# r4dl/LAENeRF

Measured on AMD Instinct MI355X. Metric: Mrays/s, lego 800x800 train-step (4096 rays/step), higher is better.
Workload: dtype f16 (table, MLP) / f32 (march, composite)

## Files before the change

### include/laenerf.h

```cpp
#ifndef LAENERF_H
#define LAENERF_H

#include <stdint.h>

#ifdef __cplusplus
extern "C" {
#endif

#if defined(__GNUC__) || defined(__clang__)
#define LAE_API __attribute__((visibility("default")))
#else
#define LAE_API
#endif

#define LAE_OK 0
#define LAE_EINVAL (-1)
#define LAE_ELAUNCH (-2)
#define LAE_ENULL (-3)

#define LAE_F32 0
#define LAE_F16 1

#define LAE_GRID_HASH 0
#define LAE_GRID_TILED 1
#define LAE_INTERP_LINEAR 0
#define LAE_INTERP_SMOOTHSTEP 1

#define LAE_ACT_RELU 0
#define LAE_ACT_EXPONENTIAL 1
#define LAE_ACT_SINE 2
#define LAE_ACT_SIGMOID 3
#define LAE_ACT_SQUAREPLUS 4
#define LAE_ACT_SOFTPLUS 5
#define LAE_ACT_NONE 6

#define LAE_ABI_TAG "abi10"
LAE_API const char* lae_version(void);
LAE_API const char* lae_last_error(void);


LAE_API int lae_near_far_from_aabb(const float* rays_o, const float* rays_d, const float* aabb,
                           uint32_t N, float min_near, float* nears, float* fars, void* stream);

LAE_API int lae_get_rays(const float* poses, uint32_t B, float fx, float fy, float cx, float cy, uint32_t H, uint32_t W,
                 const int64_t* inds, uint64_t inds_batch_stride, uint32_t N, int perturb, float off_x, float off_y,
                 float* rays_o, float* rays_d, const float* aabb, float min_near, float* nears, float* fars, void* stream);

#define LAE_IMG_U8 0
#define LAE_IMG_F16 1
#define LAE_IMG_F32 2
#define LAE_BATCH_IMAGE 0
#define LAE_BATCH_ALL 1
#define LAE_BG_WHITE 0
#define LAE_BG_RANDOM 1
LAE_API int lae_sample_train_batch(const void* images, int dtype, uint32_t n_img, uint32_t H, uint32_t W, uint32_t C,
                           const float* poses, float fx, float fy, float cx, float cy, uint32_t N,
                           const float* aabb, float min_near, uint64_t seed, int64_t* step_counter, int mode, int bg_mode,
                           int srgb_to_linear, float* rays_o, float* rays_d, float* nears, float* fars, float* gt,
                           float* bg_out, int64_t* inds, void* stream);

LAE_API int lae_sample_train_batch_weighted(const void* images, int dtype, uint32_t n_img, uint32_t H, uint32_t W, uint32_t C,
                                    const float* poses, float fx, float fy, float cx, float cy, uint32_t N,
                                    const float* aabb, float min_near, uint64_t seed, int64_t* step_counter, int bg_mode,
                                    int srgb_to_linear, const float* error_map, int32_t* cells_out, float* rays_o, float* rays_d,
                                    float* nears, float* fars, float* gt, float* bg_out, int64_t* inds, void* stream);

LAE_API int lae_error_map_update(float* error_map, uint32_t n_img, uint32_t H, uint32_t W, const int64_t* inds, const int32_t* cells,
                                 const float* pred, const float* gt, uint32_t N, void* stream);

LAE_API int lae_sph_from_ray(const float* rays_o, const float* rays_d, float radius, uint32_t N,
                     float* coords, void* stream);

LAE_API int lae_morton3D(const int32_t* coords, uint32_t N, int32_t* indices, void* stream);

LAE_API int lae_morton3D_invert(const int32_t* indices, uint32_t N, int32_t* coords, void* stream);

LAE_API int lae_packbits(const float* grid, uint32_t N, float density_thresh, uint8_t* bitfield,
                 void* stream);

LAE_API uint64_t lae_march_rays_train_scratch_bytes(uint32_t N);
LAE_API int lae_march_rays_train(const float* rays_o, const float* rays_d, const uint8_t* grid,
                         float bound, float dt_gamma, uint32_t max_steps,
                         uint32_t N, uint32_t C, uint32_t H, uint32_t M,
                         const float* nears, const float* fars,
                         float* xyzs, float* dirs, float* deltas,
                         int32_t* rays, int32_t* counter, const float* noises,
                         void* scratch, uint32_t* rows_end_out, void* stream);

LAE_API int lae_march_rays_train_limit(const float* rays_o, const float* rays_d, const uint8_t* grid,
                               float bound, float dt_gamma, uint32_t max_steps,
                               uint32_t N, uint32_t C, uint32_t H, uint32_t M_cap, const uint32_t* m_limit,
                               const float* nears, const float* fars,
                               float* xyzs, float* dirs, float* deltas,
                               int32_t* rays, int32_t* counter, const float* noises,
                               void* scratch, uint32_t* rows_end_out, void* stream);

LAE_API int lae_composite_rays_train_forward(const float* sigmas, const float* rgbs, const float* deltas,
                                     const int32_t* rays, uint32_t M, uint32_t N, float T_thresh,
                                     float* weights_sum, float* depth, float* image, void* stream);

LAE_API int lae_composite_rays_train_backward(const float* grad_weights_sum, const float* grad_image,
                                      const float* sigmas, const float* rgbs, const float* deltas,
                                      const int32_t* rays, const float* weights_sum,
                                      const float* image, uint32_t M, uint32_t N, float T_thresh,
                                      float* grad_sigmas, float* grad_rgbs, void* stream);

LAE_API int lae_composite_rays_train_forward_blend(const float* sigmas, const float* rgbs, const float* deltas, const int32_t* rays,
                                           uint32_t M, uint32_t N, float T_thresh, const float* nears, const float* fars,
                                           const float* bg_rays, float bg_r, float bg_g, float bg_b, float* weights_sum,
                                           float* depth, float* image, float* depth_out, float* image_out, void* stream);
LAE_API int lae_composite_rays_train_step(const float* sigmas, const float* rgbs, const float* deltas, const int32_t* rays, uint32_t M,
                                  uint32_t N, float T_thresh, const float* nears, const float* fars, const float* bg_rays, float bg_r,
                                  float bg_g, float bg_b, const uint32_t* rows_end, const float* target, const float* scale,
                                  float* weights_sum, float* depth, float* image, float* depth_out, float* image_out,
                                  float* grad_image, float* grad_sigmas, float* grad_rgbs, float* loss_out, float* partials,
                                  int defer_loss, void* stream);
LAE_API int lae_loss_finish(const float* partials, uint32_t n_part, uint32_t n_elem, const float* scale, float* loss_out, void* stream);

LAE_API int lae_composite_rays_train_backward_blend(const float* grad_weights_sum, const float* grad_image, const float* sigmas,
                                            const float* rgbs, const float* deltas, const int32_t* rays,
                                            const float* weights_sum, const float* image, uint32_t M, uint32_t N,
                                            float T_thresh, const float* bg_rays, float bg_r, float bg_g, float bg_b,
                                            const uint32_t* rows_end, float* grad_sigmas, float* grad_rgbs, void* stream);
LAE_API int lae_composite_rays_train_backward_blend_ex(const float* grad_weights_sum, const float* grad_image, const float* sigmas,
                                               const float* rgbs, const float* deltas, const int32_t* rays,
                                               const float* weights_sum, const float* image, uint32_t M, uint32_t N,
                                               float T_thresh, const float* bg_rays, float bg_r, float bg_g, float bg_b,
                                               const uint32_t* rows_end, const float* grad_scale, float* grad_sigmas,
                                               float* grad_rgbs, void* stream);

LAE_API int lae_march_rays(uint32_t n_alive, uint32_t n_step, const int32_t* rays_alive,
                   const float* rays_t, const float* rays_o, const float* rays_d,
                   float bound, float dt_gamma, uint32_t max_steps, uint32_t C, uint32_t H,
                   const uint8_t* grid, const float* nears, const float* fars,
                   float* xyzs, float* dirs, float* deltas, const float* noises, void* stream);

LAE_API int lae_march_rays_distill(uint32_t n_alive, uint32_t n_step, const int32_t* rays_alive,
                           const float* rays_t, const float* rays_o, const float* rays_d,
                           float bound, float dt_gamma, uint32_t max_steps, uint32_t C, uint32_t H,
                           const uint8_t* grid, const uint8_t* edit_grid,
                           const float* nears, const float* fars,
                           float* xyzs, float* dirs, float* deltas, uint8_t* edit_occ,
                           const float* noises, void* stream);

LAE_API int lae_composite_rays(uint32_t n_alive, uint32_t n_step, float T_thresh,
                       int32_t* rays_alive, float* rays_t,
                       const float* sigmas, const float* rgbs, const float* deltas,
                       float* weights_sum, float* depth, float* image, void* stream);

LAE_API int lae_composite_rays_distill(uint32_t n_alive, uint32_t n_step, float T_thresh,
                               int32_t* rays_alive, float* rays_t,
                               const float* sigmas, const float* rgbs, const float* deltas,
                               float* weights_sum, float* weights_edit_sum,
                               float* depth, float* depth_edit,
                               const uint8_t* edit_occ, float* image, void* stream);

LAE_API uint64_t lae_render_frame_workspace_bytes(uint32_t N, uint32_t L, uint64_t row_budget);
LAE_API int lae_render_frame_set_overlap(int on);
LAE_API int lae_render_frame_mode(void);
LAE_API int lae_render_frame_last_status(void);
LAE_API int lae_render_frame_probe_us(float* us, uint32_t n);
LAE_API int lae_render_frame(const float* rays_o, const float* rays_d, uint32_t N, const float* aabb, float min_near,
                     const uint8_t* grid, const uint8_t* edit_grid, float bound, float dt_gamma, uint32_t max_steps,
                     uint32_t C, uint32_t H, const void* table_f16, const int32_t* offsets, const int32_t* offsets_host,
                     uint32_t L, float S,
                     uint32_t base_resolution, uint32_t gridtype, int align_corners, uint32_t interp,
                     const void* sigma_weights, const void* color_weights, float density_scale, float T_thresh,
                     uint32_t max_n_step, uint64_t row_budget, const float* noises, const float* bg_rays, float bg_r, float bg_g,
                     float bg_b, int blend_bg, int scale_depth, float* weights_sum, float* depth, float* image,
                     float* weights_edit, float* depth_edit, void* workspace, uint64_t workspace_bytes, uint32_t* stats_out,
                     void* stream);

LAE_API uint64_t lae_compact_scratch_bytes(uint32_t n_alive);
LAE_API int lae_compact_rays_alive(const int32_t* rays_alive, uint32_t n_alive, int32_t* out_alive,
                           int32_t* n_out_dev, void* scratch, void* stream);


LAE_API int lae_grid_encode_forward(const float* inputs, const void* embeddings, const int32_t* offsets,
                            void* outputs, uint32_t B, uint32_t D, uint32_t C, uint32_t L,
                            float S, uint32_t H, void* dy_dx, uint32_t gridtype,
                            int align_corners, uint32_t interp, int dtype, void* stream);

LAE_API int lae_grid_encode_backward(const void* grad, const float* inputs, const void* embeddings,
                             const int32_t* offsets, void* grad_embeddings, uint32_t B,
                             uint32_t D, uint32_t C, uint32_t L, float S, uint32_t H,
                             const void* dy_dx, void* grad_inputs, uint32_t gridtype,
                             int align_corners, uint32_t interp, int dtype, void* stream);

LAE_API int lae_grid_encode_forward_ex(const float* inputs, const void* embeddings, const int32_t* offsets, void* outputs,
                               uint32_t B, uint32_t D, uint32_t C, uint32_t L, float S, uint32_t H, void* dy_dx,
                               uint32_t gridtype, int align_corners, uint32_t interp, int dtype, int blc, float in_shift,
                               float in_scale, const int32_t* offsets_host, void* stream);
LAE_API int lae_grid_encode_backward_ex(const void* grad, const float* inputs, const void* embeddings, const int32_t* offsets,
                                void* grad_embeddings, uint32_t B, uint32_t D, uint32_t C, uint32_t L, float S,
                                uint32_t H, const void* dy_dx, void* grad_inputs, uint32_t gridtype,
                                int align_corners, uint32_t interp, int dtype, int blc, float in_shift, float in_scale,
                                const int32_t* offsets_host, int32_t* nonfinite_flag, uint32_t* touched_lines, void* stream);

LAE_API uint64_t lae_grid_backward_plan_bytes(uint32_t B, uint32_t L);
LAE_API uint64_t lae_grid_touched_lines_words(uint64_t n_entries);
LAE_API int lae_grid_encode_backward_plan(const float* inputs, const int32_t* offsets, uint32_t B, uint32_t D, uint32_t C, uint32_t L,
                                  float S, uint32_t H, uint32_t gridtype, int align_corners, uint32_t interp, int dtype,
                                  float in_shift, float in_scale, const int32_t* offsets_host, void* plan,
                                  uint32_t* touched_lines, void* stream);
LAE_API int lae_grid_encode_backward_planned(const void* grad, const float* inputs, const int32_t* offsets, void* grad_embeddings,
                                     uint32_t B, uint32_t D, uint32_t C, uint32_t L, float S, uint32_t H, uint32_t gridtype,
                                     int align_corners, uint32_t interp, int dtype, float in_shift, float in_scale,
                                     const int32_t* offsets_host, const void* plan, int32_t* nonfinite_flag, void* stream);

LAE_API uint64_t lae_grid_backward_workspace_bytes(uint32_t B, uint32_t L, int dtype);

LAE_API int lae_grid_forward_schedule(const int32_t* offsets_host, uint32_t L, float S, uint32_t H, uint32_t n_chunks,
                              uint32_t* nseg_out, uint32_t* segs_out);

LAE_API int lae_grid_set_forward_mode(int mode);

LAE_API int lae_grid_set_backward_mode(int mode);

LAE_API int lae_grad_total_variation(const void* inputs, const void* embeddings, void* grad,
                             const int32_t* offsets, float weight, uint32_t B, uint32_t D,
                             uint32_t C, uint32_t L, float S, uint32_t H, uint32_t gridtype,
                             int align_corners, int dtype, void* stream);


LAE_API int lae_sh_encode_forward(const float* inputs, float* outputs, uint32_t B, uint32_t D,
                          uint32_t C, float* dy_dx, void* stream);

LAE_API int lae_sh_encode_backward(const float* grad, const float* inputs, uint32_t B, uint32_t D,
                           uint32_t C, const float* dy_dx, float* grad_inputs, void* stream);


LAE_API int lae_ffmlp_forward(const void* inputs, const void* weights, uint32_t B, uint32_t input_dim,
                      uint32_t output_dim, uint32_t hidden_dim, uint32_t num_layers,
                      uint32_t activation, uint32_t output_activation, void* forward_buffer,
                      void* outputs, void* stream);

LAE_API int lae_ffmlp_inference(const void* inputs, const void* weights, uint32_t B, uint32_t input_dim,
                        uint32_t output_dim, uint32_t hidden_dim, uint32_t num_layers,
                        uint32_t activation, uint32_t output_activation, void* inference_buffer,
                        void* outputs, void* stream);

LAE_API int lae_ffmlp_backward(const void* grad, const void* inputs, const void* weights,
                       const void* forward_buffer, uint32_t B, uint32_t input_dim,
                       uint32_t output_dim, uint32_t hidden_dim, uint32_t num_layers,
                       uint32_t activation, uint32_t output_activation, int calc_grad_inputs,
                       void* backward_buffer, void* grad_inputs, void* grad_weights,
                       void* stream);
LAE_API int lae_ffmlp_backward_ex(const void* grad, const void* inputs, const void* weights,
                          const void* forward_buffer, uint32_t B, uint32_t input_dim,
                          uint32_t output_dim, uint32_t hidden_dim, uint32_t num_layers,
                          uint32_t activation, uint32_t output_activation, int calc_grad_inputs,
                          void* backward_buffer, void* grad_inputs, void* grad_weights,
                          int accumulate, int32_t* nonfinite_flag, void* stream);

LAE_API int lae_nerf_head_forward(const void* enc, const float* dirs, const void* sigma_weights, const void* color_weights,
                          uint32_t M, float density_scale, void* h_out, float* sigmas, float* rgbs, int enc_level_major,
                          void* stream);

LAE_API int lae_nerf_density_forward(const void* enc, const void* sigma_weights, uint32_t M, float density_scale, void* h_out,
                             float* sigmas, int enc_level_major, void* stream);

LAE_API int lae_nerf_head_backward(const float* grad_sigmas, const float* grad_rgbs, const void* enc, const float* dirs, const void* h,
                           const float* rgbs, const void* sigma_weights, const void* color_weights, uint32_t M,
                           float density_scale, void* grad_h, void* grad_enc, void* grad_sigma_weights,
                           void* grad_color_weights, int accumulate_weight_grads, int enc_level_major,
                           int32_t* nonfinite_flag, const float* loss_partials, uint32_t loss_n_part, uint32_t loss_n_elem,
                           const float* loss_scale, float* loss_out, void* stream);

LAE_API int lae_freq_encode_forward(const float* inputs, uint32_t B, uint32_t D, uint32_t deg, uint32_t C, float* outputs,
                            void* stream);
LAE_API int lae_freq_encode_backward(const float* grad, const float* outputs, uint32_t B, uint32_t D, uint32_t deg, uint32_t C,
                             float* grad_inputs, void* stream);

LAE_API int lae_palette_forward(const void* w_logits, const void* o_raw, const float* palette, uint32_t P, uint32_t active_mask,
                        uint32_t M, void* pred, float* w_hat, void* o_hat, void* stream);
LAE_API uint64_t lae_palette_backward_scratch_bytes(uint32_t M);
LAE_API int lae_palette_backward(const void* w_logits, const void* o_raw, const float* palette, uint32_t P, uint32_t active_mask,
                         uint32_t M, const void* g_pred, const float* g_w, const void* g_o, void* g_w_logits, void* g_o_raw,
                         float* g_palette, void* scratch, void* stream);

#define LAE_RECOLOR_PREVIEW 0
#define LAE_RECOLOR_WEIGHTS 1
#define LAE_RECOLOR_OFFSETS 2
#define LAE_RECOLOR_EVAL 3
#define LAE_RECOLOR_NO_OFFSETS 1
#define LAE_RECOLOR_TANH 2
LAE_API uint64_t lae_recolor_compact_scratch_bytes(uint32_t N);
LAE_API int lae_recolor_compact(const float* depth, const float* weights_sum, const float* rays_o, const float* rays_d, uint32_t N,
                                int32_t* indices, int32_t* slot_map, float* x_term, float* dirs, float* alpha, int32_t* count,
                                void* scratch, void* stream);
LAE_API int lae_recolor_compose(const int32_t* slot_map, uint32_t N, const void* w_logits, uint32_t w_stride, const void* o_raw,
                                uint32_t o_stride, uint32_t P, uint32_t active_mask, const float* palette, const float* p_weights,
                                const float* p_bias, const float* alpha, const float* base, const float* bg, int mode, uint32_t k,
                                int flags, float* out, uint8_t* out_u8, void* stream);

#define LAE_STYLE_WITH_REG 1
#define LAE_STYLE_ACCUMULATE_PALETTE 2
LAE_API uint64_t lae_style_loss_scratch_bytes(uint32_t M);
LAE_API int lae_style_loss_forward(const void* pred, const float* target, const float* w_hat, const void* o_hat, uint32_t M,
                           uint32_t n_active, float w_uniform, float w_non_uniform, float c_offset, const float* scale, float* fin,
                           void* scratch, const float* reg_palette, uint32_t reg_P, float w_valid, float w_distinct, void* stream);
LAE_API int lae_style_loss_backward(const void* w_logits, const void* o_raw, const float* palette, uint32_t P, uint32_t active_mask,
                            uint32_t M, const float* target, const float* fin, const float* upstream, float w_uniform,
                            float w_non_uniform, float c_offset, void* g_w_logits, void* g_o_raw, float* g_palette, void* scratch,
                            int flags, float w_valid, float w_distinct, void* stream);

LAE_API int lae_style_loss_forward_dev(const void* pred, const float* target, const float* w_hat, const void* o_hat, uint32_t cap,
                               const uint32_t* m_dev, uint32_t n_active, float w_uniform, float w_non_uniform, float c_offset,
                               const float* scale, float* fin, void* scratch, const float* reg_palette, uint32_t reg_P, float w_valid,
                               float w_distinct, void* stream);
LAE_API int lae_style_loss_backward_dev(const void* w_logits, const void* o_raw, const float* palette, uint32_t P, uint32_t active_mask,
                                uint32_t cap, const uint32_t* m_dev, const float* target, const float* fin, const float* upstream,
                                float w_uniform, float w_non_uniform, float c_offset, void* g_w_logits, void* g_o_raw, float* g_palette,
                                void* scratch, int flags, float w_valid, float w_distinct, void* stream);

LAE_API int lae_sample_edit_view(const float* x_term, const float* dirs, const float* targets, const int64_t* offsets, const int32_t* counts,
                         const float* depth_factor, uint32_t V, const int32_t* schedule, uint32_t n_sched, uint32_t cap, uint64_t seed,
                         int64_t* step_counter, float* x, float* d, float* target, uint32_t* m_dev, void* stream);

LAE_API int lae_style_assemble_forward(const void* feats_lm, const float* dirs, uint32_t M, uint32_t Mp, uint32_t degree, void* feat,
                               void* off_in, uint32_t off_cols, void* stream);
LAE_API int lae_style_assemble_backward(const void* g_feat, const void* g_off, uint32_t M, uint32_t off_cols, void* grad_lm, void* stream);

LAE_API int lae_grow_region(uint8_t* grid, const float* density_grid, uint32_t C, uint32_t H, float density_thresh,
                    uint32_t* queue, uint32_t capacity, uint32_t* state, uint32_t grow_iterations, uint32_t max_batch,
                    void* stream);

LAE_API int lae_min_dist_to_points(const float* pts, uint32_t n, const float* set, uint32_t m, float max_dist, float* out,
                           float* out_max, void* scratch, void* stream);

LAE_API int lae_density_grid_positions(const int32_t* coords, uint32_t n, uint32_t H, float bound_c, const float* noise,
                               float* xyzs, int32_t* indices, void* stream);
LAE_API uint64_t lae_density_grid_partial_scratch_bytes(uint32_t cells, uint32_t n);
LAE_API int lae_density_grid_partial_positions(const float* grid_c, uint32_t cells, const int32_t* coords_rand, const float* u, const float* rnd,
                                       uint32_t n, uint32_t H, float bound_c, const float* noise, float* xyzs, int32_t* indices,
                                       void* scratch, void* stream);
LAE_API int lae_density_grid_update(const float* sigmas, const int32_t* indices, uint32_t n, float density_scale, float decay,
                            uint32_t cells, float* grid, uint32_t* tmp, void* stream);
LAE_API int lae_mark_untrained_grid(const float* poses, uint32_t B, float fx, float fy, float cx, float cy, uint32_t C, uint32_t H,
                            float bound, float min_near, int filter_close_point, float* grid, void* stream);

LAE_API int lae_adam_check(const void* grad, int grad_is_half, uint64_t n, void* state, void* stream);
LAE_API int lae_adam_begin(void* state, float beta1, float beta2, int growth_interval, float growth_factor, float backoff_factor,
                   int use_scaler, void* stream);
LAE_API int lae_adam_apply(float* param, float* exp_avg, float* exp_avg_sq, void* grad, int grad_is_half, void* shadow_half, uint64_t n,
                   const void* state, const float* lr, float beta1, float beta2, float eps, float weight_decay, void* stream);

LAE_API int lae_mse_loss_forward(const float* pred, const float* target, uint32_t n, const float* scale, float* loss_out, float* grad,
                         void* stream);

LAE_API int lae_adam_check_multi(uint32_t n_tensors, const void* const* grads, const int* grad_is_half, const uint64_t* sizes, void* state,
                         void* stream);
LAE_API int lae_adam_apply_multi(uint32_t n_tensors, float* const* params, float* const* exp_avgs, float* const* exp_avg_sqs, void* const* grads,
                         const int* grad_is_half, void* const* shadows_half, const uint64_t* sizes, const float* const* lrs, const void* const* touched_lines,
                         const void* state, float beta1, float beta2, float eps, float weight_decay, void* stream);

LAE_API int lae_ema_update_multi(uint32_t n_tensors, float* const* shadows, const float* const* params, const uint64_t* sizes,
                         float one_minus_decay, void* stream);

LAE_API int lae_ffmlp_set_mode(int mode);

LAE_API int lae_allocate_splitk(uint64_t size);
LAE_API int lae_free_splitk(void);

LAE_API int lae_free_workspaces(void);
LAE_API uint64_t lae_workspace_bytes(int retired);

#ifdef __cplusplus
}
#endif
#endif
```

### laenerf_amd/_lib.py

```python
import ctypes
import os

import torch

_HERE = os.path.dirname(os.path.abspath(__file__))
SO_PATH = os.environ.get("LAE_HIP_LIB") or os.path.join(_HERE, "lib", "liblaenerf_hip.so")

u32, u64, f32, i32, vp = ctypes.c_uint32, ctypes.c_uint64, ctypes.c_float, ctypes.c_int, ctypes.c_void_p

SIGNATURES = {
    "lae_near_far_from_aabb": [vp, vp, vp, u32, f32, vp, vp, vp],
    "lae_sph_from_ray": [vp, vp, f32, u32, vp, vp],
    "lae_get_rays": [vp, u32, f32, f32, f32, f32, u32, u32, vp, u64, u32, i32, f32, f32, vp, vp, vp, f32, vp, vp, vp],
    "lae_morton3D": [vp, u32, vp, vp],
    "lae_morton3D_invert": [vp, u32, vp, vp],
    "lae_packbits": [vp, u32, f32, vp, vp],
    "lae_march_rays_train_scratch_bytes": [u32],
    "lae_march_rays_train": [vp, vp, vp, f32, f32, u32, u32, u32, u32, u32, vp, vp, vp, vp, vp, vp, vp, vp, vp, vp, vp],
    "lae_march_rays_train_limit": [vp, vp, vp, f32, f32, u32, u32, u32, u32, u32, vp, vp, vp, vp, vp, vp, vp, vp, vp, vp, vp, vp],
    "lae_sample_train_batch": [vp, i32, u32, u32, u32, u32, vp, f32, f32, f32, f32, u32, vp, f32, u64, vp, i32, i32, i32, vp, vp, vp, vp, vp,
                               vp, vp, vp],
    "lae_sample_train_batch_weighted": [vp, i32, u32, u32, u32, u32, vp, f32, f32, f32, f32, u32, vp, f32, u64, vp, i32, i32, vp, vp,
                                        vp, vp, vp, vp, vp, vp, vp, vp],
    "lae_error_map_update": [vp, u32, u32, u32, vp, vp, vp, vp, u32, vp],
    "lae_composite_rays_train_forward": [vp, vp, vp, vp, u32, u32, f32, vp, vp, vp, vp],
    "lae_composite_rays_train_backward": [vp, vp, vp, vp, vp, vp, vp, vp, u32, u32, f32, vp, vp, vp],
    "lae_composite_rays_train_forward_blend": [vp, vp, vp, vp, u32, u32, f32, vp, vp, vp, f32, f32, f32, vp, vp, vp, vp, vp, vp],
    "lae_composite_rays_train_step": [vp, vp, vp, vp, u32, u32, f32, vp, vp, vp, f32, f32, f32, vp, vp, vp, vp, vp, vp, vp, vp, vp, vp, vp, vp, vp, i32, vp],
    "lae_loss_finish": [vp, u32, u32, vp, vp, vp],
    "lae_composite_rays_train_backward_blend": [vp, vp, vp, vp, vp, vp, vp, vp, u32, u32, f32, vp, f32, f32, f32, vp, vp, vp, vp],
    "lae_composite_rays_train_backward_blend_ex": [vp, vp, vp, vp, vp, vp, vp, vp, u32, u32, f32, vp, f32, f32, f32, vp, vp, vp, vp, vp],
    "lae_march_rays": [u32, u32, vp, vp, vp, vp, f32, f32, u32, u32, u32, vp, vp, vp, vp, vp, vp, vp, vp],
    "lae_march_rays_distill": [u32, u32, vp, vp, vp, vp, f32, f32, u32, u32, u32, vp, vp, vp, vp, vp, vp, vp, vp, vp, vp],
    "lae_composite_rays": [u32, u32, f32, vp, vp, vp, vp, vp, vp, vp, vp, vp],
    "lae_composite_rays_distill": [u32, u32, f32, vp, vp, vp, vp, vp, vp, vp, vp, vp, vp, vp, vp],
    "lae_render_frame_workspace_bytes": [u32, u32, u64],
    "lae_render_frame_set_overlap": [i32],
    "lae_render_frame_mode": [],
    "lae_render_frame_last_status": [],
    "lae_render_frame_probe_us": [vp, u32],
    "lae_render_frame": [vp, vp, u32, vp, f32, vp, vp, f32, f32, u32, u32, u32, vp, vp, vp, u32, f32, u32, u32, i32, u32, vp, vp, f32, f32,
                         u32, u64, vp, vp, f32, f32, f32, i32, i32, vp, vp, vp, vp, vp, vp, u64, vp, vp],
    "lae_compact_scratch_bytes": [u32],
    "lae_compact_rays_alive": [vp, u32, vp, vp, vp, vp],
    "lae_grid_encode_forward": [vp, vp, vp, vp, u32, u32, u32, u32, f32, u32, vp, u32, i32, u32, i32, vp],
    "lae_grid_encode_backward": [vp, vp, vp, vp, vp, u32, u32, u32, u32, f32, u32, vp, vp, u32, i32, u32, i32, vp],
    "lae_grid_encode_forward_ex": [vp, vp, vp, vp, u32, u32, u32, u32, f32, u32, vp, u32, i32, u32, i32, i32, f32, f32, vp, vp],
    "lae_grid_encode_backward_ex": [vp, vp, vp, vp, vp, u32, u32, u32, u32, f32, u32, vp, vp, u32, i32, u32, i32, i32, f32, f32, vp, vp, vp, vp],
    "lae_grid_backward_workspace_bytes": [u32, u32, i32],
    "lae_grid_backward_plan_bytes": [u32, u32],
    "lae_grid_touched_lines_words": [u64],
    "lae_grid_encode_backward_plan": [vp, vp, u32, u32, u32, u32, f32, u32, u32, i32, u32, i32, f32, f32, vp, vp, vp, vp],
    "lae_grid_encode_backward_planned": [vp, vp, vp, vp, u32, u32, u32, u32, f32, u32, u32, i32, u32, i32, f32, f32, vp, vp, vp, vp],
    "lae_grid_set_backward_mode": [i32],
    "lae_grid_set_forward_mode": [i32],
    "lae_grid_forward_schedule": [vp, u32, f32, u32, u32, vp, vp],
    "lae_grad_total_variation": [vp, vp, vp, vp, f32, u32, u32, u32, u32, f32, u32, u32, i32, i32, vp],
    "lae_sh_encode_forward": [vp, vp, u32, u32, u32, vp, vp],
    "lae_sh_encode_backward": [vp, vp, u32, u32, u32, vp, vp, vp],
    "lae_freq_encode_forward": [vp, u32, u32, u32, u32, vp, vp],
    "lae_freq_encode_backward": [vp, vp, u32, u32, u32, u32, vp, vp],
    "lae_ffmlp_forward": [vp, vp, u32, u32, u32, u32, u32, u32, u32, vp, vp, vp],
    "lae_ffmlp_inference": [vp, vp, u32, u32, u32, u32, u32, u32, u32, vp, vp, vp],
    "lae_ffmlp_backward": [vp, vp, vp, vp, u32, u32, u32, u32, u32, u32, u32, i32, vp, vp, vp, vp],
    "lae_ffmlp_backward_ex": [vp, vp, vp, vp, u32, u32, u32, u32, u32, u32, u32, i32, vp, vp, vp, i32, vp, vp],
    "lae_nerf_head_forward": [vp, vp, vp, vp, u32, f32, vp, vp, vp, i32, vp],
    "lae_nerf_density_forward": [vp, vp, u32, f32, vp, vp, i32, vp],
    "lae_density_grid_positions": [vp, u32, u32, f32, vp, vp, vp, vp],
    "lae_density_grid_partial_scratch_bytes": [u32, u32],
    "lae_density_grid_partial_positions": [vp, u32, vp, vp, vp, u32, u32, f32, vp, vp, vp, vp, vp],
    "lae_density_grid_update": [vp, vp, u32, f32, f32, u32, vp, vp, vp],
    "lae_mark_untrained_grid": [vp, u32, f32, f32, f32, f32, u32, u32, f32, f32, i32, vp, vp],
    "lae_nerf_head_backward": [vp, vp, vp, vp, vp, vp, vp, vp, u32, f32, vp, vp, vp, vp, i32, i32, vp, vp, u32, u32, vp, vp, vp],
    "lae_palette_forward": [vp, vp, vp, u32, u32, u32, vp, vp, vp, vp],
    "lae_palette_backward_scratch_bytes": [u32],
    "lae_palette_backward": [vp, vp, vp, u32, u32, u32, vp, vp, vp, vp, vp, vp, vp, vp],
    "lae_recolor_compact_scratch_bytes": [u32],
    "lae_recolor_compact": [vp, vp, vp, vp, u32, vp, vp, vp, vp, vp, vp, vp, vp],
    "lae_recolor_compose": [vp, u32, vp, u32, vp, u32, u32, u32, vp, vp, vp, vp, vp, vp, i32, u32, i32, vp, vp, vp],
    "lae_style_loss_scratch_bytes": [u32],
    "lae_style_loss_forward": [vp, vp, vp, vp, u32, u32, f32, f32, f32, vp, vp, vp, vp, u32, f32, f32, vp],
    "lae_style_loss_backward": [vp, vp, vp, u32, u32, u32, vp, vp, vp, f32, f32, f32, vp, vp, vp, vp, i32, f32, f32, vp],
    "lae_style_loss_forward_dev": [vp, vp, vp, vp, u32, vp, u32, f32, f32, f32, vp, vp, vp, vp, u32, f32, f32, vp],
    "lae_style_loss_backward_dev": [vp, vp, vp, u32, u32, u32, vp, vp, vp, vp, f32, f32, f32, vp, vp, vp, vp, i32, f32, f32, vp],
    "lae_sample_edit_view": [vp, vp, vp, vp, vp, vp, u32, vp, u32, u32, u64, vp, vp, vp, vp, vp, vp],
    "lae_grow_region": [vp, vp, u32, u32, f32, vp, u32, vp, u32, u32, vp],
    "lae_style_assemble_forward": [vp, vp, u32, u32, u32, vp, vp, u32, vp],
    "lae_style_assemble_backward": [vp, vp, u32, u32, vp, vp],
    "lae_min_dist_to_points": [vp, u32, vp, u32, f32, vp, vp, vp, vp],
    "lae_mse_loss_forward": [vp, vp, u32, vp, vp, vp, vp],
    "lae_adam_check": [vp, i32, u64, vp, vp],
    "lae_adam_check_multi": [u32, vp, vp, vp, vp, vp],
    "lae_adam_apply_multi": [u32, vp, vp, vp, vp, vp, vp, vp, vp, vp, vp, f32, f32, f32, f32, vp],
    "lae_adam_begin": [vp, f32, f32, i32, f32, f32, i32, vp],
    "lae_ema_update_multi": [u32, vp, vp, vp, f32, vp],
    "lae_adam_apply": [vp, vp, vp, vp, i32, vp, u64, vp, vp, f32, f32, f32, f32, vp],
    "lae_ffmlp_set_mode": [i32],
    "lae_allocate_splitk": [u64],
    "lae_free_splitk": [],
    "lae_free_workspaces": [],
    "lae_workspace_bytes": [i32],
    "lae_version": [],
    "lae_last_error": [],
}
_RESTYPES = {
    "lae_march_rays_train_scratch_bytes": u64,
    "lae_compact_scratch_bytes": u64,
    "lae_density_grid_partial_scratch_bytes": u64,
    "lae_palette_backward_scratch_bytes": u64,
    "lae_style_loss_scratch_bytes": u64,
    "lae_recolor_compact_scratch_bytes": u64,
    "lae_render_frame_workspace_bytes": u64,
    "lae_workspace_bytes": u64,
    "lae_grid_backward_workspace_bytes": u64,
    "lae_grid_backward_plan_bytes": u64,
    "lae_grid_touched_lines_words": u64,
    "lae_version": ctypes.c_char_p,
    "lae_last_error": ctypes.c_char_p,
}

_lib = None
ABI_TAG = b"abi10"


def _abi_of(path):
    lib = ctypes.CDLL(path)
    fn = lib.lae_version
    fn.argtypes, fn.restype = [], ctypes.c_char_p
    return lib, fn().split()[-1]


def load():
    global _lib
    if _lib is not None:
        return _lib
    if not os.path.exists(SO_PATH):
        raise RuntimeError(
            f"laenerf_amd: HIP library not built ({SO_PATH}); run `python -m laenerf_amd.build` "
            "(there is no CPU fallback)")
    if not os.environ.get("LAE_HIP_LIB"):
        from . import build as _build
        if _build.default_is_packed(SO_PATH):
            _build.build(force=True)
            if _build.default_is_packed(SO_PATH):
                raise RuntimeError(f"laenerf_amd: {SO_PATH} was built with packed-fp32 instructions and could not be rebuilt without them")
    lib, tag = _abi_of(SO_PATH)
    if tag != ABI_TAG:
        if os.environ.get("LAE_HIP_LIB"):
            raise RuntimeError(f"laenerf_amd: {SO_PATH} is ABI {tag.decode()}, this package binds {ABI_TAG.decode()}")
        import fcntl
        import shutil
        from . import build as _build
        with open(SO_PATH + ".lock", "w") as lock:
            fcntl.flock(lock, fcntl.LOCK_EX)
            try:
                probe = SO_PATH + f".{os.getpid()}.probe"
                shutil.copyfile(SO_PATH, probe)
                try:
                    still_stale = _abi_of(probe)[1] != ABI_TAG
                finally:
                    os.remove(probe)
                if still_stale:
                    _build.build(force=True)
            finally:
                fcntl.flock(lock, fcntl.LOCK_UN)
        fresh = SO_PATH + f".{os.getpid()}.reload"
        shutil.copyfile(SO_PATH, fresh)
        try:
            lib, tag = _abi_of(fresh)
        finally:
            os.remove(fresh)
        if tag != ABI_TAG:
            raise RuntimeError(f"laenerf_amd: rebuilt library is ABI {tag.decode()}, this package binds {ABI_TAG.decode()}")
    for name, argtypes in SIGNATURES.items():
        fn = getattr(lib, name)
        fn.argtypes = argtypes
        fn.restype = _RESTYPES.get(name, ctypes.c_int)
    _lib = lib
    return lib


def check(rc, what):
    if rc != 0:
        msg = load().lae_last_error().decode() if rc == -2 else {-1: "invalid argument / unsupported configuration",
                                                                 -3: "null pointer"}.get(rc, "error")
        raise RuntimeError(f"laenerf_amd.{what} failed (code {rc}): {msg}")


def ptr(t):
    return None if t is None else t.data_ptr()


def stream():
    return torch.cuda.current_stream().cuda_stream


def need_cuda(*tensors):
    cur = None
    for t in tensors:
        if t is None:
            continue
        if not t.is_cuda:
            raise RuntimeError("laenerf_amd: tensor must be on the GPU (HIP backend, no CPU fallback)")
        if cur is None:
            cur = torch.cuda.current_device()
# ... 10 lines not shown
```

### laenerf_amd/backend.py

```python
import sys
import types

import numpy as np
import torch

from . import _lib
from ._lib import check, need_contig, need_cuda, ptr, stream

_F16 = torch.float16


def _dtype_code(t):
    if t.dtype == torch.float32:
        return 0
    if t.dtype == torch.float16:
        return 1
    raise RuntimeError(f"laenerf_amd: unsupported dtype {t.dtype} (float32 / float16 only)")


def _host_i32(a, n):
    if a is None:
        return None
    if not (isinstance(a, np.ndarray) and a.dtype == np.int32 and a.flags.c_contiguous and a.size == n):
        raise RuntimeError("laenerf_amd: offsets_host must be a contiguous int32 numpy array with L + 1 entries")
# ... 291 lines not shown
        check(lib.lae_render_frame(ptr(rays_o), ptr(rays_d), N, ptr(aabb), float(min_near), ptr(grid), ptr(edit_grid), float(bound),
                                   float(dt_gamma), max_steps, C, H, ptr(table_f16), ptr(offsets), _host_i32(offsets_host, L + 1), L, float(S),
                                   base_resolution,
                                   gridtype, int(bool(align_corners)), interp, ptr(sigma_weights), ptr(color_weights),
                                   float(density_scale), float(T_thresh), max_n_step, int(row_budget), ptr(noises), ptr(bg_rays), float(bg_rgb[0]),
                                   float(bg_rgb[1]), float(bg_rgb[2]), int(bool(blend_bg)), int(bool(scale_depth)), ptr(weights_sum),
                                   ptr(depth), ptr(image), ptr(weights_edit), ptr(depth_edit), ptr(ws), ws.numel(),
                                   ctypes.cast(stats, ctypes.c_void_p) if want_stats else None, stream()), "render_frame")
        if want_stats:
            if lib.lae_render_frame_last_status() == 1:
                raise RuntimeError("laenerf_amd.render_frame: a cross-stream wait timed out behind the call; the frame's outputs are NaN")
            return {"iterations": stats[0], "rows": stats[1], "iterations_launched": stats[2]}
        return None

    @staticmethod
    def render_frame_set_overlap(on):
        check(_lib.load().lae_render_frame_set_overlap(int(bool(on))), "render_frame_set_overlap")

    @staticmethod
    def render_frame_probe():
        import ctypes
        us = (ctypes.c_float * 5)(*([-1.0] * 5))
        used = int(_lib.load().lae_render_frame_probe_us(ctypes.cast(us, ctypes.c_void_p), 5))
        return {"in_use": used, "handshake_us": [round(float(v), 1) for v in us]}

    @staticmethod
    def render_frame_mode():
        return int(_lib.load().lae_render_frame_mode())

    @staticmethod
    def render_frame_last_status():
        return int(_lib.load().lae_render_frame_last_status())

    @staticmethod
    def render_frame_check():
        torch.cuda.current_stream().synchronize()
        if _lib.load().lae_render_frame_last_status() == 1:
            raise RuntimeError("laenerf_amd.render_frame: a cross-stream wait of the most recent frame timed out after the call returned; "
                               "its outputs are NaN -- render the frame again (the library runs in line from now on)")

    @staticmethod
    def compact_rays_alive(rays_alive, n_alive, out_alive, n_out_dev):
        need_cuda(rays_alive, out_alive, n_out_dev)
        lib = _lib.load()
        ws = _workspace(rays_alive.device, lib.lae_compact_scratch_bytes(n_alive))
        check(lib.lae_compact_rays_alive(ptr(rays_alive), n_alive, ptr(out_alive), ptr(n_out_dev), ptr(ws), stream()),
              "compact_rays_alive")


class _GridEncoder:
    @staticmethod
    def grid_encode_forward(inputs, embeddings, offsets, outputs, B, D, C, L, S, H, dy_dx, gridtype, align_corners,
                            interp, blc=False, in_map=(0.0, 1.0), offsets_host=None):
        need_cuda(inputs, embeddings, offsets, outputs, dy_dx); need_contig(inputs, embeddings, offsets, outputs, dy_dx)
        if inputs.dtype != torch.float32 or offsets.dtype != torch.int32:
            raise RuntimeError("grid_encode_forward: inputs must be float32, offsets int32")
        if outputs.dtype != embeddings.dtype or (dy_dx is not None and dy_dx.dtype != embeddings.dtype):
            raise RuntimeError("grid_encode_forward: outputs/dy_dx must have the embeddings dtype")
        lib = _lib.load()
        args = (ptr(inputs), ptr(embeddings), ptr(offsets), ptr(outputs), B, D, C, L, float(S), H, ptr(dy_dx), gridtype,
                int(bool(align_corners)), interp, _dtype_code(embeddings))
        if blc or tuple(in_map) != (0.0, 1.0) or offsets_host is not None:
            check(lib.lae_grid_encode_forward_ex(*args, int(bool(blc)), float(in_map[0]), float(in_map[1]), _host_i32(offsets_host, L + 1),
                                                 stream()), "grid_encode_forward")
        else:
            check(lib.lae_grid_encode_forward(*args, stream()), "grid_encode_forward")

    @staticmethod
    def grid_backward_plan(inputs, offsets, B, D, C, L, S, H, gridtype, align_corners, interp, half, in_map=(0.0, 1.0),
                           offsets_host=None, touched_lines=None):
        need_cuda(inputs, offsets); need_contig(inputs, offsets)
        lib = _lib.load()
        plan = torch.empty(int(lib.lae_grid_backward_plan_bytes(B, L)), dtype=torch.uint8, device=inputs.device)
        check(lib.lae_grid_encode_backward_plan(ptr(inputs), ptr(offsets), B, D, C, L, float(S), H, gridtype, int(bool(align_corners)),
                                                interp, 1 if half else 0, float(in_map[0]), float(in_map[1]),
                                                _host_i32(offsets_host, L + 1), ptr(plan), touched_lines, stream()),
              "grid_backward_plan")
        plan.marks_touched = touched_lines is not None
        return plan

    @staticmethod
    def grid_encode_backward(grad, inputs, embeddings, offsets, grad_embeddings, B, D, C, L, S, H, dy_dx, grad_inputs,
                             gridtype, align_corners, interp, blc=False, in_map=(0.0, 1.0), offsets_host=None, plan=None,
                             nonfinite_flag=None, touched_lines=None):
        ts = (grad, inputs, embeddings, offsets, grad_embeddings, dy_dx, grad_inputs, plan)
        need_cuda(*ts); need_contig(*ts)
        if grad.dtype != grad_embeddings.dtype:
            raise RuntimeError("grid_encode_backward: grad and grad_embeddings dtypes differ")
        lib = _lib.load()
        if plan is not None:
            if blc or dy_dx is not None:
                raise RuntimeError("grid_encode_backward: a plan needs level-major gradients and no input gradient")
            if touched_lines is not None and not getattr(plan, "marks_touched", False):
                raise RuntimeError("grid_encode_backward: the plan was made without the touched-lines bitmap (pass it to grid_backward_plan)")
            check(lib.lae_grid_encode_backward_planned(ptr(grad), ptr(inputs), ptr(offsets), ptr(grad_embeddings), B, D, C, L, float(S), H,
                                                       gridtype, int(bool(align_corners)), interp, _dtype_code(grad), float(in_map[0]),
                                                       float(in_map[1]), _host_i32(offsets_host, L + 1), ptr(plan), nonfinite_flag, stream()),
                  "grid_encode_backward")
            return
        args = (ptr(grad), ptr(inputs), ptr(embeddings), ptr(offsets), ptr(grad_embeddings), B, D, C, L, float(S), H,
                ptr(dy_dx), ptr(grad_inputs), gridtype, int(bool(align_corners)), interp, _dtype_code(grad))
        if blc or tuple(in_map) != (0.0, 1.0) or offsets_host is not None or nonfinite_flag is not None or touched_lines is not None:
            check(lib.lae_grid_encode_backward_ex(*args, int(bool(blc)), float(in_map[0]), float(in_map[1]), _host_i32(offsets_host, L + 1),
                                                  nonfinite_flag, touched_lines, stream()), "grid_encode_backward")
        else:
            check(lib.lae_grid_encode_backward(*args, stream()), "grid_encode_backward")

    @staticmethod
    def grid_backward_workspace_bytes(B, L, half=True):
        return int(_lib.load().lae_grid_backward_workspace_bytes(B, L, 1 if half else 0))

    @staticmethod
    def set_backward_mode(mode):
        check(_lib.load().lae_grid_set_backward_mode(int(mode)), "grid_set_backward_mode")

    @staticmethod
    def grad_total_variation(inputs, embeddings, grad, offsets, weight, B, D, C, L, S, H, gridtype, align_corners):
        need_cuda(inputs, embeddings, grad, offsets); need_contig(inputs, embeddings, grad, offsets)
        check(_lib.load().lae_grad_total_variation(ptr(inputs), ptr(embeddings), ptr(grad), ptr(offsets), float(weight), B, D,
                                                   C, L, float(S), H, gridtype, int(bool(align_corners)),
                                                   _dtype_code(embeddings), stream()), "grad_total_variation")


class _SHEncoder:
    @staticmethod
    def sh_encode_forward(inputs, outputs, B, D, C, dy_dx):
        need_cuda(inputs, outputs, dy_dx); need_contig(inputs, outputs, dy_dx)
        if inputs.dtype != torch.float32 or outputs.dtype != torch.float32:
            raise RuntimeError("sh_encode_forward: float32 required (sphere_harmonics.py:16 casts to fp32)")
        check(_lib.load().lae_sh_encode_forward(ptr(inputs), ptr(outputs), B, D, C, ptr(dy_dx), stream()), "sh_encode_forward")

    @staticmethod
    def sh_encode_backward(grad, inputs, B, D, C, dy_dx, grad_inputs):
        need_cuda(grad, inputs, dy_dx, grad_inputs); need_contig(grad, inputs, dy_dx, grad_inputs)
        if grad.dtype != torch.float32:
            raise RuntimeError("sh_encode_backward: float32 required")
        check(_lib.load().lae_sh_encode_backward(ptr(grad), ptr(inputs), B, D, C, ptr(dy_dx), ptr(grad_inputs), stream()),
              "sh_encode_backward")


class _FreqEncoder:

    @staticmethod
    def freq_encode_forward(inputs, B, D, deg, C, outputs):
        need_cuda(inputs, outputs); need_contig(inputs, outputs); _need_f32(inputs, outputs)
        check(_lib.load().lae_freq_encode_forward(ptr(inputs), B, D, deg, C, ptr(outputs), stream()), "freq_encode_forward")

    @staticmethod
    def freq_encode_backward(grad, outputs, B, D, deg, C, grad_inputs):
        need_cuda(grad, outputs, grad_inputs); need_contig(grad, outputs, grad_inputs); _need_f32(grad, outputs, grad_inputs)
        check(_lib.load().lae_freq_encode_backward(ptr(grad), ptr(outputs), B, D, deg, C, ptr(grad_inputs), stream()),
              "freq_encode_backward")


class _FFMLP:
    @staticmethod
    def _half(*ts):
        for t in ts:
            if t is not None and t.dtype != _F16:
                raise RuntimeError("ffmlp: float16 tensors required (CHECK_IS_HALF, ffmlp.cu:638-642)")

    @staticmethod
    def ffmlp_forward(inputs, weights, B, input_dim, output_dim, hidden_dim, num_layers, activation, output_activation,
                      forward_buffer, outputs):
        need_cuda(inputs, weights, forward_buffer, outputs); need_contig(inputs, weights, forward_buffer, outputs)
        _FFMLP._half(inputs, weights, forward_buffer, outputs)
        check(_lib.load().lae_ffmlp_forward(ptr(inputs), ptr(weights), B, input_dim, output_dim, hidden_dim, num_layers,
                                            activation, output_activation, ptr(forward_buffer), ptr(outputs), stream()),
              "ffmlp_forward")

    @staticmethod
    def ffmlp_inference(inputs, weights, B, input_dim, output_dim, hidden_dim, num_layers, activation, output_activation,
                        inference_buffer, outputs):
        need_cuda(inputs, weights, outputs); need_contig(inputs, weights, outputs)
        _FFMLP._half(inputs, weights, outputs)
        check(_lib.load().lae_ffmlp_inference(ptr(inputs), ptr(weights), B, input_dim, output_dim, hidden_dim, num_layers,
                                              activation, output_activation, ptr(inference_buffer), ptr(outputs), stream()),
              "ffmlp_inference")

    @staticmethod
    def ffmlp_backward(grad, inputs, weights, forward_buffer, B, input_dim, output_dim, hidden_dim, num_layers, activation,
                       output_activation, calc_grad_inputs, backward_buffer, grad_inputs, grad_weights, accumulate=False,
                       nonfinite_flag=None):
        ts = (grad, inputs, weights, forward_buffer, backward_buffer, grad_inputs, grad_weights)
        need_cuda(*ts); need_contig(*ts); _FFMLP._half(*ts)
        if accumulate or nonfinite_flag is not None:
            check(_lib.load().lae_ffmlp_backward_ex(ptr(grad), ptr(inputs), ptr(weights), ptr(forward_buffer), B, input_dim,
# ... 283 lines not shown
```

### laenerf_amd/csrc/gridencoder.hip

```cpp
#include <math.h>
#include <stdio.h>
#include <stdlib.h>
#include <algorithm>
#include <type_traits>
#include "lae_common.h"
#include <vector>
#include <mutex>
#include <utility>

namespace {

constexpr int MAX_LEVELS = 32;
struct LevelScales { float scale[MAX_LEVELS]; float in_shift, in_scale; };

typedef _Float16 half_t;
typedef _Float16 half2_t __attribute__((ext_vector_type(2)));

__constant__ uint32_t k_primes[7] = {1u, 2654435761u, 805459861u, 3674653429u, 2097192037u, 1434869437u, 2165219737u};

#ifdef LAE_GRID_STAMPS
__device__ unsigned long long g_grid_stamps[32768 * 32];
#define GRID_STAMP(slot, i) do { if (threadIdx.x == 0 && (uint32_t)(i) < 32u) g_grid_stamps[(size_t)(slot) * 32 + (i)] = wall_clock64(); } while (0)
#define GRID_NOTE(slot, i, v) do { if (threadIdx.x == 0 && (uint32_t)(i) < 32u) g_grid_stamps[(size_t)(slot) * 32 + (i)] = (v); } while (0)
#else
// ... 292 lines not shown
struct LevelBins { uint32_t P, SUB; };
__host__ __device__ __forceinline__ LevelBins level_bins_of(uint32_t hashmap_size, uint32_t bk_target = BK_TARGET) {
    LevelBins lb;
    lb.P = (hashmap_size + PART - 1) >> PART_SHIFT;
    lb.SUB = lb.P >= bk_target ? 1u : (bk_target + lb.P - 1) / lb.P;
    return lb;
}
__host__ __device__ __forceinline__ bool level_is_binned(uint32_t hashmap_size) { return level_bins_of(hashmap_size).P <= BK_MAX; }


template <typename T, int D, int C>
__global__ __launch_bounds__(GRID_BLOCK) void k_grid_bwd(
    const T* __restrict__ grad, const float* __restrict__ inputs, const int32_t* __restrict__ offsets,
    T* __restrict__ grad_grid, uint32_t B, uint32_t L, LevelScales sc, uint32_t gridtype, bool align_corners,
    uint32_t interp, uint32_t nb, bool xcd_mode, uint64_t gs_b, uint64_t gs_l, bool only_unbinned) {
    uint32_t level, chunk;
    block_to_level_chunk(nb, xcd_mode, level, chunk);
    if (level >= L) return;
    const uint32_t b = chunk * GRID_BLOCK + threadIdx.x;
    if (b >= B) return;
    const LevelInfo<D> li = level_info<D>(sc, offsets, level, gridtype, align_corners);
    if (only_unbinned) {
        if constexpr (D == 3) { if (level_is_binned(li.hashmap_size)) return; }
    }
    T* __restrict__ tab = grad_grid + (size_t)li.table_off * C;

    float frac[D];
    uint32_t pg[D];
#pragma unroll
    for (int d = 0; d < D; d++) {
        const float xv = (inputs[(size_t)b * D + d] + sc.in_shift) * sc.in_scale;
        if (xv < 0.0f || xv > 1.0f) return;
        float p = fmaf(xv, li.scale, align_corners ? 0.0f : 0.5f);
        const float fl = floorf(p);
        pg[d] = (uint32_t)fl;
        p -= (float)pg[d];
        if (interp == 1) p = p * p * (3.0f - 2.0f * p);
        frac[d] = p;
    }
    const T* g = grad + (size_t)b * gs_b + (size_t)level * gs_l;
    float gc[C];
#pragma unroll
    for (int ch = 0; ch < C; ch++) gc[ch] = (float)g[ch];

#pragma unroll
    for (int idx = 0; idx < (1 << D); idx++) {
        float w = 1.0f;
        uint32_t pgl[D];
#pragma unroll
        for (int d = 0; d < D; d++) {
            if ((idx & (1 << d)) == 0) { w *= 1 - frac[d]; pgl[d] = pg[d]; }
            else { w *= frac[d]; pgl[d] = pg[d] + 1; }
        }
        const uint32_t gi = cell_index<D>(li, pgl) * C;
        if constexpr (sizeof(T) == 2) {
            static_assert(C % 2 == 0 || sizeof(T) == 4, "fp16 grads need an even channel count");
#pragma unroll
            for (int ch = 0; ch < C; ch += 2) {
                half2_t v = {(half_t)(w * gc[ch]), (half_t)(w * gc[ch + 1])};
                __builtin_amdgcn_global_atomic_fadd_v2f16(
                    (__attribute__((address_space(1))) half2_t*)(tab + gi + ch), v);
            }
        } else {
#pragma unroll
            for (int ch = 0; ch < C; ch++) atomicAdd(tab + gi + ch, w * gc[ch]);
        }
    }
}

template <typename T> struct BVal;
template <> struct BVal<half_t> { using type = uint2; };
template <> struct BVal<float> { using type = float4; };
constexpr int FILL_THREADS = 256;
constexpr int SPT = 4;
constexpr int SEGS = 1;
constexpr uint32_t UNIT_SAMPLES = FILL_THREADS * SPT;
constexpr uint32_t STAGE_CAP = 4096 + 256;
constexpr uint32_t KEY_SINGLE = 15u;
constexpr int ACC_THREADS = 1024;
constexpr uint32_t BWD_MAX_SAMPLES = 1u << 24;
constexpr uint32_t COARSE_RES = 64;
constexpr bool WIDE_COARSE_UNITS = false;
constexpr uint32_t SUB_RECS = 64;
constexpr uint32_t TICKET_ARRIVALS = 2;
constexpr uint32_t TICKET_WORDS = TICKET_ARRIVALS + MAX_LEVELS * SUB_RECS;
template <typename T> constexpr uint32_t sub_rec_words() { return (sizeof(T) == 2 ? 2 * PART : PART) + PART / 64; }

struct BwdPlan {
    uint16_t* cnt;
    uint32_t* part_cnt;
    uint32_t* totals;
    uint32_t* offs;
    uint32_t* tickets;
};

__device__ __forceinline__ uint32_t pack_half2(float a, float b) {
    const half2_t h = {(half_t)a, (half_t)b};
    return __builtin_bit_cast(uint32_t, h);
}

template <typename T, bool FILL, bool PLAIN>
__global__ __launch_bounds__(FILL_THREADS) void k_bwd_walk(
    const T* __restrict__ gradT, const float* __restrict__ inputs, const int32_t* __restrict__ offsets, uint32_t B,
    uint32_t L, LevelScales sc, uint32_t gridtype_, bool align_corners_, uint32_t interp_, uint32_t U, BwdPlan plan,
    typename BVal<T>::type* __restrict__ qvals, uint16_t* __restrict__ qkeys, uint32_t* __restrict__ touched_,
    uint32_t* __restrict__ level_full) {
    const uint32_t gridtype = PLAIN ? 0u : gridtype_, interp = PLAIN ? 0u : interp_;
    const bool align_corners = PLAIN ? false : align_corners_;
    using V = typename BVal<T>::type;
    if constexpr (FILL) GRID_STAMP(blockIdx.x, 0);
    const uint32_t NBLK = U / SEGS;
    const uint32_t level = blockIdx.x / NBLK, chunk = blockIdx.x % NBLK;
    if (FILL && blockIdx.x == 0) for (uint32_t k = threadIdx.x; k < TICKET_WORDS; k += FILL_THREADS) plan.tickets[k] = 0;
    const LevelInfo<3> li = level_info<3>(sc, offsets, level, gridtype, align_corners);
    const uint32_t P = (li.hashmap_size + PART - 1) >> PART_SHIFT;
    if (P > BK_MAX) return;
    __shared__ uint32_t hist[BK_MAX], start[BK_MAX + 1], gbase[FILL ? BK_MAX : 1];
    __shared__ __attribute__((aligned(16))) V s_vals[FILL ? STAGE_CAP : 1];
    __shared__ __attribute__((aligned(16))) uint16_t s_keys[FILL ? STAGE_CAP : 8];
    extern __shared__ uint32_t s_lines[];
    const uint32_t tid = threadIdx.x, lane = tid & 63u;
    const uint32_t line_shift = (li.table_off >> 3) & 31u;
    const uint32_t line_words = (line_shift + ((li.hashmap_size + 7u) >> 3) + 31u) >> 5;
    __shared__ uint32_t s_mark;
    if (!FILL) {
        if (tid == 0) s_mark = (touched_ && !level_full[level]) ? 1u : 0u;
        __syncthreads();
    }
    uint32_t* __restrict__ touched = (!FILL && s_mark) ? touched_ : nullptr;
    if (!FILL && touched) { for (uint32_t k = tid; k < line_words; k += FILL_THREADS) s_lines[k] = 0u; }
    const bool wide = li.resolution < COARSE_RES && WIDE_COARSE_UNITS;
    const uint32_t NSUB = wide ? 4u : 1u;
    if (wide && (chunk & 3u)) {
        if constexpr (!FILL) {
            const uint32_t u_e = chunk * SEGS, unit_e = level * U + u_e;
            for (uint32_t k = tid; k < BK_MAX / 2; k += FILL_THREADS) reinterpret_cast<uint32_t*>(plan.cnt + (size_t)unit_e * BK_MAX)[k] = 0u;
            for (uint32_t k = tid; k < P; k += FILL_THREADS) plan.part_cnt[((size_t)level * BK_MAX + k) * U + u_e] = 0u;
        }
        return;
    }
    const uint32_t b0 = wide ? ((chunk >> 2) * (UNIT_SAMPLES * 4u) + tid * (SPT * 4u)) : (chunk * FILL_THREADS + tid) * (SPT * SEGS);
    const uint32_t NC = (P <= BK_MAX / 8 && li.resolution >= COARSE_RES) ? 8u : 1u;
    const T* __restrict__ g_lvl = gradT + (size_t)level * B * 2;

    uint32_t cpg[3] = {0, 0, 0};
    bool have = false;
    float a0[8], a1[8];
#pragma unroll
    for (int c = 0; c < 8; c++) { a0[c] = 0.f; a1[c] = 0.f; }

    struct Rows { uint32_t c0[4], k0[4], c1[4], k1[4], i0[4], i1[4]; bool pair[4]; };
    auto cell_rows = [&](const uint32_t (&cp)[3], Rows& r) {
        const uint32_t lane_copy = lane & (NC - 1);
        if (li.use_hash && li.pow2) {
            const uint32_t m = li.hashmap_size - 1u;
            const uint32_t dx = (cp[0] ^ (cp[0] + 1u)) & m;
            const bool pr = dx != 0u && dx < PART;
            const uint32_t code = (pr ? (uint32_t)(__builtin_popcount(dx) - 1) : KEY_SINGLE) << 12;
            const uint32_t hy0 = cp[1] * 2654435761u, hy1 = hy0 + 2654435761u, hz0 = cp[2] * 805459861u, hz1 = hz0 + 805459861u;
#pragma unroll
            for (int yz = 0; yz < 4; yz++) {
                const uint32_t i0 = (cp[0] ^ ((yz & 1) ? hy1 : hy0) ^ ((yz & 2) ? hz1 : hz0)) & m, i1 = i0 ^ dx;
                r.c0[yz] = (i0 >> PART_SHIFT) * NC + lane_copy; r.c1[yz] = (i1 >> PART_SHIFT) * NC + lane_copy;
                r.i0[yz] = i0; r.i1[yz] = i1;
                r.pair[yz] = pr;
                r.k0[yz] = (i0 & (PART - 1)) | code;
// ... 246 lines not shown
                    const uint32_t np = min(64u, kend - kb);
#pragma unroll 4
                    for (uint32_t q = 0; q < np; q += 2) {
                        const int src = (int)(q + (lane >> 5));
                        const uint32_t s0 = __shfl(s0v, src, 64), s1 = __shfl(s1v, src, 64), gb = __shfl(gbv, src, 64);
                        for (uint32_t i = s0 + (lane & 31u); i < s1; i += 32) { qvals[gb + (i - s0)] = s_vals[i]; qkeys[gb + (i - s0)] = s_keys[i]; }
                    }
                }
            }
            GRID_STAMP(blockIdx.x, 6);
            GRID_NOTE(blockIdx.x, 7, total);
            __syncthreads();
        }
    }
}

__global__ __launch_bounds__(256) void k_bwd_scan_units(const int32_t* __restrict__ offsets, uint32_t L, uint32_t U, BwdPlan plan) {
    const uint32_t t = blockIdx.x * 4 + (threadIdx.x >> 6);
    if (t >= L * BK_MAX) return;
    const uint32_t level = t / BK_MAX, k = t % BK_MAX;
    const uint32_t size = (uint32_t)(offsets[level + 1] - offsets[level]);
    const uint32_t P = (size + PART - 1) >> PART_SHIFT;
    const int lane = threadIdx.x & 63;
    if (P > BK_MAX || k >= P) { if (lane == 0) plan.totals[t] = 0; return; }
    uint32_t* p = plan.part_cnt + (size_t)t * U;
    uint32_t carry = 0;
    for (uint32_t c0 = 0; c0 < U; c0 += 64) {
        const uint32_t c = c0 + lane;
        const uint32_t v = c < U ? p[c] : 0u;
        const uint32_t inc = lae::wave_incl_scan(v);
        if (c < U) p[c] = carry + inc - v;
        carry += __shfl(inc, 63, 64);
    }
    if (lane == 0) plan.totals[t] = carry;
}

__global__ __launch_bounds__(1024) void k_bwd_scan_parts(uint32_t n, BwdPlan plan) {
    __shared__ uint32_t lds[17];
    uint32_t carry = 0;
    for (uint32_t base = 0; base < n; base += 1024) {
        const uint32_t i = base + threadIdx.x;
        const uint32_t v = i < n ? plan.totals[i] : 0;
        uint32_t total;
        const uint32_t ex = lae::block_excl_scan<16>(v, &total, lds);
        if (i < n) plan.offs[i] = carry + ex;
        carry += total;
    }
}

__device__ __forceinline__ long long half_to_fix24(uint32_t u) {
    const uint32_t e = (u >> 10) & 31u;
    const int32_t smask = (int32_t)(u << 16) >> 31;
    const uint32_t mant = (u & 1023u) | (min(e, 1u) << 10);
    const int32_t sm = (int32_t)(mant ^ (uint32_t)smask) - smask;
    return (long long)sm << (max(e, 1u) - 1u);
}
__device__ __forceinline__ void half2_to_fix24_small(uint32_t w, long long& lo, long long& hi) {
    const half2_t h = __builtin_bit_cast(half2_t, w);
    lo = (long long)(int32_t)((float)h[0] * 16777216.0f);
    hi = (long long)(int32_t)((float)h[1] * 16777216.0f);
}
__device__ __forceinline__ uint32_t fix24_to_half(long long t) {
    const uint32_t sign = t < 0 ? 0x8000u : 0u;
    const unsigned long long mag = t < 0 ? (unsigned long long)(-t) : (unsigned long long)t;
    if (mag < 1024ull) return sign | (uint32_t)mag;
    const int msb = 63 - __builtin_clzll(mag);
    const int shift = msb - 10;
    unsigned long long q = mag >> shift;
    if (shift > 0) {
        const unsigned long long rem = mag & ((1ull << shift) - 1ull), halfway = 1ull << (shift - 1);
        if (rem > halfway || (rem == halfway && (q & 1ull))) q++;
    }
    int e = msb - 9;
    if (q == 2048ull) { q = 1024ull; e++; }
    if (e >= 31) return sign | 0x7c00u;
    return sign | ((uint32_t)e << 10) | ((uint32_t)q & 1023u);
}
__device__ __forceinline__ bool half_nonfinite(uint32_t u) { return (u & 0x7c00u) == 0x7c00u; }

template <typename T>
__global__ __launch_bounds__(ACC_THREADS, 8) void k_bwd_acc(
    const int32_t* __restrict__ offsets, T* __restrict__ grad_grid, uint32_t L, LevelScales sc, uint32_t gridtype,
    bool align_corners, BwdPlan plan, const typename BVal<T>::type* __restrict__ qvals, const uint16_t* __restrict__ qkeys,
    unsigned long long* __restrict__ partials, int32_t* __restrict__ nf_flag, uint32_t bk_target) {
    using V = typename BVal<T>::type;
    constexpr bool HALF = sizeof(T) == 2;
    constexpr uint32_t ACCW = HALF ? 2 * PART : PART;
    __shared__ unsigned long long acc64[ACCW];
    __shared__ uint32_t poison[PART / 32];
    __shared__ uint32_t s_cnt[MAX_LEVELS], s_sub[MAX_LEVELS], s_first[MAX_LEVELS];
    __shared__ uint32_t s_ticket, s_arr;
    const uint32_t tid = threadIdx.x;
    if (tid < L) {
        const LevelBins lb = level_bins_of((uint32_t)(offsets[tid + 1] - offsets[tid]), bk_target);
        s_cnt[tid] = lb.P <= BK_MAX ? lb.P * lb.SUB : 0u;
        s_sub[tid] = lb.SUB;
    }
    __syncthreads();
    if (tid == 0) { uint32_t run = 0; for (uint32_t l = 0; l < L; l++) { s_first[l] = run; run += s_cnt[l]; } s_arr = run; }
    __syncthreads();
    const uint32_t total_buckets = s_arr;
    __syncthreads();

    auto apply = [&](uint32_t key, const V& v) {
        const uint32_t e0 = key & (PART - 1), code = key >> 12;
        const uint32_t e1 = e0 ^ ((2u << code) - 1u);
        if constexpr (HALF) {
            const uint32_t w0 = v.x, w1 = v.y;
            const uint32_t carry = (((w0 & 0x7c007c00u) + 0x28002800u) | ((w1 & 0x7c007c00u) + 0x28002800u)) & 0x80008000u;
            if (carry == 0) {
                long long a, b;
                half2_to_fix24_small(w0, a, b);
                atomicAdd(&acc64[e0], (unsigned long long)a);
                atomicAdd(&acc64[PART + e0], (unsigned long long)b);
                const uint32_t e1s = code != KEY_SINGLE ? e1 : e0;
                half2_to_fix24_small(w1, a, b);
                atomicAdd(&acc64[e1s], (unsigned long long)a);
                atomicAdd(&acc64[PART + e1s], (unsigned long long)b);
            } else {
                if (half_nonfinite(w0) || half_nonfinite(w0 >> 16)) atomicOr(&poison[e0 >> 5], 1u << (e0 & 31));
                else {
                    atomicAdd(&acc64[e0], (unsigned long long)half_to_fix24(w0 & 0xffffu));
                    atomicAdd(&acc64[PART + e0], (unsigned long long)half_to_fix24(w0 >> 16));
                }
                if (code != KEY_SINGLE) {
                    if (half_nonfinite(w1) || half_nonfinite(w1 >> 16)) atomicOr(&poison[e1 >> 5], 1u << (e1 & 31));
                    else {
                        atomicAdd(&acc64[e1], (unsigned long long)half_to_fix24(w1 & 0xffffu));
                        atomicAdd(&acc64[PART + e1], (unsigned long long)half_to_fix24(w1 >> 16));
                    }
                }
            }
        } else {
            float* af = reinterpret_cast<float*>(acc64);
            atomicAdd(af + e0, v.x); atomicAdd(af + PART + e0, v.y);
            if (code != KEY_SINGLE) { atomicAdd(af + e1, v.z); atomicAdd(af + PART + e1, v.w); }
        }
    };

    bool first_task = true;
    [[maybe_unused]] uint32_t stamp_task = 0;
    GRID_STAMP(4096 + blockIdx.x, 0);
    for (;;) {
        if (tid == 0) s_ticket = first_task ? blockIdx.x : atomicAdd(&plan.tickets[0], 1u) + gridDim.x;
        first_task = false;
        __syncthreads();
        const uint32_t t = __builtin_amdgcn_readfirstlane(s_ticket);
        GRID_STAMP(4096 + blockIdx.x, 1 + stamp_task * 6);
        if (t >= total_buckets) break;
        GRID_NOTE(4096 + blockIdx.x, 2 + stamp_task * 6, t);
        const uint32_t item = t;
        uint32_t level = 0;
        while (level + 1 < L && item >= s_first[level + 1]) level++;
        level = __builtin_amdgcn_readfirstlane(level);
        const uint32_t bk = item - __builtin_amdgcn_readfirstlane(s_first[level]);
        const uint32_t SUB = __builtin_amdgcn_readfirstlane(s_sub[level]), p = bk / SUB, sub = bk % SUB;
        const uint32_t table_off = (uint32_t)offsets[level], hashmap_size = (uint32_t)offsets[level + 1] - table_off;
        const uint32_t n = __builtin_amdgcn_readfirstlane(plan.totals[level * BK_MAX + p]), q0 = __builtin_amdgcn_readfirstlane(plan.offs[level * BK_MAX + p]);
        const uint32_t lo = (uint32_t)(((uint64_t)n * sub) / SUB), hi = (uint32_t)(((uint64_t)n * (sub + 1)) / SUB);
        if (n == 0) { __syncthreads(); continue; }
        const uint32_t part_lo = p << PART_SHIFT;
        const uint32_t n_ent = min(PART, hashmap_size - part_lo);
        T* __restrict__ dst = grad_grid + ((size_t)table_off + part_lo) * 2;
        uint32_t oldv[HALF ? PART / ACC_THREADS : 1];
        if constexpr (HALF) {
#pragma unroll
            for (int it = 0; it < (int)(PART / ACC_THREADS); it++) { const uint32_t e = tid + it * ACC_THREADS; oldv[it] = e < n_ent ? reinterpret_cast<const uint32_t*>(dst)[e] : 0u; }
        }
        for (uint32_t i = tid; i < ACCW; i += ACC_THREADS) acc64[i] = 0ull;
        if (tid < PART / 32) poison[tid] = 0u;
        __syncthreads();
        GRID_STAMP(4096 + blockIdx.x, 3 + stamp_task * 6);
        const uint32_t scale_res = (uint32_t)ceilf(sc.scale[level]) + 1;
        const V* __restrict__ pv = qvals + q0;
        const uint16_t* __restrict__ pk = qkeys + q0;
        if (!HALF && scale_res >= COARSE_RES) {
            uint32_t i = lo + tid;
            for (; i + 3 * ACC_THREADS < hi; i += 4 * ACC_THREADS) {
                V v[4]; uint32_t k[4];
#pragma unroll
                for (int j = 0; j < 4; j++) { v[j] = pv[i + j * ACC_THREADS]; k[j] = pk[i + j * ACC_THREADS]; }
#pragma unroll
                for (int j = 0; j < 4; j++) apply(k[j], v[j]);
            }
            for (; i < hi; i += ACC_THREADS) { const V v = pv[i]; const uint32_t k = pk[i]; apply(k, v); }
        } else {
            if constexpr (HALF) {
                using u4 = __attribute__((__vector_size__(16))) uint32_t;
                const uint32_t abs_lo = q0 + lo, abs_hi = q0 + hi, A0 = abs_lo & ~7u;
                const uint32_t n_groups = (abs_hi - A0 + 7u) >> 3;
                const __amdgpu_buffer_rsrc_t rs_v = __builtin_amdgcn_make_buffer_rsrc(const_cast<V*>(qvals + A0), 0, (int)(n_groups * 64u), 0x00020000);
                const __amdgpu_buffer_rsrc_t rs_k = __builtin_amdgcn_make_buffer_rsrc(const_cast<uint16_t*>(qkeys + A0), 0, (int)(n_groups * 16u), 0x00020000);
                const bool coarse = scale_res < COARSE_RES;
                for (uint32_t gq = coarse ? (tid & 63u) * (ACC_THREADS / 64) + (tid >> 6) : tid; gq < n_groups; gq += ACC_THREADS) {
                    const u4 va = __builtin_amdgcn_raw_buffer_load_b128(rs_v, (int)(gq * 64u), 0, 0);
                    const u4 vb = __builtin_amdgcn_raw_buffer_load_b128(rs_v, (int)(gq * 64u + 16u), 0, 0);
                    const u4 vc = __builtin_amdgcn_raw_buffer_load_b128(rs_v, (int)(gq * 64u + 32u), 0, 0);
                    const u4 vd = __builtin_amdgcn_raw_buffer_load_b128(rs_v, (int)(gq * 64u + 48u), 0, 0);
                    const u4 kk = __builtin_amdgcn_raw_buffer_load_b128(rs_k, (int)(gq * 16u), 0, 0);
                    const uint32_t w[16] = {va[0], va[1], va[2], va[3], vb[0], vb[1], vb[2], vb[3], vc[0], vc[1], vc[2], vc[3], vd[0], vd[1], vd[2], vd[3]};
                    const uint32_t a0 = A0 + gq * 8u;
                    const uint32_t first = a0 < abs_lo ? abs_lo - a0 : 0u, last = min(8u, abs_hi - a0);
                    if (!coarse) {
#pragma unroll
                        for (int j = 0; j < 8; j++)
                            if ((uint32_t)j >= first && (uint32_t)j < last) { V v; v.x = w[2 * j]; v.y = w[2 * j + 1]; apply((kk[j >> 1] >> (16 * (j & 1))) & 0xffffu, v); }
                        continue;
                    }
                    uint32_t ckey = 0;
                    long long s00 = 0, s01 = 0, s10 = 0, s11 = 0;
                    bool bad0 = false, bad1 = false, started = false;
                    auto flush = [&]() {
                        const uint32_t e0 = ckey & (PART - 1), code = ckey >> 12;
                        const uint32_t e1 = e0 ^ ((2u << code) - 1u);
                        if (bad0) atomicOr(&poison[e0 >> 5], 1u << (e0 & 31));
                        else { atomicAdd(&acc64[e0], (unsigned long long)s00); atomicAdd(&acc64[PART + e0], (unsigned long long)s01); }
                        if (code != KEY_SINGLE) {
                            if (bad1) atomicOr(&poison[e1 >> 5], 1u << (e1 & 31));
                            else { atomicAdd(&acc64[e1], (unsigned long long)s10); atomicAdd(&acc64[PART + e1], (unsigned long long)s11); }
                        }
                    };
#pragma unroll
                    for (int j = 0; j < 8; j++) {
                        if ((uint32_t)j >= first && (uint32_t)j < last) {
                            const uint32_t kj = (kk[j >> 1] >> (16 * (j & 1))) & 0xffffu;
                            if (!started || kj != ckey) {
                                if (started) flush();
                                ckey = kj; s00 = s01 = s10 = s11 = 0; bad0 = bad1 = false; started = true;
                            }
                            const uint32_t w0 = w[2 * j], w1 = w[2 * j + 1];
                            const uint32_t carry = (((w0 & 0x7c007c00u) + 0x28002800u) | ((w1 & 0x7c007c00u) + 0x28002800u)) & 0x80008000u;
                            if (carry == 0) {
                                long long a, b;
                                half2_to_fix24_small(w0, a, b); s00 += a; s01 += b;
                                half2_to_fix24_small(w1, a, b); s10 += a; s11 += b;
                            } else {
                                if (half_nonfinite(w0) || half_nonfinite(w0 >> 16)) bad0 = true;
                                else { s00 += half_to_fix24(w0 & 0xffffu); s01 += half_to_fix24(w0 >> 16); }
                                if (half_nonfinite(w1) || half_nonfinite(w1 >> 16)) bad1 = true;
                                else { s10 += half_to_fix24(w1 & 0xffffu); s11 += half_to_fix24(w1 >> 16); }
                            }
                        }
                    }
                    if (started) flush();
                }
            } else {
                for (uint32_t c = lo + tid * 8u; c < hi; c += ACC_THREADS * 8u) {
                    V v[8]; uint32_t k[8];
#pragma unroll
                    for (int j = 0; j < 8; j++) { const uint32_t ii = min(c + (uint32_t)j, hi - 1u); v[j] = pv[ii]; k[j] = pk[ii]; }
                    const uint32_t cnt = min(8u, hi - c);
#pragma unroll
                    for (int j = 0; j < 8; j++) if ((uint32_t)j < cnt) apply(k[j], v[j]);
                }
            }
        }
        GRID_STAMP(4096 + blockIdx.x, 4 + stamp_task * 6);
        __syncthreads();
        GRID_STAMP(4096 + blockIdx.x, 5 + stamp_task * 6);
        if (SUB > 1) {
            unsigned long long* __restrict__ rec = partials + (size_t)(level * SUB_RECS + p) * sub_rec_words<T>();
            uint32_t* __restrict__ rec_poison = reinterpret_cast<uint32_t*>(rec + ACCW);
            if constexpr (HALF) {
                for (uint32_t i = tid; i < ACCW; i += ACC_THREADS) { const unsigned long long v = acc64[i]; if (v) atomicAdd(rec + i, v); }
            } else {
                const float* af = reinterpret_cast<const float*>(acc64);
                float* rf = reinterpret_cast<float*>(rec);
                for (uint32_t i = tid; i < 2 * PART; i += ACC_THREADS) { const float v = af[i]; if (v != 0.0f) atomicAdd(rf + i, v); }
            }
            if (tid < PART / 32 && poison[tid]) atomicOr(rec_poison + tid, poison[tid]);
            asm volatile("s_waitcnt vmcnt(0)" ::: "memory");
            __syncthreads();
            if (tid == 0) s_arr = atomicAdd(&plan.tickets[TICKET_ARRIVALS + level * SUB_RECS + p], 1u);
            __syncthreads();
            if (s_arr != SUB - 1) { GRID_STAMP(4096 + blockIdx.x, 6 + stamp_task * 6); stamp_task++; __syncthreads(); continue; }
            for (uint32_t i = tid; i < ACCW; i += ACC_THREADS) acc64[i] = atomicExch(rec + i, 0ull);
            if (tid < PART / 32) poison[tid] = atomicExch(rec_poison + tid, 0u);
            __syncthreads();
        }
        if constexpr (HALF) {
            uint32_t* d2 = reinterpret_cast<uint32_t*>(dst);
            bool wrote_nonfinite = false;
#pragma unroll
            for (int it = 0; it < (int)(PART / ACC_THREADS); it++) {
                const uint32_t e = tid + it * ACC_THREADS;
                if (e >= n_ent) break;
                const long long i0 = (long long)acc64[e], i1 = (long long)acc64[PART + e];
                const bool bad = (poison[e >> 5] >> (e & 31)) & 1u;
                if (i0 == 0 && i1 == 0 && !bad) continue;
                const uint32_t o = oldv[it];
                uint32_t r0, r1;
                if (bad) { r0 = 0x7e00u; r1 = 0x7e00u; }
                else {
                    r0 = half_nonfinite(o) ? (o & 0xffffu) : fix24_to_half(i0 + half_to_fix24(o & 0xffffu));
                    r1 = half_nonfinite(o >> 16) ? (o >> 16) : fix24_to_half(i1 + half_to_fix24(o >> 16));
                }
                d2[e] = r0 | (r1 << 16);
                wrote_nonfinite |= half_nonfinite(r0) || half_nonfinite(r1);
            }
            if (nf_flag && wrote_nonfinite) atomicOr(nf_flag, 1);
        } else {
            const float* af = reinterpret_cast<const float*>(acc64);
            float2* d2 = reinterpret_cast<float2*>(dst);
            for (uint32_t e = tid; e < n_ent; e += ACC_THREADS) {
                const float v0 = af[e], v1 = af[PART + e];
                if (v0 == 0.0f && v1 == 0.0f) continue;
                float2 o = d2[e]; o.x += v0; o.y += v1; d2[e] = o;
                if (nf_flag && !(isfinite(o.x) && isfinite(o.y))) atomicOr(nf_flag, 1);
            }
        }
        GRID_STAMP(4096 + blockIdx.x, 6 + stamp_task * 6);
        stamp_task++;
        __syncthreads();
    }
}

template <typename T>
__global__ __launch_bounds__(256) void k_out_transpose(const T* __restrict__ in, T* __restrict__ out, uint32_t B, uint32_t L) {
    using V = typename std::conditional<sizeof(T) == 2, uint32_t, uint2>::type;
    __shared__ V tile[256 * 33];
    const uint32_t b0 = blockIdx.x * 256;
    const uint32_t nb = min(256u, B - b0);
    const V* src = reinterpret_cast<const V*>(in);
    for (uint32_t e = threadIdx.x; e < nb * L; e += 256) {
        const uint32_t l = e / nb, b = e % nb;
        tile[b * (L + 1) + l] = src[(size_t)l * B + b0 + b];
    }
    __syncthreads();
    V* dstv = reinterpret_cast<V*>(out) + (size_t)b0 * L;
    for (uint32_t e = threadIdx.x; e < nb * L; e += 256) dstv[e] = tile[(e / L) * (L + 1) + (e % L)];
}

template <typename T>
__global__ __launch_bounds__(256) void k_grad_transpose(const T* __restrict__ in, T* __restrict__ out, uint32_t B, uint32_t L) {
    using V = typename std::conditional<sizeof(T) == 2, uint32_t, uint2>::type;
    __shared__ V tile[256 * 33];
    const uint32_t b0 = blockIdx.x * 256;
    const uint32_t nb = min(256u, B - b0);
    const V* src = reinterpret_cast<const V*>(in) + (size_t)b0 * L;
    for (uint32_t e = threadIdx.x; e < nb * L; e += 256) tile[(e / L) * (L + 1) + (e % L)] = src[e];
    __syncthreads();
    V* dstv = reinterpret_cast<V*>(out);
    for (uint32_t e = threadIdx.x; e < nb * L; e += 256) {
        const uint32_t l = e / nb, b = e % nb;
        dstv[(size_t)l * B + b0 + b] = tile[b * (L + 1) + l];
    }
}

template <typename T>
__global__ void k_grid_input_bwd(const T* __restrict__ grad, const T* __restrict__ dy_dx, T* __restrict__ grad_inputs,
                                 uint32_t B, uint32_t D, uint32_t C, uint32_t L, uint64_t gs_b, uint64_t gs_l) {
    const uint32_t t = blockIdx.x * blockDim.x + threadIdx.x;
    if (t >= B * D) return;
    const uint32_t b = t / D, d = t - b * D;
    const T* dd = dy_dx + (size_t)b * L * D * C;
    T r = (T)0.0f;
    for (uint32_t l = 0; l < L; l++)
        for (uint32_t ch = 0; ch < C; ch++) {
            const T gv = grad[(size_t)b * gs_b + (size_t)l * gs_l + ch];
            const T dv = dd[(size_t)l * D * C + d * C + ch];
            if constexpr (sizeof(T) == 2) r = (half_t)((float)r + (float)(half_t)((float)gv * (float)dv));
            else r = fmaf(gv, dv, r);
        }
    grad_inputs[t] = r;
}

template <int D, int C>
__global__ __launch_bounds__(GRID_BLOCK) void k_grad_tv(const float* __restrict__ inputs, const float* __restrict__ grid,
                                                         float* __restrict__ grad, const int32_t* __restrict__ offsets,
                                                         float weight, uint32_t B, uint32_t L, LevelScales sc,
                                                         uint32_t gridtype, bool align_corners, uint32_t nb) {
    uint32_t level, chunk;
    block_to_level_chunk(nb, false, level, chunk);
    if (level >= L) return;
    const uint32_t b = chunk * GRID_BLOCK + threadIdx.x;
// ... 128 lines not shown
                    c0 += pieces[x][l];
                }
                if (c0 != std::min(8u, lae::cdiv(nb, piece))) ok = false;
                continue;
            }
            for (int x = 0; x < 8; x++) {
                if (!pieces[x][l]) continue;
                const uint32_t n = std::min(pieces[x][l] * piece, nb - c0);
                if (fs.nseg[x] < FWD_MAX_SEG) fs.seg[x][fs.nseg[x]++] = FwdSeg{l, c0, n, 0u}; else ok = false;
                c0 += n;
            }
            if (c0 != nb) ok = false;
        }
    }
    if (!ok) fwd_sched_default(fs, L, nb);
    uint32_t mx = 0;
    for (int x = 0; x < 8; x++) {
        uint32_t t = 0;
        for (uint32_t q = 0; q < fs.nseg[x]; q++) t += fs.seg[x][q].n;
        mx = std::max(mx, t);
    }
    return mx;
}
static int g_fwd_mode = 0;

template <typename T, int D, int C>
static void launch_fwd(const FwdArgs& a) {
    const uint32_t nb_safe = lae::cdiv(a.B_dev ? a.B_launch : a.B, GRID_BLOCK);
    static const uint32_t tail_min_chunks = [] { const char* e = getenv("LAE_GRID_FWD_TAIL_MIN"); return e ? (uint32_t)atoi(e) : 2048u; }();
    uint32_t nb = a.B_dev && a.B_likely ? std::min((lae::cdiv(a.B_likely, GRID_BLOCK) + 7u) / 8u * 8u, nb_safe) : nb_safe;
    if (nb_safe - nb < tail_min_chunks) nb = nb_safe;
    if constexpr (std::is_same<T, half_t>::value && D == 3 && C == 2) {
        if (g_fwd_mode != 2 && !a.dy_dx && a.interp == 0 && !a.align && a.gridtype == 0 && a.L <= 8 * FWD_MAX_SEG && a.L <= MAX_LEVELS) {
            FwdSched fs;
            static const std::vector<float> env_cost = [] {
                std::vector<float> v; const char* e = getenv("LAE_GRID_FWD_COSTS");
                while (e && *e) { char* end; v.push_back(strtof(e, &end)); if (end == e) break; e = *end ? end + 1 : end; }
                return v; }();
            const float* co = a.level_cost ? a.level_cost : (env_cost.size() >= a.L ? env_cost.data() : nullptr);
            const uint32_t per_xcd = fwd_sched_build(fs, a.L, nb, a.sc, g_fwd_mode == 0 ? a.offsets_host : nullptr, a.B_dev != nullptr, co);
            k_grid_fwd_lean<<<per_xcd * 8, GRID_BLOCK, 0, a.stream>>>(a.inputs, (const half_t*)a.emb, a.offsets, (half_t*)a.out, std::min(a.B, nb * (uint32_t)GRID_BLOCK), a.sc,
                                                                      fs, a.os_b, a.os_l, a.B_dev
#ifdef LAE_GRID_FWD_LOOP_PROBE
                                                                      , 0u
#endif
                                                                      );
            if (nb < nb_safe)
                k_grid_fwd_lean_tail<<<nb_safe - nb, GRID_BLOCK, 0, a.stream>>>(a.inputs, (const half_t*)a.emb, a.offsets, (half_t*)a.out, a.B, a.sc, a.L,
                                                                                 a.os_b, a.os_l, a.B_dev, nb * (uint32_t)GRID_BLOCK);
            return;
        }
    }
    const bool xcd = (a.L % 8) == 0;
    k_grid_fwd<T, D, C><<<nb_safe * a.L, GRID_BLOCK, 0, a.stream>>>(a.inputs, (const T*)a.emb, a.offsets, (T*)a.out, a.B, a.L,
                                                                a.sc, (T*)a.dy_dx, a.gridtype, a.align, a.interp, nb_safe,
                                                                xcd, a.os_b, a.os_l, a.B_dev);
}
template <typename T, int D>
static int dispatch_fwd_c(const FwdArgs& a, uint32_t C) {
    switch (C) {
        case 1: launch_fwd<T, D, 1>(a); return LAE_OK;
        case 2: launch_fwd<T, D, 2>(a); return LAE_OK;
        case 4: launch_fwd<T, D, 4>(a); return LAE_OK;
        case 8: launch_fwd<T, D, 8>(a); return LAE_OK;
        default: return LAE_EINVAL;
    }
}
template <typename T>
static int dispatch_fwd_d(const FwdArgs& a, uint32_t D, uint32_t C) {
    switch (D) {
        case 2: return dispatch_fwd_c<T, 2>(a, C);
        case 3: return dispatch_fwd_c<T, 3>(a, C);
        case 4: return dispatch_fwd_c<T, 4>(a, C);
        case 5: return dispatch_fwd_c<T, 5>(a, C);
        default: return LAE_EINVAL;
    }
}

struct BwdArgs {
    const void* grad; const float* inputs; const int32_t* offsets; void* gemb; uint32_t B, L; LevelScales sc;
    uint32_t gridtype; bool align; uint32_t interp; uint64_t gs_b, gs_l; hipStream_t stream;
    const int32_t* offsets_host = nullptr;
    int32_t* nf_flag = nullptr;
    uint32_t* touched = nullptr;
    uint32_t* touched_full = nullptr;
};
template <typename T, int D, int C>
static void launch_bwd(const BwdArgs& a) {
    const uint32_t nb = lae::cdiv(a.B, GRID_BLOCK);
    const bool xcd = (a.L % 8) == 0;
    k_grid_bwd<T, D, C><<<nb * a.L, GRID_BLOCK, 0, a.stream>>>(a.grad ? (const T*)a.grad : nullptr, a.inputs, a.offsets,
                                                                (T*)a.gemb, a.B, a.L, a.sc, a.gridtype, a.align,
                                                                a.interp, nb, xcd, a.gs_b, a.gs_l, false);
}
template <typename T, int D>
static int dispatch_bwd_c(const BwdArgs& a, uint32_t C) {
    if constexpr (sizeof(T) == 2) {
        switch (C) {
            case 2: launch_bwd<T, D, 2>(a); return LAE_OK;
            case 4: launch_bwd<T, D, 4>(a); return LAE_OK;
            case 8: launch_bwd<T, D, 8>(a); return LAE_OK;
            default: return LAE_EINVAL;
        }
    } else {
        switch (C) {
            case 1: launch_bwd<T, D, 1>(a); return LAE_OK;
            case 2: launch_bwd<T, D, 2>(a); return LAE_OK;
            case 4: launch_bwd<T, D, 4>(a); return LAE_OK;
            case 8: launch_bwd<T, D, 8>(a); return LAE_OK;
            default: return LAE_EINVAL;
        }
    }
}
template <typename T>
static int dispatch_bwd_d(const BwdArgs& a, uint32_t D, uint32_t C) {
    switch (D) {
        case 2: return dispatch_bwd_c<T, 2>(a, C);
        case 3: return dispatch_bwd_c<T, 3>(a, C);
        case 4: return dispatch_bwd_c<T, 4>(a, C);
        case 5: return dispatch_bwd_c<T, 5>(a, C);
        default: return LAE_EINVAL;
    }
}

static int grid_forward(const float* inputs, const void* embeddings, const int32_t* offsets, void* outputs, uint32_t B,
                        uint32_t D, uint32_t C, uint32_t L, float S, uint32_t H, void* dy_dx, uint32_t gridtype,
                        int align_corners, uint32_t interp, int dtype, bool blc, void* stream, float in_shift = 0.0f,
                        float in_scale = 1.0f, const int32_t* offsets_host = nullptr) {
    if (B == 0) return LAE_OK;
    if (!inputs || !embeddings || !offsets || !outputs) return LAE_ENULL;
    if (gridtype > 1 || interp > 1) return LAE_EINVAL;
    FwdArgs a;
    a.offsets_host = offsets_host;
    a.inputs = inputs; a.emb = embeddings; a.offsets = offsets; a.out = outputs; a.B = B; a.L = L;
    int rc = fill_scales(a.sc, L, S, H);
    if (rc) return rc;
    a.sc.in_shift = in_shift; a.sc.in_scale = in_scale;
    a.dy_dx = dy_dx; a.gridtype = gridtype; a.align = align_corners != 0; a.interp = interp;
    a.stream = reinterpret_cast<hipStream_t>(stream);
    if (dtype != LAE_F32 && dtype != LAE_F16) return LAE_EINVAL;
    const bool staged = blc && C == 2 && L <= 32;
    void* lbc = nullptr;
    if (staged) {
        lbc = lae::workspace(lae::WS_GRID_OUT_T, (size_t)B * L * C * (dtype == LAE_F16 ? 2 : 4), a.stream);
        if (!lbc) return LAE_ELAUNCH;
        a.out = lbc;
    }
    const bool level_major = !blc || staged;
    a.os_b = level_major ? C : (uint64_t)L * C;
    a.os_l = level_major ? (uint64_t)B * C : C;
    if (dtype == LAE_F32) rc = dispatch_fwd_d<float>(a, D, C);
    else rc = dispatch_fwd_d<half_t>(a, D, C);
    if (rc) return rc;
    if (staged) {
        if (dtype == LAE_F16) k_out_transpose<half_t><<<lae::cdiv(B, 256), 256, 0, a.stream>>>((const half_t*)lbc, (half_t*)outputs, B, L);
        else k_out_transpose<float><<<lae::cdiv(B, 256), 256, 0, a.stream>>>((const float*)lbc, (float*)outputs, B, L);
    }
    return lae::check_launch("grid_encode_forward");
}

struct PlanLayout { size_t totals_off, offs_off, cnt_off, part_off, bytes; };
static inline uint32_t bwd_units(uint32_t B) { return lae::cdiv(B, UNIT_SAMPLES * SEGS) * SEGS; }
static inline PlanLayout plan_layout(uint32_t B, uint32_t L) {
    const size_t U = bwd_units(B);
    auto up = [](size_t v) { return (v + 255) / 256 * 256; };
    PlanLayout w;
// ... 15 lines not shown
    plan.part_cnt = reinterpret_cast<uint32_t*>(p + lay.part_off);
    return plan;
}
static inline size_t merge_bytes() { return ((size_t)MAX_LEVELS * SUB_RECS * sub_rec_words<half_t>() * 8 + 255) / 256 * 256; }
template <typename T>
static inline size_t bwd_exec_ws_bytes(uint32_t B, uint32_t L) {
    auto up = [](size_t v) { return (v + 255) / 256 * 256; };
    const size_t cap = (size_t)L * bwd_units(B) * UNIT_SAMPLES * 8;
    return merge_bytes() + up(cap * sizeof(typename BVal<T>::type)) + up(cap * 2);
}

template <typename T>
static void bwd_plan(const float* inputs, const int32_t* offsets, uint32_t B, uint32_t L, const BwdArgs& a, const BwdPlan& plan) {
    const uint32_t U = bwd_units(B);
    size_t line_lds = 0;
    if (a.touched) {
        uint32_t words = ((1u << 21) >> 3 >> 5) + 2;
        if (a.offsets_host) {
            words = 1;
            for (uint32_t l = 0; l < L; l++) {
                const uint32_t off = (uint32_t)a.offsets_host[l], size = (uint32_t)(a.offsets_host[l + 1] - a.offsets_host[l]);
                words = std::max(words, ((((off >> 3) & 31u) + ((size + 7u) >> 3) + 31u) >> 5));
            }
        }
        line_lds = (size_t)words * 4;
    }
    if (a.gridtype == 0 && !a.align && a.interp == 0)
        k_bwd_walk<T, false, true><<<U / SEGS * L, FILL_THREADS, line_lds, a.stream>>>(nullptr, inputs, offsets, B, L, a.sc, a.gridtype, a.align, a.interp, U, plan, nullptr, nullptr, a.touched, a.touched_full);
    else
        k_bwd_walk<T, false, false><<<U / SEGS * L, FILL_THREADS, line_lds, a.stream>>>(nullptr, inputs, offsets, B, L, a.sc, a.gridtype, a.align, a.interp, U, plan, nullptr, nullptr, a.touched, a.touched_full);
    k_bwd_scan_units<<<lae::cdiv((size_t)L * BK_MAX, 4), 256, 0, a.stream>>>(offsets, L, U, plan);
    k_bwd_scan_parts<<<1, 1024, 0, a.stream>>>(L * BK_MAX, plan);
}

template <typename T>
static int launch_bwd_fast(const void* gT, const float* inputs, const int32_t* offsets, void* gemb, uint32_t B, uint32_t L,
                           const BwdArgs& a, const void* caller_plan = nullptr) {
    using V = typename BVal<T>::type;
    auto up = [](size_t v) { return (v + 255) / 256 * 256; };
    const uint32_t U = bwd_units(B);
    const size_t plan_bytes = caller_plan ? 0 : plan_layout(B, L).bytes;
    uint8_t* ws = reinterpret_cast<uint8_t*>(lae::workspace(lae::WS_GRID_BINS, plan_bytes + bwd_exec_ws_bytes<T>(B, L), a.stream));
    if (!ws) return LAE_ELAUNCH;
    unsigned long long* partials = reinterpret_cast<unsigned long long*>(ws);
    {
        static std::mutex mtx;
        static std::vector<void*> zeroed;
        static uint64_t epoch = 0;
        std::lock_guard<std::mutex> lk(mtx);
        if (epoch != lae::workspace_epoch()) { zeroed.clear(); epoch = lae::workspace_epoch(); }
        if (std::find(zeroed.begin(), zeroed.end(), (void*)ws) == zeroed.end()) {
            if (hipMemsetAsync(ws, 0, merge_bytes(), a.stream) != hipSuccess) {
                (void)hipGetLastError();
                lae::set_last_error_str("grid backward: could not zero the merge records (first call inside a capture? warm up eagerly)");
                return LAE_ELAUNCH;
            }
            if (zeroed.size() > 64) zeroed.clear();
            zeroed.push_back((void*)ws);
        }
    }
    const BwdPlan plan = plan_at(caller_plan ? const_cast<void*>(caller_plan) : ws + merge_bytes(), B, L);
    uint8_t* ex = ws + merge_bytes() + plan_bytes;
    const size_t cap = (size_t)L * U * UNIT_SAMPLES * 8;
    V* qvals = reinterpret_cast<V*>(ex);
    uint16_t* qkeys = reinterpret_cast<uint16_t*>(ex + up(cap * sizeof(V)));
    const T* g = (const T*)gT;
    T* ge = (T*)gemb;
    if (!caller_plan) bwd_plan<T>(inputs, offsets, B, L, a, plan);
#ifdef LAE_GRID_BWD_PHASE_PROBE
    const char* phase_env = getenv("LAE_GRID_BWD_PHASE");
    const int phase_probe = phase_env ? atoi(phase_env) : 0;
    if (phase_probe != 2)
#endif
    if (a.gridtype == 0 && !a.align && a.interp == 0)
        k_bwd_walk<T, true, true><<<U / SEGS * L, FILL_THREADS, 0, a.stream>>>(g, inputs, offsets, B, L, a.sc, a.gridtype, a.align, a.interp, U, plan, qvals, qkeys, nullptr, nullptr);
    else
        k_bwd_walk<T, true, false><<<U / SEGS * L, FILL_THREADS, 0, a.stream>>>(g, inputs, offsets, B, L, a.sc, a.gridtype, a.align, a.interp, U, plan, qvals, qkeys, nullptr, nullptr);
#ifdef LAE_GRID_BWD_PHASE_PROBE
    if (phase_probe == 1) return lae::check_launch("grid backward (fill-only probe)");
#endif
    static const uint32_t bk_env = [] { const char* e = getenv("LAE_GRID_BWD_BK_TARGET"); return e ? (uint32_t)std::min(std::max(atoi(e), 1), (int)SUB_RECS) : 0u; }();
    static_assert(BK_TARGET <= SUB_RECS && 64u <= SUB_RECS, "bk_target choices must fit the merge records");
    const uint32_t bk_target = std::min(bk_env ? bk_env : (B >= 400000u ? 64u : BK_TARGET), SUB_RECS);
    k_bwd_acc<T><<<(uint32_t)lae::num_cus() * 2, ACC_THREADS, 0, a.stream>>>(offsets, ge, L, a.sc, a.gridtype, a.align, plan, qvals, qkeys, partials, a.nf_flag, bk_target);
    bool need_generic = true;
    if (a.offsets_host) {
        need_generic = false;
        for (uint32_t l = 0; l < L; l++)
            if (!level_is_binned((uint32_t)(a.offsets_host[l + 1] - a.offsets_host[l]))) need_generic = true;
    }
    if (need_generic) {
        const uint32_t nbg = lae::cdiv(B, GRID_BLOCK);
        k_grid_bwd<T, 3, 2><<<nbg * L, GRID_BLOCK, 0, a.stream>>>(g, inputs, offsets, ge, B, L, a.sc, a.gridtype, a.align, a.interp, nbg,
                                                                  (L % 8) == 0, 2, (uint64_t)B * 2, true);
    }
    return LAE_OK;
}

static inline size_t touched_words(const int32_t* offsets_host, uint32_t L) { return ((size_t)offsets_host[L] >> 3 >> 5) + 2; }

static int g_force_atomic_bwd = 0;

static int grid_backward(const void* grad, const float* inputs, const void* embeddings, const int32_t* offsets,
                         void* grad_embeddings, uint32_t B, uint32_t D, uint32_t C, uint32_t L, float S, uint32_t H,
                         const void* dy_dx, void* grad_inputs, uint32_t gridtype, int align_corners, uint32_t interp,
                         int dtype, bool blc, void* stream, float in_shift = 0.0f, float in_scale = 1.0f,
                         const int32_t* offsets_host = nullptr, const void* plan = nullptr, int32_t* nf_flag = nullptr,
                         uint32_t* touched = nullptr) {
    (void)embeddings;
    if (B == 0) return LAE_OK;
    if (!grad || !inputs || !offsets || !grad_embeddings) return LAE_ENULL;
    if (plan && !(D == 3 && C == 2 && L <= 32 && B <= BWD_MAX_SAMPLES && !blc && !g_force_atomic_bwd)) return LAE_EINVAL;
    if (gridtype > 1 || interp > 1) return LAE_EINVAL;
    if (touched && dtype != LAE_F16) return LAE_EINVAL;
    if (nf_flag || touched) {
        if (!(D == 3 && C == 2 && L <= 32 && B <= BWD_MAX_SAMPLES && !g_force_atomic_bwd) || !offsets_host) return LAE_EINVAL;
        for (uint32_t l = 0; l < L; l++)
            if (!level_is_binned((uint32_t)(offsets_host[l + 1] - offsets_host[l]))) return LAE_EINVAL;
    }
    BwdArgs a;
    a.offsets_host = offsets_host;
    a.nf_flag = nf_flag;
    a.touched = touched;
    if (touched) a.touched_full = touched + touched_words(offsets_host, L);
    a.grad = grad; a.inputs = inputs; a.offsets = offsets; a.gemb = grad_embeddings; a.B = B; a.L = L;
    int rc = fill_scales(a.sc, L, S, H);
    if (rc) return rc;
    a.sc.in_shift = in_shift; a.sc.in_scale = in_scale;
    a.gridtype = gridtype; a.align = align_corners != 0; a.interp = interp;
    a.gs_b = blc ? (uint64_t)L * C : C;
    a.gs_l = blc ? C : (uint64_t)B * C;
    a.stream = reinterpret_cast<hipStream_t>(stream);
    if (dtype != LAE_F32 && dtype != LAE_F16) return LAE_EINVAL;
    if (D == 3 && C == 2 && L <= 32 && B <= BWD_MAX_SAMPLES && !g_force_atomic_bwd) {
        const size_t esz = dtype == LAE_F16 ? 2 : 4;
        const void* gT = grad;
        if (blc) {
            void* ws = lae::workspace(lae::WS_GRID_GRAD_T, (size_t)B * L * 2 * esz, a.stream);
            if (!ws) return LAE_ELAUNCH;
            if (dtype == LAE_F16) k_grad_transpose<half_t><<<lae::cdiv(B, 256), 256, 0, a.stream>>>((const half_t*)grad, (half_t*)ws, B, L);
            else k_grad_transpose<float><<<lae::cdiv(B, 256), 256, 0, a.stream>>>((const float*)grad, (float*)ws, B, L);
            gT = ws;
        }
        rc = (dtype == LAE_F16) ? launch_bwd_fast<half_t>(gT, inputs, offsets, grad_embeddings, B, L, a, plan)
                                : launch_bwd_fast<float>(gT, inputs, offsets, grad_embeddings, B, L, a, plan);
        if (rc) return rc;
        rc = LAE_OK;
    } else if (dtype == LAE_F32) rc = dispatch_bwd_d<float>(a, D, C);
    else rc = dispatch_bwd_d<half_t>(a, D, C);
    if (rc) return rc;
    if (dy_dx && grad_inputs) {
        const uint32_t n = B * D;
        if (dtype == LAE_F32)
            k_grid_input_bwd<float><<<lae::cdiv(n, 256), 256, 0, a.stream>>>((const float*)grad, (const float*)dy_dx,
                                                                            (float*)grad_inputs, B, D, C, L, a.gs_b, a.gs_l);
        else
            k_grid_input_bwd<half_t><<<lae::cdiv(n, 256), 256, 0, a.stream>>>((const half_t*)grad, (const half_t*)dy_dx,
                                                                             (half_t*)grad_inputs, B, D, C, L, a.gs_b, a.gs_l);
    }
    return lae::check_launch("grid_encode_backward");
}

template <int D>
static int tv_c(const float* inputs, const float* emb, float* grad, const int32_t* offsets, float weight, uint32_t B,
                uint32_t C, uint32_t L, const LevelScales& sc, uint32_t gridtype, bool align, hipStream_t s) {
    const uint32_t nb = lae::cdiv(B, GRID_BLOCK);
    switch (C) {
        case 1: k_grad_tv<D, 1><<<nb * L, GRID_BLOCK, 0, s>>>(inputs, emb, grad, offsets, weight, B, L, sc, gridtype, align, nb); break;
        case 2: k_grad_tv<D, 2><<<nb * L, GRID_BLOCK, 0, s>>>(inputs, emb, grad, offsets, weight, B, L, sc, gridtype, align, nb); break;
        case 4: k_grad_tv<D, 4><<<nb * L, GRID_BLOCK, 0, s>>>(inputs, emb, grad, offsets, weight, B, L, sc, gridtype, align, nb); break;
        case 8: k_grad_tv<D, 8><<<nb * L, GRID_BLOCK, 0, s>>>(inputs, emb, grad, offsets, weight, B, L, sc, gridtype, align, nb); break;
        default: return LAE_EINVAL;
    }
    return LAE_OK;
}

}

int lae::grid_forward_frame(const float* inputs, const void* embeddings, const int32_t* offsets, void* outputs, uint32_t B_cap,
                            uint32_t B_launch, const uint32_t* B_dev, uint32_t L, float S, uint32_t H, uint32_t gridtype,
                            int align_corners, uint32_t interp, float in_shift, float in_scale, hipStream_t stream,
                            const int32_t* offsets_host, uint32_t B_likely) {
    if (B_launch == 0) return LAE_OK;
    FwdArgs a;
    a.offsets_host = offsets_host;
    a.inputs = inputs; a.emb = embeddings; a.offsets = offsets; a.out = outputs; a.B = B_cap; a.L = L;
    int rc = fill_scales(a.sc, L, S, H);
    if (rc) return rc;
    a.sc.in_shift = in_shift; a.sc.in_scale = in_scale;
    a.dy_dx = nullptr; a.gridtype = gridtype; a.align = align_corners != 0; a.interp = interp;
    a.stream = stream; a.os_b = 2; a.os_l = (uint64_t)B_cap * 2;
    a.B_dev = B_dev; a.B_launch = std::min(B_launch, B_cap); a.B_likely = std::min(B_likely, a.B_launch);
    launch_fwd<half_t, 3, 2>(a);
    return LAE_OK;
}

extern "C" {

int lae_grid_encode_forward(const float* inputs, const void* embeddings, const int32_t* offsets, void* outputs,
                            uint32_t B, uint32_t D, uint32_t C, uint32_t L, float S, uint32_t H, void* dy_dx,
                            uint32_t gridtype, int align_corners, uint32_t interp, int dtype, void* stream) {
    return grid_forward(inputs, embeddings, offsets, outputs, B, D, C, L, S, H, dy_dx, gridtype, align_corners, interp,
                        dtype, false, stream);
}
int lae_grid_encode_backward(const void* grad, const float* inputs, const void* embeddings, const int32_t* offsets,
                             void* grad_embeddings, uint32_t B, uint32_t D, uint32_t C, uint32_t L, float S, uint32_t H,
                             const void* dy_dx, void* grad_inputs, uint32_t gridtype, int align_corners,
                             uint32_t interp, int dtype, void* stream) {
    return grid_backward(grad, inputs, embeddings, offsets, grad_embeddings, B, D, C, L, S, H, dy_dx, grad_inputs,
                         gridtype, align_corners, interp, dtype, false, stream);
}

int lae_grid_encode_forward_ex(const float* inputs, const void* embeddings, const int32_t* offsets, void* outputs,
                               uint32_t B, uint32_t D, uint32_t C, uint32_t L, float S, uint32_t H, void* dy_dx,
                               uint32_t gridtype, int align_corners, uint32_t interp, int dtype, int blc, float in_shift,
                               float in_scale, const int32_t* offsets_host, void* stream) {
    return grid_forward(inputs, embeddings, offsets, outputs, B, D, C, L, S, H, dy_dx, gridtype, align_corners, interp,
                        dtype, blc != 0, stream, in_shift, in_scale, offsets_host);
}
int lae_grid_encode_backward_ex(const void* grad, const float* inputs, const void* embeddings, const int32_t* offsets,
                                void* grad_embeddings, uint32_t B, uint32_t D, uint32_t C, uint32_t L, float S,
                                uint32_t H, const void* dy_dx, void* grad_inputs, uint32_t gridtype,
                                int align_corners, uint32_t interp, int dtype, int blc, float in_shift, float in_scale,
                                const int32_t* offsets_host, int32_t* nonfinite_flag, uint32_t* touched_lines, void* stream) {
    return grid_backward(grad, inputs, embeddings, offsets, grad_embeddings, B, D, C, L, S, H, dy_dx, grad_inputs,
                         gridtype, align_corners, interp, dtype, blc != 0, stream, in_shift, in_scale, offsets_host, nullptr,
                         nonfinite_flag, touched_lines);
}

uint64_t lae_grid_backward_workspace_bytes(uint32_t B, uint32_t L, int dtype) {
    return plan_layout(B, L).bytes + (dtype == LAE_F16 ? bwd_exec_ws_bytes<half_t>(B, L) : bwd_exec_ws_bytes<float>(B, L));
}

uint64_t lae_grid_backward_plan_bytes(uint32_t B, uint32_t L) { return plan_layout(B, L).bytes; }

uint64_t lae_grid_touched_lines_words(uint64_t n_entries) { return (n_entries >> 3 >> 5) + 2 + MAX_LEVELS; }

int lae_grid_encode_backward_plan(const float* inputs, const int32_t* offsets, uint32_t B, uint32_t D, uint32_t C, uint32_t L, float S,
                                  uint32_t H, uint32_t gridtype, int align_corners, uint32_t interp, int dtype, float in_shift,
                                  float in_scale, const int32_t* offsets_host, void* plan, uint32_t* touched_lines, void* stream) {
    if (B == 0) return LAE_OK;
    if (!inputs || !offsets || !plan) return LAE_ENULL;
    if (D != 3 || C != 2 || L > 32 || B > BWD_MAX_SAMPLES || gridtype > 1 || interp > 1 || (dtype != LAE_F32 && dtype != LAE_F16)) return LAE_EINVAL;
    if (touched_lines) {
        if (!offsets_host || dtype != LAE_F16 || g_force_atomic_bwd) return LAE_EINVAL;
        for (uint32_t l = 0; l < L; l++)
            if (!level_is_binned((uint32_t)(offsets_host[l + 1] - offsets_host[l]))) return LAE_EINVAL;
    }
    BwdArgs a;
    a.offsets_host = offsets_host;
    a.touched = touched_lines;
    if (touched_lines) a.touched_full = touched_lines + touched_words(offsets_host, L);
    a.grad = nullptr; a.inputs = inputs; a.offsets = offsets; a.gemb = nullptr; a.B = B; a.L = L;
    int rc = fill_scales(a.sc, L, S, H);
    if (rc) return rc;
    a.sc.in_shift = in_shift; a.sc.in_scale = in_scale;
    a.gridtype = gridtype; a.align = align_corners != 0; a.interp = interp;
    a.gs_b = C; a.gs_l = (uint64_t)B * C;
    a.stream = reinterpret_cast<hipStream_t>(stream);
    if (dtype == LAE_F16) bwd_plan<half_t>(inputs, offsets, B, L, a, plan_at(plan, B, L));
    else bwd_plan<float>(inputs, offsets, B, L, a, plan_at(plan, B, L));
    return lae::check_launch("grid_encode_backward_plan");
}

int lae_grid_encode_backward_planned(const void* grad, const float* inputs, const int32_t* offsets, void* grad_embeddings, uint32_t B,
                                     uint32_t D, uint32_t C, uint32_t L, float S, uint32_t H, uint32_t gridtype, int align_corners,
                                     uint32_t interp, int dtype, float in_shift, float in_scale, const int32_t* offsets_host,
                                     const void* plan, int32_t* nonfinite_flag, void* stream) {
    if (!plan) return LAE_ENULL;
    return grid_backward(grad, inputs, nullptr, offsets, grad_embeddings, B, D, C, L, S, H, nullptr, nullptr, gridtype, align_corners,
                         interp, dtype, false, stream, in_shift, in_scale, offsets_host, plan, nonfinite_flag, nullptr);
}

int lae_grid_forward_schedule(const int32_t* offsets_host, uint32_t L, float S, uint32_t H, uint32_t n_chunks, uint32_t* nseg_out,
                              uint32_t* segs_out) {
    if (!offsets_host || !nseg_out || !segs_out) return LAE_ENULL;
    LevelScales sc;
    if (fill_scales(sc, L, S, H) != LAE_OK || L > 8 * FWD_MAX_SEG) return LAE_EINVAL;
    FwdSched fs;
    const uint32_t per_xcd = fwd_sched_build(fs, L, n_chunks, sc, offsets_host);
    for (int x = 0; x < 8; x++) {
        nseg_out[x] = fs.nseg[x];
        for (uint32_t q = 0; q < fs.nseg[x]; q++) {
            uint32_t* o = segs_out + ((size_t)x * FWD_MAX_SEG + q) * 3;
            o[0] = fs.seg[x][q].level; o[1] = fs.seg[x][q].c0; o[2] = fs.seg[x][q].n;
        }
    }
    return (int)per_xcd;
}

int lae_grid_set_forward_mode(int mode) {
    if (mode < 0 || mode > 2) return LAE_EINVAL;
    g_fwd_mode = mode;
    return LAE_OK;
}

int lae_grid_set_backward_mode(int mode) {
    if (mode != 0 && mode != 1) return LAE_EINVAL;
    g_force_atomic_bwd = mode;
    return LAE_OK;
}

int lae_grad_total_variation(const void* inputs, const void* embeddings, void* grad, const int32_t* offsets,
                             float weight, uint32_t B, uint32_t D, uint32_t C, uint32_t L, float S, uint32_t H,
                             uint32_t gridtype, int align_corners, int dtype, void* stream) {
    if (B == 0) return LAE_OK;
    if (!inputs || !embeddings || !grad || !offsets) return LAE_ENULL;
    if (dtype != LAE_F32 || gridtype > 1) return LAE_EINVAL;
    LevelScales sc;
    int rc = fill_scales(sc, L, S, H);
    if (rc) return rc;
    hipStream_t s = reinterpret_cast<hipStream_t>(stream);
    const bool al = align_corners != 0;
    const float* in = (const float*)inputs; const float* e = (const float*)embeddings; float* g = (float*)grad;
    switch (D) {
        case 2: rc = tv_c<2>(in, e, g, offsets, weight, B, C, L, sc, gridtype, al, s); break;
        case 3: rc = tv_c<3>(in, e, g, offsets, weight, B, C, L, sc, gridtype, al, s); break;
        case 4: rc = tv_c<4>(in, e, g, offsets, weight, B, C, L, sc, gridtype, al, s); break;
        case 5: rc = tv_c<5>(in, e, g, offsets, weight, B, C, L, sc, gridtype, al, s); break;
        default: rc = LAE_EINVAL;
    }
    if (rc) return rc;
    return lae::check_launch("grad_total_variation");
}

}

#ifdef LAE_GRID_STAMPS
extern "C" __attribute__((visibility("default"))) int lae_debug_grid_stamps(void* out, size_t bytes) {
    if (hipDeviceSynchronize() != hipSuccess) return 1;
    return hipMemcpyFromSymbol(out, HIP_SYMBOL(g_grid_stamps), bytes) == hipSuccess ? 0 : 1;
}
#endif
```

### laenerf_amd/csrc/optimizer.hip

```cpp
#include "lae_common.h"
#include <hip/hip_fp16.h>

#define STREAM(s) reinterpret_cast<hipStream_t>(s)

namespace {

typedef _Float16 half_t;

struct OptState {
    float scale;
    int32_t growth_tracker;
    int32_t found_inf;
    int32_t skip;
    int32_t step;
    float inv_bc1;
    float bc2_sqrt;
    float inv_scale;
    int32_t skipped_total;
    float next_inv_bc1;
    float next_bc2_sqrt;
    int32_t next_for;
    float next_beta1;
    float next_beta2;
    int32_t pad[2];
};

__device__ __forceinline__ void bias_corrections(float beta1, float beta2, int step, float& inv_bc1, float& bc2_sqrt) {
    inv_bc1 = (float)(1.0 / (1.0 - pow((double)beta1, (double)step)));
    bc2_sqrt = (float)sqrt(1.0 - pow((double)beta2, (double)step));
}
__device__ __forceinline__ void prepare_next_step(OptState* st, float beta1, float beta2) {
    const int nxt = st->step + 1;
    float a, b;
    bias_corrections(beta1, beta2, nxt, a, b);
    st->next_inv_bc1 = a; st->next_bc2_sqrt = b; st->next_beta1 = beta1; st->next_beta2 = beta2;
    st->next_for = nxt;
}

template <typename G> __device__ __forceinline__ float ldg(const G* g, size_t i) { return (float)g[i]; }

template <typename G>
__global__ __launch_bounds__(256) void k_check(const G* __restrict__ grad, size_t n, OptState* __restrict__ st) {
    bool bad = false;
    const size_t stride = (size_t)gridDim.x * blockDim.x * 8;
    for (size_t i = ((size_t)blockIdx.x * blockDim.x + threadIdx.x) * 8; i < n; i += stride) {
        if (i + 8 <= n) {
            if constexpr (sizeof(G) == 2) {
                const uint4 v = *reinterpret_cast<const uint4*>(grad + i);
                const uint32_t w[4] = {v.x, v.y, v.z, v.w};
#pragma unroll
                for (int k = 0; k < 4; k++) bad |= ((w[k] & 0x7c00u) == 0x7c00u) || ((w[k] & 0x7c000000u) == 0x7c000000u);
            } else {
                const float4 a = *reinterpret_cast<const float4*>(grad + i), b = *reinterpret_cast<const float4*>(grad + i + 4);
                bad |= !isfinite(a.x) || !isfinite(a.y) || !isfinite(a.z) || !isfinite(a.w) || !isfinite(b.x) || !isfinite(b.y) ||
                       !isfinite(b.z) || !isfinite(b.w);
            }
        } else {
            for (size_t j = i; j < n; j++) bad |= !isfinite(ldg(grad, j));
        }
    }
    if (__any(bad) && (threadIdx.x & 63) == 0) atomicOr(&st->found_inf, 1);
}

__global__ void k_begin(OptState* __restrict__ st, float beta1, float beta2, int growth_interval, float growth, float backoff,
                        int use_scaler) {
    if (threadIdx.x != 0 || blockIdx.x != 0) return;
    const bool bad = use_scaler && st->found_inf != 0;
    st->found_inf = 0;
    st->skip = bad;
    st->inv_scale = use_scaler ? (float)(1.0 / (double)st->scale) : 1.0f;
    if (bad) {
        st->scale = st->scale * backoff;
        st->growth_tracker = 0;
        st->skipped_total += 1;
        return;
    }
    st->step += 1;
    if (st->next_for == st->step && st->next_beta1 == beta1 && st->next_beta2 == beta2) {
        st->inv_bc1 = st->next_inv_bc1; st->bc2_sqrt = st->next_bc2_sqrt;
    } else {
        float a, b;
        bias_corrections(beta1, beta2, st->step, a, b);
        st->inv_bc1 = a; st->bc2_sqrt = b;
    }
    if (use_scaler) {
        st->growth_tracker += 1;
        if (st->growth_tracker == growth_interval) { st->scale = st->scale * growth; st->growth_tracker = 0; }
    }
}

struct AdamHyper { float beta1, beta2, eps, weight_decay; };

__device__ __forceinline__ void adam1(float& p, float& m, float& v, float g, float lr_over_bc1, float bc2_sqrt, const AdamHyper& h) {
    if (h.weight_decay != 0.0f) g = g + h.weight_decay * p;
    m = m + (g - m) * (1.0f - h.beta1);
    v = v * h.beta2 + (1.0f - h.beta2) * (g * g);
    const float denom = sqrtf(v) / bc2_sqrt + h.eps;
    p = p - lr_over_bc1 * (m / denom);
}

template <typename G>
__global__ __launch_bounds__(256) void k_apply(float* __restrict__ p, float* __restrict__ m, float* __restrict__ v,
                                               G* __restrict__ grad, half_t* __restrict__ shadow, size_t n,
                                               OptState* __restrict__ st, const float* __restrict__ lr_ptr, AdamHyper h) {
    const bool skip = st->skip != 0;
    const float inv_scale = st->inv_scale, bc2_sqrt = st->bc2_sqrt;
    const float lr_over_bc1 = (float)((double)lr_ptr[0] * (double)st->inv_bc1);
    if (blockIdx.x == 0 && threadIdx.x == 0) prepare_next_step(st, h.beta1, h.beta2);
    const size_t stride = (size_t)gridDim.x * blockDim.x * 4;
    for (size_t i = ((size_t)blockIdx.x * blockDim.x + threadIdx.x) * 4; i < n; i += stride) {
        if (i + 4 <= n) {
            float g[4];
            if constexpr (sizeof(G) == 2) {
                const uint2 raw = *reinterpret_cast<const uint2*>(grad + i);
                const half_t* gh = reinterpret_cast<const half_t*>(&raw);
#pragma unroll
                for (int k = 0; k < 4; k++) g[k] = (float)gh[k];
                *reinterpret_cast<uint2*>(grad + i) = uint2{0u, 0u};
            } else {
                const float4 raw = *reinterpret_cast<const float4*>(grad + i);
                g[0] = raw.x; g[1] = raw.y; g[2] = raw.z; g[3] = raw.w;
                *reinterpret_cast<float4*>(grad + i) = float4{0, 0, 0, 0};
            }
            if (skip) continue;
            float4 pp = *reinterpret_cast<const float4*>(p + i), mm = *reinterpret_cast<const float4*>(m + i),
                   vv = *reinterpret_cast<const float4*>(v + i);
            adam1(pp.x, mm.x, vv.x, g[0] * inv_scale, lr_over_bc1, bc2_sqrt, h);
            adam1(pp.y, mm.y, vv.y, g[1] * inv_scale, lr_over_bc1, bc2_sqrt, h);
            adam1(pp.z, mm.z, vv.z, g[2] * inv_scale, lr_over_bc1, bc2_sqrt, h);
            adam1(pp.w, mm.w, vv.w, g[3] * inv_scale, lr_over_bc1, bc2_sqrt, h);
            *reinterpret_cast<float4*>(p + i) = pp;
            *reinterpret_cast<float4*>(m + i) = mm;
            *reinterpret_cast<float4*>(v + i) = vv;
            if (shadow) {
                half_t s[4] = {(half_t)pp.x, (half_t)pp.y, (half_t)pp.z, (half_t)pp.w};
                *reinterpret_cast<uint2*>(shadow + i) = *reinterpret_cast<const uint2*>(s);
            }
        } else {
            for (size_t j = i; j < n; j++) {
                const float gj = ldg(grad, j) * inv_scale;
                grad[j] = (G)0.0f;
                if (skip) continue;
                float pj = p[j], mj = m[j], vj = v[j];
                adam1(pj, mj, vj, gj, lr_over_bc1, bc2_sqrt, h);
                p[j] = pj; m[j] = mj; v[j] = vj;
                if (shadow) shadow[j] = (half_t)pj;
            }
        }
    }
}

constexpr int MAX_SEGS = 8;
struct CheckSegs { const void* grad[MAX_SEGS]; size_t n[MAX_SEGS]; int is_half[MAX_SEGS]; int count; };
struct ApplySegs {
    float* p[MAX_SEGS]; float* m[MAX_SEGS]; float* v[MAX_SEGS]; void* grad[MAX_SEGS]; half_t* shadow[MAX_SEGS];
    const float* lr[MAX_SEGS]; size_t n[MAX_SEGS]; int is_half[MAX_SEGS]; int count;
    const uint32_t* touched[MAX_SEGS];
};

template <typename G>
__device__ __forceinline__ bool seg_has_nonfinite(const G* __restrict__ grad, size_t n) {
    bool bad = false;
    const size_t stride = (size_t)gridDim.x * blockDim.x * 8;
    for (size_t i = ((size_t)blockIdx.x * blockDim.x + threadIdx.x) * 8; i < n; i += stride) {
        if (i + 8 <= n) {
            if constexpr (sizeof(G) == 2) {
                const uint4 v = *reinterpret_cast<const uint4*>(grad + i);
                const uint32_t w[4] = {v.x, v.y, v.z, v.w};
#pragma unroll
                for (int k = 0; k < 4; k++) bad |= ((w[k] & 0x7c00u) == 0x7c00u) || ((w[k] & 0x7c000000u) == 0x7c000000u);
            } else {
                const float4 a = *reinterpret_cast<const float4*>(grad + i), b = *reinterpret_cast<const float4*>(grad + i + 4);
                bad |= !isfinite(a.x) || !isfinite(a.y) || !isfinite(a.z) || !isfinite(a.w) || !isfinite(b.x) || !isfinite(b.y) ||
                       !isfinite(b.z) || !isfinite(b.w);
            }
        } else {
            for (size_t j = i; j < n; j++) bad |= !isfinite(ldg(grad, j));
        }
    }
    return bad;
}

__global__ __launch_bounds__(256) void k_check_multi(CheckSegs sg, OptState* __restrict__ st) {
    bool bad = false;
    for (int s = 0; s < sg.count; s++)
        bad |= sg.is_half[s] ? seg_has_nonfinite((const half_t*)sg.grad[s], sg.n[s]) : seg_has_nonfinite((const float*)sg.grad[s], sg.n[s]);
    if (__any(bad) && (threadIdx.x & 63) == 0) atomicOr(&st->found_inf, 1);
}

template <typename G>
__device__ __forceinline__ void seg_apply(float* __restrict__ p, float* __restrict__ m, float* __restrict__ v, G* __restrict__ grad,
                                          half_t* __restrict__ shadow, size_t n, bool skip, float inv_scale, float bc2_sqrt,
                                          float lr_over_bc1, const AdamHyper& h, const uint32_t* __restrict__ touched = nullptr) {
    const size_t stride = (size_t)gridDim.x * blockDim.x * 4;
    for (size_t i = ((size_t)blockIdx.x * blockDim.x + threadIdx.x) * 4; i < n; i += stride) {
        if (touched) {
            const size_t line = i >> 4;
            if (!((touched[line >> 5] >> (line & 31)) & 1u)) continue;
        }
        if (i + 4 <= n) {
            float g[4];
            if constexpr (sizeof(G) == 2) {
                const uint2 raw = *reinterpret_cast<const uint2*>(grad + i);
                const half_t* gh = reinterpret_cast<const half_t*>(&raw);
#pragma unroll
                for (int k = 0; k < 4; k++) g[k] = (float)gh[k];
                *reinterpret_cast<uint2*>(grad + i) = uint2{0u, 0u};
            } else {
                const float4 raw = *reinterpret_cast<const float4*>(grad + i);
                g[0] = raw.x; g[1] = raw.y; g[2] = raw.z; g[3] = raw.w;
                *reinterpret_cast<float4*>(grad + i) = float4{0, 0, 0, 0};
            }
            if (skip) continue;
            float4 pp = *reinterpret_cast<const float4*>(p + i), mm = *reinterpret_cast<const float4*>(m + i),
                   vv = *reinterpret_cast<const float4*>(v + i);
            adam1(pp.x, mm.x, vv.x, g[0] * inv_scale, lr_over_bc1, bc2_sqrt, h);
            adam1(pp.y, mm.y, vv.y, g[1] * inv_scale, lr_over_bc1, bc2_sqrt, h);
            adam1(pp.z, mm.z, vv.z, g[2] * inv_scale, lr_over_bc1, bc2_sqrt, h);
            adam1(pp.w, mm.w, vv.w, g[3] * inv_scale, lr_over_bc1, bc2_sqrt, h);
            *reinterpret_cast<float4*>(p + i) = pp;
            *reinterpret_cast<float4*>(m + i) = mm;
            *reinterpret_cast<float4*>(v + i) = vv;
            if (shadow) {
                half_t s[4] = {(half_t)pp.x, (half_t)pp.y, (half_t)pp.z, (half_t)pp.w};
                *reinterpret_cast<uint2*>(shadow + i) = *reinterpret_cast<const uint2*>(s);
            }
        } else {
            for (size_t j = i; j < n; j++) {
                const float gj = ldg(grad, j) * inv_scale;
                grad[j] = (G)0.0f;
                if (skip) continue;
                float pj = p[j], mj = m[j], vj = v[j];
                adam1(pj, mj, vj, gj, lr_over_bc1, bc2_sqrt, h);
                p[j] = pj; m[j] = mj; v[j] = vj;
                if (shadow) shadow[j] = (half_t)pj;
            }
        }
    }
}

__global__ __launch_bounds__(256) void k_apply_multi(ApplySegs sg, OptState* __restrict__ st, AdamHyper h) {
    const bool skip = st->skip != 0;
    const float inv_scale = st->inv_scale, bc2_sqrt = st->bc2_sqrt;
    if (blockIdx.x == gridDim.x - 1 && threadIdx.x == 0) prepare_next_step(st, h.beta1, h.beta2);
    for (int s = 0; s < sg.count; s++) {
        const float lr_over_bc1 = (float)((double)sg.lr[s][0] * (double)st->inv_bc1);
        if (sg.is_half[s]) seg_apply(sg.p[s], sg.m[s], sg.v[s], (half_t*)sg.grad[s], sg.shadow[s], sg.n[s], skip, inv_scale, bc2_sqrt, lr_over_bc1, h, sg.touched[s]);
        else seg_apply(sg.p[s], sg.m[s], sg.v[s], (float*)sg.grad[s], sg.shadow[s], sg.n[s], skip, inv_scale, bc2_sqrt, lr_over_bc1, h, sg.touched[s]);
    }
}

struct EmaSegs { float* shadow[MAX_SEGS]; const float* param[MAX_SEGS]; size_t n[MAX_SEGS]; int count; };
__global__ __launch_bounds__(256) void k_ema_multi(EmaSegs sg, float one_minus_decay) {
    const size_t stride = (size_t)gridDim.x * 256 * 4;
    for (int s = 0; s < sg.count; s++) {
        float* __restrict__ sh = sg.shadow[s];
        const float* __restrict__ p = sg.param[s];
        const size_t n = sg.n[s], n4 = n & ~(size_t)3;
        for (size_t i = ((size_t)blockIdx.x * 256 + threadIdx.x) * 4; i < n4; i += stride) {
            float4 a = *reinterpret_cast<const float4*>(sh + i);
            const float4 b = *reinterpret_cast<const float4*>(p + i);
            a.x -= (a.x - b.x) * one_minus_decay; a.y -= (a.y - b.y) * one_minus_decay;
            a.z -= (a.z - b.z) * one_minus_decay; a.w -= (a.w - b.w) * one_minus_decay;
            *reinterpret_cast<float4*>(sh + i) = a;
        }
        if (blockIdx.x == 0 && threadIdx.x < n - n4) { const size_t j = n4 + threadIdx.x; sh[j] -= (sh[j] - p[j]) * one_minus_decay; }
    }
}

uint32_t stream_blocks(size_t n, int per_thread) {
    const size_t want = (n + 256ull * per_thread - 1) / (256ull * per_thread);
    return (uint32_t)std::max<size_t>(1, std::min<size_t>(want, (size_t)lae::num_cus() * 16));
}

}

extern "C" {

int lae_adam_check(const void* grad, int grad_is_half, uint64_t n, void* state, void* stream) {
    if (n == 0) return LAE_OK;
    if (!grad || !state) return LAE_ENULL;
    if ((reinterpret_cast<uintptr_t>(grad) & 15) != 0) return LAE_EINVAL;
    OptState* st = reinterpret_cast<OptState*>(state);
    if (grad_is_half) k_check<half_t><<<stream_blocks(n, 8), 256, 0, STREAM(stream)>>>((const half_t*)grad, n, st);
    else k_check<float><<<stream_blocks(n, 8), 256, 0, STREAM(stream)>>>((const float*)grad, n, st);
    return lae::check_launch("adam_check");
}

int lae_adam_check_multi(uint32_t n_tensors, const void* const* grads, const int* grad_is_half, const uint64_t* sizes, void* state,
                         void* stream) {
    if (n_tensors == 0) return LAE_OK;
    if (!grads || !grad_is_half || !sizes || !state) return LAE_ENULL;
    if (n_tensors > (uint32_t)MAX_SEGS) return LAE_EINVAL;
    CheckSegs sg{};
    size_t biggest = 0;
    for (uint32_t i = 0; i < n_tensors; i++) {
        if (sizes[i] && !grads[i]) return LAE_ENULL;
        if (reinterpret_cast<uintptr_t>(grads[i]) & 15) return LAE_EINVAL;
        sg.grad[i] = grads[i]; sg.n[i] = sizes[i]; sg.is_half[i] = grad_is_half[i];
        biggest = std::max(biggest, (size_t)sizes[i]);
    }
    sg.count = (int)n_tensors;
    k_check_multi<<<stream_blocks(biggest, 8), 256, 0, STREAM(stream)>>>(sg, reinterpret_cast<OptState*>(state));
    return lae::check_launch("adam_check_multi");
}

int lae_ema_update_multi(uint32_t n_tensors, float* const* shadows, const float* const* params, const uint64_t* sizes, float one_minus_decay,
                         void* stream) {
    if (n_tensors == 0) return LAE_OK;
    if (!shadows || !params || !sizes) return LAE_ENULL;
    if (n_tensors > (uint32_t)MAX_SEGS) return LAE_EINVAL;
    EmaSegs sg{};
    size_t biggest = 0;
    for (uint32_t i = 0; i < n_tensors; i++) {
        if (sizes[i] && (!shadows[i] || !params[i])) return LAE_ENULL;
        if ((reinterpret_cast<uintptr_t>(shadows[i]) | reinterpret_cast<uintptr_t>(params[i])) & 15) return LAE_EINVAL;
        sg.shadow[i] = shadows[i]; sg.param[i] = params[i]; sg.n[i] = sizes[i];
        biggest = std::max(biggest, (size_t)sizes[i]);
    }
    sg.count = (int)n_tensors;
    k_ema_multi<<<stream_blocks(biggest, 4), 256, 0, STREAM(stream)>>>(sg, one_minus_decay);
    return lae::check_launch("ema_update_multi");
}

int lae_adam_apply_multi(uint32_t n_tensors, float* const* params, float* const* exp_avgs, float* const* exp_avg_sqs, void* const* grads,
                         const int* grad_is_half, void* const* shadows_half, const uint64_t* sizes, const float* const* lrs,
                         const void* const* touched_lines, const void* state, float beta1, float beta2, float eps, float weight_decay,
                         void* stream) {
    if (n_tensors == 0) return LAE_OK;
    if (!params || !exp_avgs || !exp_avg_sqs || !grads || !grad_is_half || !shadows_half || !sizes || !lrs || !state) return LAE_ENULL;
    if (n_tensors > (uint32_t)MAX_SEGS) return LAE_EINVAL;
    ApplySegs sg{};
    size_t biggest = 0;
    for (uint32_t i = 0; i < n_tensors; i++) {
        if (sizes[i] && (!params[i] || !exp_avgs[i] || !exp_avg_sqs[i] || !grads[i] || !lrs[i])) return LAE_ENULL;
        const uintptr_t al = reinterpret_cast<uintptr_t>(params[i]) | reinterpret_cast<uintptr_t>(exp_avgs[i]) |
                             reinterpret_cast<uintptr_t>(exp_avg_sqs[i]) | reinterpret_cast<uintptr_t>(grads[i]) |
                             reinterpret_cast<uintptr_t>(shadows_half[i]);
        if (al & 15) return LAE_EINVAL;
        sg.p[i] = params[i]; sg.m[i] = exp_avgs[i]; sg.v[i] = exp_avg_sqs[i]; sg.grad[i] = grads[i];
        sg.shadow[i] = (half_t*)shadows_half[i]; sg.lr[i] = lrs[i]; sg.n[i] = sizes[i]; sg.is_half[i] = grad_is_half[i];
        sg.touched[i] = (touched_lines && weight_decay == 0.0f) ? (const uint32_t*)touched_lines[i] : nullptr;
        biggest = std::max(biggest, (size_t)sizes[i]);
    }
    sg.count = (int)n_tensors;
    k_apply_multi<<<stream_blocks(biggest, 4), 256, 0, STREAM(stream)>>>(sg, reinterpret_cast<OptState*>(const_cast<void*>(state)),
                                                                        AdamHyper{beta1, beta2, eps, weight_decay});
    return lae::check_launch("adam_apply_multi");
}

int lae_adam_begin(void* state, float beta1, float beta2, int growth_interval, float growth_factor, float backoff_factor,
                   int use_scaler, void* stream) {
    if (!state) return LAE_ENULL;
    k_begin<<<1, 64, 0, STREAM(stream)>>>(reinterpret_cast<OptState*>(state), beta1, beta2, growth_interval, growth_factor,
                                          backoff_factor, use_scaler);
    return lae::check_launch("adam_begin");
}

int lae_adam_apply(float* param, float* exp_avg, float* exp_avg_sq, void* grad, int grad_is_half, void* shadow_half, uint64_t n,
                   const void* state, const float* lr, float beta1, float beta2, float eps, float weight_decay, void* stream) {
    if (n == 0) return LAE_OK;
    if (!param || !exp_avg || !exp_avg_sq || !grad || !state || !lr) return LAE_ENULL;
    const uintptr_t al = reinterpret_cast<uintptr_t>(param) | reinterpret_cast<uintptr_t>(exp_avg) | reinterpret_cast<uintptr_t>(exp_avg_sq) |
                         reinterpret_cast<uintptr_t>(grad) | reinterpret_cast<uintptr_t>(shadow_half);
    if (al & 15) return LAE_EINVAL;
    const AdamHyper h{beta1, beta2, eps, weight_decay};
    OptState* st = reinterpret_cast<OptState*>(const_cast<void*>(state));
    if (grad_is_half)
        k_apply<half_t><<<stream_blocks(n, 4), 256, 0, STREAM(stream)>>>(param, exp_avg, exp_avg_sq, (half_t*)grad, (half_t*)shadow_half, n, st, lr, h);
    else
        k_apply<float><<<stream_blocks(n, 4), 256, 0, STREAM(stream)>>>(param, exp_avg, exp_avg_sq, (float*)grad, (half_t*)shadow_half, n, st, lr, h);
    return lae::check_launch("adam_apply");
}

}
```

### laenerf_amd/dist.py

```python
import os

import torch
import torch.distributed as dist

TILE = 128
RS_AG_MIN_ELEMS = 1 << 20
FORCE_COLLECTIVES = os.environ.get("LAE_DIST_FORCE_COLLECTIVES") == "1"


def _exchange(world_size):
    return world_size > 1 or (FORCE_COLLECTIVES and dist.is_available() and dist.is_initialized())


def shard_indices(n_rays, rank, world_size, tile=TILE):
    n_tiles = (n_rays + tile - 1) // tile
    tiles_per_rank = (n_tiles + world_size - 1) // world_size
    t = torch.arange(tiles_per_rank) * world_size + rank
    idx = (t[:, None] * tile + torch.arange(tile)[None, :]).reshape(-1)
    idx[idx >= n_rays] = -1
    return idx


_shard_cache = {}

# ... 107 lines not shown


@torch.no_grad()
def broadcast_model_state(module, src=0, group=None):
    if not dist.is_available() or not dist.is_initialized() or not _exchange(dist.get_world_size(group)):
        return module
    tensors = list(module.parameters()) + [b for b in module.buffers()]
    attrs = [getattr(module, n) for n in ("density_bitfield", "density_grid") if isinstance(getattr(module, n, None), torch.Tensor)]
    seen, uniq = set(), []
    for t in tensors + attrs:
        if t.data_ptr() not in seen and t.numel():
            seen.add(t.data_ptr()); uniq.append(t)
    by_dtype = {}
    for t in uniq:
        by_dtype.setdefault((t.dtype, t.device), []).append(t)
    for (dtype, dev), ts in by_dtype.items():
        flat = torch.cat([t.reshape(-1) for t in ts])
        rehearsal = flat.is_cuda and dist.get_backend(group) == "gloo"
        buf = flat.cpu() if rehearsal else flat
        dist.broadcast(buf, src=src, group=group)
        if rehearsal:
            flat = buf.to(dev)
        off = 0
        for t in ts:
            t.copy_(flat[off:off + t.numel()].view_as(t)); off += t.numel()
    for m in module.modules():
        sh = getattr(m, "shadow", None)
        if sh is not None and hasattr(sh, "half"):
            p = getattr(m, "embeddings", None) if hasattr(m, "embeddings") else getattr(m, "weights", None)
            if p is not None:
                sh.half.copy_(p.detach()); sh.version = p._version
    return module


def allreduce_mean_(tensors, world_size=None, group=None, bucket_bytes=64 << 20):
    world_size = dist.get_world_size(group) if world_size is None else world_size
    if not _exchange(world_size):
        return tensors
    by_dtype = {}
    for t in tensors:
        by_dtype.setdefault((t.dtype, t.device), []).append(t)
    for (dtype, dev), ts in by_dtype.items():
        bucket, size = [], 0
        buckets = []
        for t in ts:
            nbytes = t.numel() * t.element_size()
            if t.numel() >= RS_AG_MIN_ELEMS and t.is_contiguous():
                buckets.append([t])
                continue
            if bucket and size + nbytes > bucket_bytes:
                buckets.append(bucket); bucket, size = [], 0
            bucket.append(t); size += nbytes
        if bucket:
            buckets.append(bucket)
        for b in buckets:
            flat = torch.cat([t.reshape(-1) for t in b]) if len(b) > 1 else b[0].reshape(-1)
            flat.mul_(1.0 / world_size)
            backend = dist.get_backend(group)
            rehearsal = flat.is_cuda and backend == "gloo"
            if backend == "nccl" and flat.numel() >= RS_AG_MIN_ELEMS:
                pad = (-flat.numel()) % world_size
                work = torch.cat([flat, flat.new_zeros(pad)]) if pad else flat
                shard = torch.empty(work.numel() // world_size, dtype=work.dtype, device=work.device)
                dist.reduce_scatter_tensor(shard, work, op=dist.ReduceOp.SUM, group=group)
                dist.all_gather_into_tensor(work, shard, group=group)
                if pad:
                    flat.copy_(work[:flat.numel()])
            else:
                buf = flat.cpu() if rehearsal else flat
                dist.all_reduce(buf, op=dist.ReduceOp.SUM, group=group)
                if rehearsal:
                    flat.copy_(buf)
            if len(b) > 1:
                off = 0
                for t in b:
                    t.copy_(flat[off:off + t.numel()].view_as(t)); off += t.numel()
    return tensors


def allreduce_gradients(optimizer, world_size=None, group=None):
    grads = []
    for p, _, _, shadow, _ in optimizer.items:
        if shadow is not None:
            if p.grad is not None:
                shadow.grad_half.add_(p.grad.to(torch.half)); p.grad = None
            if hasattr(shadow, "unreported"):
                shadow.unreported = True
                shadow.mark_all_touched()
            grads.append(getattr(shadow, "grad_store", shadow.grad_half))
        elif p.grad is not None:
            grads.append(p.grad)
    return allreduce_mean_(grads, world_size, group)
```

### laenerf_amd/editing/style_encoder.py

```python
import torch
import torch.nn as nn
from torch.autograd import Function
from torch.amp import custom_bwd, custom_fwd

from ..backend import style_backend as _backend
from ..encoding import get_encoder
from ..ffmlp import FFMLP


class _palette_recompose(Function):
    @staticmethod
    @custom_fwd(device_type="cuda")
    def forward(ctx, w_logits, o_raw, palette, active_mask):
        M = w_logits.shape[0]
        w_logits, o_raw = w_logits.half().contiguous(), o_raw.half().contiguous()
        palette = palette.float().contiguous()
        P = palette.shape[0]
        n_active = bin(active_mask & ((1 << P) - 1)).count("1")
        dev = w_logits.device
        pred = torch.empty(M, 3, dtype=torch.half, device=dev)
        w_hat = torch.empty(M, n_active, dtype=torch.float32, device=dev)
        o_hat = torch.empty(M, 3, dtype=torch.half, device=dev)
        _backend.palette_forward(w_logits, o_raw, palette, P, active_mask, M, pred, w_hat, o_hat)
        ctx.save_for_backward(w_logits, o_raw, palette)
# ... 31 lines not shown
        w_hat = torch.empty(M, n_active, dtype=torch.float32, device=dev)
        o_hat = torch.empty(M, 3, dtype=torch.half, device=dev)
        _backend.palette_forward(w_logits, o_raw, palette, P, active_mask, M, pred, w_hat, o_hat)
        fin = torch.empty(12, dtype=torch.float32, device=dev)
        _backend.style_loss_forward(pred, target, w_hat, o_hat, M, n_active, lw, scale, fin,
                                    reg_palette=palette if reg_w is not None else None, reg_w=reg_w or (0.0, 0.0), m_dev=m_dev)
        ctx.save_for_backward(w_logits, o_raw, palette, target, fin)
        ctx.meta = (P, active_mask, M, lw, reg_w)
        ctx.m_dev = m_dev
        ctx.palette_param = palette_in if getattr(palette_in, "_lae_persistent_grad", False) and palette_in is palette else None
        ctx.mark_non_differentiable(pred, w_hat, o_hat, fin)
        ctx.set_materialize_grads(False)
        return fin[0], pred, w_hat, o_hat, fin

    @staticmethod
    @custom_bwd(device_type="cuda")
    def backward(ctx, g_loss, *_):
        if g_loss is None:
            return (None,) * 9
        w_logits, o_raw, palette, target, fin = ctx.saved_tensors
        P, active_mask, M, lw, reg_w = ctx.meta
        g_wl, g_ol = torch.empty_like(w_logits), torch.empty_like(o_raw)
        owner = ctx.palette_param
        from ..optim import _direct_grad
        direct = owner is not None and _direct_grad["depth"] > 0 and owner.grad is not None and owner.grad.dtype == torch.float32 \
            and owner.grad.is_contiguous() and owner.grad.shape == palette.shape and not owner._backward_hooks \
            and not getattr(owner, "_post_accumulate_grad_hooks", None)
        g_pal = owner.grad if direct else torch.empty_like(palette)
        _backend.style_loss_backward(w_logits, o_raw, palette, P, active_mask, M, target, fin, g_loss.float().reshape(1).contiguous(), lw,
                                     g_wl, g_ol, g_pal, reg_w=reg_w, accumulate=direct, m_dev=ctx.m_dev)
        return g_wl, g_ol, (None if direct else g_pal), None, None, None, None, None, None


def palette_recompose(w_logits, o_raw, palette, active_mask):
    return _palette_recompose.apply(w_logits, o_raw, palette, int(active_mask))


class _style_features(Function):

    @staticmethod
    @custom_fwd(device_type="cuda")
    def forward(ctx, x, d, embeddings, enc, bound, degree, off_cols, plan=None):
        import numpy as np
        from ..backend import gridencoder_backend as _grid
        M = x.shape[0]
        Mp = (M + 15) // 16 * 16
        L = enc.num_levels
        x = x.float().contiguous()
        table = enc.shadow.table_half(embeddings) if enc.shadow is not None else embeddings.to(torch.half)
        in_map = (float(bound), float(np.float32(1.0) / np.float32(2 * bound)))
        S, H = np.log2(enc.per_level_scale), enc.base_resolution
        feats = torch.empty(L, M, 2, device=x.device, dtype=torch.half)
        _grid.grid_encode_forward(x, table, enc.offsets, feats, M, 3, 2, L, S, H, None, enc.gridtype_id, enc.align_corners,
                                  enc.interp_id, blc=False, in_map=in_map, offsets_host=enc.offsets_host)
        feat = torch.empty(Mp, 32, device=x.device, dtype=torch.half)
        off_in = torch.empty(Mp, off_cols, device=x.device, dtype=torch.half) if degree else None
        _backend.style_assemble_forward(feats, d.float().contiguous() if degree else None, M, Mp, degree, feat, off_in, off_cols)
        ctx.save_for_backward(x, table)
        ctx.enc, ctx.in_map, ctx.geom, ctx.off_cols, ctx.plan = enc, in_map, (M, L, S, H), off_cols, plan
        return (feat, off_in) if degree else (feat, feat)

    @staticmethod
    @custom_bwd(device_type="cuda")
    def backward(ctx, g_feat, g_off):
        from ..backend import gridencoder_backend as _grid
        x, table = ctx.saved_tensors
        enc = ctx.enc
        M, L, S, H = ctx.geom
        if g_feat is None and g_off is None:
            return (None,) * 8
        g_feat = None if g_feat is None else g_feat.to(torch.half).contiguous()
        g_off = None if g_off is None else g_off.to(torch.half).contiguous()
        off_cols = ctx.off_cols if g_off is not None and g_off.shape[1] != 32 else 32
        grad_feats = torch.empty(L, M, 2, device=x.device, dtype=torch.half)
        _backend.style_assemble_backward(g_feat, g_off, M, off_cols, grad_feats)
        grad_table = enc.shadow.grad_half if enc.shadow is not None else torch.zeros_like(table)
        flag = enc.shadow.flag_for_backward(M) if enc.shadow is not None else None
        touched = enc.shadow.touched_for_backward(M) if flag is not None else None
        if ctx.plan is not None and touched is not None and not getattr(ctx.plan, "marks_touched", False):
            touched = None
        if enc.shadow is not None and touched is None:
            enc.shadow.unreported = enc.shadow.unreported or flag is None
            enc.shadow.mark_all_touched()
        _grid.grid_encode_backward(grad_feats, x, table, enc.offsets, grad_table, M, 3, 2, L, S, H, None, None, enc.gridtype_id,
                                   enc.align_corners, enc.interp_id, blc=False, in_map=ctx.in_map, offsets_host=enc.offsets_host,
                                   plan=ctx.plan, nonfinite_flag=flag, touched_lines=touched)
        return None, None, (None if enc.shadow is not None else grad_table), None, None, None, None, None


class LAENeRF(nn.Module):

    def __init__(self, params, encoding="hashgrid", dir_encoding=None, num_layers=3, hidden_dim=64, color_palette=None, size=256,
                 style_img=None):
        super().__init__()
        self.opt = params
        self.bound = params.bound
        self.encoder, self.in_dim = get_encoder(encoding, desired_resolution=2048 * self.bound, num_levels=16, log2_hashmap_size=19)
        self.num_layers = num_layers
        self.hidden_dim = hidden_dim
        self.num_color_bases = params.num_palette_bases
        if not 0 < self.num_color_bases <= 16:
            raise ValueError("LAENeRF: 1..16 palette bases (the MLP output tile is 16 wide)")
        if getattr(params, "style_weight", 0) > 0:
            raise NotImplementedError("LAENeRF: the VGG style network is outside the MI355X hot path (SURVEY.md 2.1)")
        self.register_buffer("active_palets", torch.ones(self.num_color_bases, dtype=torch.bool))
        self._active_mask = (1 << self.num_color_bases) - 1
        pal = color_palette if color_palette is not None else torch.rand(self.num_color_bases, 3, dtype=torch.float32)
        self.color_palette = nn.Parameter(pal.detach().clone().float())
        self.original_color_palette = None
        self.size = size
        self.dir_encoding, self.in_dim_dir = None, 0
        if dir_encoding is not None:
            self.dir_encoding, self.in_dim_dir = get_encoder(dir_encoding, degree=3)
        self.offset_in_dim = (self.in_dim + self.in_dim_dir + 15) // 16 * 16
        self.offset_net = FFMLP(self.offset_in_dim, 3, hidden_dim, num_layers - 1)
        self.weight_net = FFMLP(self.in_dim, self.num_color_bases, hidden_dim, num_layers - 1)

    def plan_backward(self, x):
        from ..field import field_backward_plan
        if not (self.fused_inputs and x.is_cuda and x.dim() == 2 and self._encoder_fits()):
            return None
        return field_backward_plan(x, self.encoder, self.bound)

    def _encoder_fits(self):
        from ..gridencoder import GridEncoder
        enc = self.encoder
        return isinstance(enc, GridEncoder) and enc.num_levels == 16 and enc.level_dim == 2 and enc.input_dim == 3

    def _logits(self, x, d, plan=None):
        M = x.shape[0]
        fused = self._fused_inputs_ok(x, d)
        if plan is not None and not fused:
            raise RuntimeError("LAENeRF: a backward plan needs the one-node input path (half-precision hash grid under autocast)")
        if fused:
            deg = self.dir_encoding.degree if self.dir_encoding is not None else 0
            feat, off_in = _style_features.apply(x, d if deg else None, self.encoder.embeddings, self.encoder, self.bound, deg, self.offset_in_dim,
                                                 plan)
            wn, on = self.weight_net, self.offset_net
            from ..ffmlp.ffmlp import ffmlp_forward
            w_logits = ffmlp_forward(feat, wn.weights, wn.input_dim, 16, wn.hidden_dim, wn.num_layers, wn.activation, wn.output_activation,
                                     not self.training, True, wn.shadow if self.ffmlp_shadows else None)
            o_raw = ffmlp_forward(off_in, on.weights, on.input_dim, 16, on.hidden_dim, on.num_layers, on.activation, on.output_activation,
                                  not self.training, True, on.shadow if self.ffmlp_shadows else None)
            return w_logits, o_raw, M
        pad = (16 - M % 16) % 16
        feat = self.encoder(x, bound=self.bound)
        if pad:
            feat = torch.cat([feat, feat.new_zeros(pad, feat.shape[1])], 0)
        wn, on = self.weight_net, self.offset_net
        from ..ffmlp.ffmlp import ffmlp_forward
        w_logits = ffmlp_forward(feat, wn.weights, wn.input_dim, 16, wn.hidden_dim, wn.num_layers, wn.activation, wn.output_activation,
                                 not self.training, feat.requires_grad, wn.shadow if self.ffmlp_shadows else None)
        cols = [feat]
        if self.dir_encoding is not None:
            enc_d = self.dir_encoding(d).to(feat.dtype)
            if pad:
                enc_d = torch.cat([enc_d, enc_d.new_zeros(pad, enc_d.shape[1])], 0)
            cols.append(enc_d)
        width = sum(c.shape[1] for c in cols)
        if width < self.offset_in_dim:
            cols.append(feat.new_zeros(feat.shape[0], self.offset_in_dim - width))
        off_in = torch.cat(cols, -1) if len(cols) > 1 else feat
        o_raw = ffmlp_forward(off_in, on.weights, on.input_dim, 16, on.hidden_dim, on.num_layers, on.activation, on.output_activation,
                              not self.training, off_in.requires_grad, on.shadow if self.ffmlp_shadows else None)
        return w_logits, o_raw, M

    fused_inputs = True
    ffmlp_shadows = True

# ... 91 lines not shown
```

### laenerf_amd/field.py

```python
import numpy as np
import torch
from torch.autograd import Function
from torch.amp import custom_bwd, custom_fwd

from .backend import ffmlp_backend as _mlp
from .backend import gridencoder_backend as _grid
from .ffmlp.head import COLOR_NET_PARAMS, SIGMA_NET_PARAMS


class _nerf_field(Function):
    calls = 0

    @staticmethod
    @custom_fwd(device_type="cuda")
    def forward(ctx, x, dirs, embeddings, sigma_weights, color_weights, enc, sigma_shadow, color_shadow, bound, density_scale, plan=None):
        _nerf_field.calls += 1
        M = x.shape[0]
        L = enc.num_levels
        x = x.float().contiguous()
        dirs = dirs.float().contiguous()
        table = enc.shadow.table_half(embeddings) if enc.shadow is not None else embeddings.to(torch.half)
        shadows = (sigma_shadow, color_shadow) if sigma_shadow is not None and color_shadow is not None else None
        if shadows is not None:
            ws, wc = sigma_shadow.table_half(sigma_weights), color_shadow.table_half(color_weights)
        else:
            ws, wc = sigma_weights.half().contiguous(), color_weights.half().contiguous()
        in_map = (float(bound), float(np.float32(1.0) / np.float32(2 * bound)))
        S, H = np.log2(enc.per_level_scale), enc.base_resolution
        feats = torch.empty(L, M, 2, device=x.device, dtype=torch.half)
        _grid.grid_encode_forward(x, table, enc.offsets, feats, M, 3, 2, L, S, H, None, enc.gridtype_id, enc.align_corners,
                                  enc.interp_id, blc=False, in_map=in_map, offsets_host=enc.offsets_host)
        h = torch.empty(M, 16, device=x.device, dtype=torch.half)
        sigmas = torch.empty(M, device=x.device, dtype=torch.float32)
        rgbs = torch.empty(M, 3, device=x.device, dtype=torch.float32)
        _mlp.nerf_head_forward(feats, dirs, ws, wc, M, density_scale, h, sigmas, rgbs, level_major=True)
        ctx.save_for_backward(x, dirs, table, ws, wc, feats, h, rgbs)
        ctx.enc, ctx.shadows, ctx.in_map, ctx.geom = enc, shadows, in_map, (M, L, S, H)
        ctx.density_scale = density_scale
        ctx.plan = plan
        ctx.wdtypes = (sigma_weights.dtype, color_weights.dtype)
        return sigmas, rgbs

    @staticmethod
    @custom_bwd(device_type="cuda")
    def backward(ctx, grad_sigmas, grad_rgbs):
        x, dirs, table, ws, wc, feats, h, rgbs = ctx.saved_tensors
        enc = ctx.enc
        M, L, S, H = ctx.geom
        grad_sigmas = grad_sigmas.float().contiguous()
        grad_rgbs = grad_rgbs.float().contiguous()
        grad_h = torch.empty_like(h)
        grad_feats = torch.empty_like(feats)
        wflag = None
        if ctx.shadows is not None:
            gws, gwc = ctx.shadows[0].grad_half, ctx.shadows[1].grad_half
            wflag = _weights_flag(ctx.shadows)
        else:
            gws, gwc = torch.empty_like(ws), torch.empty_like(wc)
        _mlp.nerf_head_backward(grad_sigmas, grad_rgbs, feats, dirs, h, rgbs, ws, wc, M, ctx.density_scale, grad_h, grad_feats,
                                gws, gwc, accumulate=ctx.shadows is not None, level_major=True, nonfinite_flag=wflag)
        grad_table = enc.shadow.grad_half if enc.shadow is not None else torch.zeros_like(table)
        flag = enc.shadow.flag_for_backward(M) if enc.shadow is not None else None
        touched = enc.shadow.touched_for_backward(M) if flag is not None else None
        if ctx.plan is not None and touched is not None and not getattr(ctx.plan, "marks_touched", False):
            touched = None
        if enc.shadow is not None and touched is None:
            enc.shadow.mark_all_touched()
        _grid.grid_encode_backward(grad_feats, x, table, enc.offsets, grad_table, M, 3, 2, L, S, H, None, None, enc.gridtype_id,
                                   enc.align_corners, enc.interp_id, blc=False, in_map=ctx.in_map, offsets_host=enc.offsets_host, plan=ctx.plan,
                                   nonfinite_flag=flag, touched_lines=touched)
        return (None, None, None if enc.shadow is not None else grad_table,
                None if ctx.shadows is not None else gws.to(ctx.wdtypes[0]),
                None if ctx.shadows is not None else gwc.to(ctx.wdtypes[1]), None, None, None, None, None, None)


def _weights_flag(shadows):
    a, b = shadows[0].flag_for_backward(), shadows[1].flag_for_backward()
    if a is not None and a == b:
        return a
    shadows[0].unreported = shadows[1].unreported = True
    return None


def field_supported(enc, sigma_net, color_net):
    return (enc.input_dim == 3 and enc.level_dim == 2 and enc.num_levels == 16
            and sigma_net.weights.numel() == SIGMA_NET_PARAMS and color_net.weights.numel() == COLOR_NET_PARAMS)


def nerf_field(x, dirs, enc, sigma_net, color_net, bound=1, density_scale=1.0, plan=None):
    if x.shape[0] % 16 != 0:
        raise RuntimeError("nerf_field: the number of samples must be a multiple of 16")
    return _nerf_field.apply(x, dirs, enc.embeddings, sigma_net.weights, color_net.weights, enc, sigma_net.shadow,
                             color_net.shadow, float(bound), float(density_scale), plan)


@torch.no_grad()
def field_backward_plan(x, enc, bound=1):
    x = x.float().contiguous()
    if x.shape[0] > (1 << 24):
        return None
    in_map = (float(bound), float(np.float32(1.0) / np.float32(2 * bound)))
    touched = enc.shadow.touched_for_backward(x.shape[0]) if enc.shadow is not None else None
    return _grid.grid_backward_plan(x, enc.offsets, x.shape[0], 3, 2, enc.num_levels, np.log2(enc.per_level_scale), enc.base_resolution,
                                    enc.gridtype_id, enc.align_corners, enc.interp_id, True, in_map, offsets_host=enc.offsets_host,
                                    touched_lines=touched)


@torch.no_grad()
def field_density(x, enc, sigma_net, bound=1, density_scale=1.0):
    M = x.shape[0]
    Mp = (M + 15) // 16 * 16
    x = x.float().contiguous()
    if Mp != M:
        x = torch.cat([x, x.new_zeros(Mp - M, 3)], dim=0)
    table = enc.shadow.table_half(enc.embeddings) if enc.shadow is not None else enc.embeddings.detach().to(torch.half)
    ws = sigma_net.shadow.table_half(sigma_net.weights) if sigma_net.shadow is not None else sigma_net.weights.detach().half().contiguous()
    in_map = (float(bound), float(np.float32(1.0) / np.float32(2 * bound)))
    L = enc.num_levels
    feats = torch.empty(L, Mp, 2, device=x.device, dtype=torch.half)
    _grid.grid_encode_forward(x, table, enc.offsets, feats, Mp, 3, 2, L, np.log2(enc.per_level_scale), enc.base_resolution, None,
                              enc.gridtype_id, enc.align_corners, enc.interp_id, blc=False, in_map=in_map, offsets_host=enc.offsets_host)
    sigmas = torch.empty(Mp, device=x.device, dtype=torch.float32)
    _mlp.nerf_density_forward(feats, ws, Mp, density_scale, None, sigmas, level_major=True)
    return sigmas[:M]
```

### laenerf_amd/gridencoder/grid.py

```python
import numpy as np
import torch
import torch.nn as nn
from torch.autograd import Function
from torch.amp import custom_bwd, custom_fwd

from ..backend import gridencoder_backend as _backend

_gridtype_to_id = {"hash": 0, "tiled": 1}
_interp_to_id = {"linear": 0, "smoothstep": 1}


class _grid_encode(Function):

    @staticmethod
    @custom_fwd(device_type="cuda")
    def forward(ctx, inputs, embeddings, offsets, per_level_scale, base_resolution, calc_grad_inputs=False, gridtype=0,
                align_corners=False, interpolation=0, shadow=None, in_map=(0.0, 1.0), offsets_host=None):
        inputs = inputs.contiguous()
        B, D = inputs.shape
        L = offsets.shape[0] - 1
        C = embeddings.shape[1]
        S = np.log2(per_level_scale)
        H = base_resolution
        ctx.shadow = None
        if torch.is_autocast_enabled("cuda") and C % 2 == 0:
            if shadow is not None:
                embeddings = shadow.table_half(embeddings)
                ctx.shadow = shadow
            else:
                embeddings = embeddings.to(torch.half)
        outputs = torch.empty(B, L * C, device=inputs.device, dtype=embeddings.dtype)
        dy_dx = torch.empty(B, L * D * C, device=inputs.device, dtype=embeddings.dtype) if calc_grad_inputs else None
        _backend.grid_encode_forward(inputs, embeddings, offsets, outputs, B, D, C, L, S, H, dy_dx, gridtype,
                                     align_corners, interpolation, blc=True, in_map=in_map, offsets_host=offsets_host)
        ctx.offsets_host = offsets_host
        ctx.save_for_backward(inputs, embeddings, offsets, dy_dx)
        ctx.dims = [B, D, C, L, S, H, gridtype, interpolation]
        ctx.in_map = in_map
        ctx.align_corners = align_corners
        return outputs

    @staticmethod
    @custom_bwd(device_type="cuda")
    def backward(ctx, grad):
        inputs, embeddings, offsets, dy_dx = ctx.saved_tensors
        B, D, C, L, S, H, gridtype, interpolation = ctx.dims
        grad = grad.contiguous()
        if grad.dtype != embeddings.dtype:
            grad = grad.to(embeddings.dtype)
        grad_embeddings = ctx.shadow.grad_half if ctx.shadow is not None else torch.zeros_like(embeddings)
        grad_inputs = torch.zeros_like(inputs, dtype=embeddings.dtype) if dy_dx is not None else None
        flag = ctx.shadow.flag_for_backward(B) if ctx.shadow is not None and D == 3 and C == 2 else None
        touched = ctx.shadow.touched_for_backward(B) if flag is not None and grad.dtype == torch.half else None
        if ctx.shadow is not None and (flag is None or touched is None):
            ctx.shadow.unreported = ctx.shadow.unreported or flag is None
            ctx.shadow.mark_all_touched()
        _backend.grid_encode_backward(grad, inputs, embeddings, offsets, grad_embeddings, B, D, C, L, S, H, dy_dx,
                                      grad_inputs, gridtype, ctx.align_corners, interpolation, blc=True, in_map=ctx.in_map,
                                      offsets_host=ctx.offsets_host, nonfinite_flag=flag, touched_lines=touched)
        if dy_dx is not None:
            grad_inputs = grad_inputs.to(inputs.dtype)
            if ctx.in_map[1] != 1.0:
                grad_inputs = grad_inputs * ctx.in_map[1]
        return (grad_inputs, (None if ctx.shadow is not None else grad_embeddings), None, None, None, None, None, None, None,
                None, None, None)


class TableShadow:

    def __init__(self, embeddings):
        self.half = embeddings.detach().to(torch.half).contiguous()
        n = self.half.numel()
        self.grad_store = torch.zeros((n + 839) // 840 * 840, dtype=torch.half, device=self.half.device)
        self.grad_half = self.grad_store[:n].view_as(self.half)
        self.version = embeddings._version
        self.nonfinite_flag = None
        self.unreported = False
        self.touched_lines = None

    def mark_all_touched(self):
        if self.touched_lines is not None:
            self.touched_lines.fill_(-1)

    def flag_for_backward(self, n_samples=0):
        if self.nonfinite_flag is None or n_samples > (1 << 24):
            self.unreported = True
            self.mark_all_touched()
            return None
        return self.nonfinite_flag

    def touched_for_backward(self, n_samples=0):
        if self.touched_lines is None or self.nonfinite_flag is None or n_samples > (1 << 24):
            return None
        return self.touched_lines.data_ptr()

    def table_half(self, embeddings):
        if embeddings._version != self.version:
            self.half.copy_(embeddings.detach())
            self.version = embeddings._version
        return self.half


grid_encode = _grid_encode.apply


def level_offsets(input_dim, num_levels, per_level_scale, base_resolution, log2_hashmap_size, align_corners):
    offsets, offset = [], 0
    max_params = 2 ** log2_hashmap_size
    for i in range(num_levels):
        resolution = int(np.ceil(base_resolution * per_level_scale ** i))
        n = min(max_params, (resolution if align_corners else resolution + 1) ** input_dim)
        n = int(np.ceil(n / 8) * 8)
        offsets.append(offset)
        offset += n
    offsets.append(offset)
    return np.array(offsets, dtype=np.int32)


class GridEncoder(nn.Module):

    def __init__(self, input_dim=3, num_levels=16, level_dim=2, per_level_scale=2, base_resolution=16,
                 log2_hashmap_size=19, desired_resolution=None, gridtype="hash", align_corners=False,
                 interpolation="linear"):
        super().__init__()
        if desired_resolution is not None:
            per_level_scale = np.exp2(np.log2(desired_resolution / base_resolution) / (num_levels - 1))
        self.input_dim = input_dim
        self.num_levels = num_levels
        self.level_dim = level_dim
        self.per_level_scale = per_level_scale
        self.log2_hashmap_size = log2_hashmap_size
        self.base_resolution = base_resolution
        self.output_dim = num_levels * level_dim
        self.gridtype = gridtype
        self.gridtype_id = _gridtype_to_id[gridtype]
        self.interpolation = interpolation
        self.interp_id = _interp_to_id[interpolation]
        self.align_corners = align_corners
        self.max_params = 2 ** log2_hashmap_size

        offsets = level_offsets(input_dim, num_levels, per_level_scale, base_resolution, log2_hashmap_size, align_corners)
        self.register_buffer("offsets", torch.from_numpy(offsets))
        self.offsets_host = offsets.copy()
        self.n_params = int(offsets[-1]) * level_dim
        self.embeddings = nn.Parameter(torch.empty(int(offsets[-1]), level_dim))
        self.shadow = None
        self.reset_parameters()

    def reset_parameters(self):
        self.embeddings.data.uniform_(-1e-4, 1e-4)

    def __repr__(self):
        return (f"GridEncoder: input_dim={self.input_dim} num_levels={self.num_levels} level_dim={self.level_dim} "
                f"resolution={self.base_resolution} -> "
                f"{int(round(self.base_resolution * self.per_level_scale ** (self.num_levels - 1)))} "
                f"per_level_scale={self.per_level_scale:.4f} params={tuple(self.embeddings.shape)} "
                f"gridtype={self.gridtype} align_corners={self.align_corners} interpolation={self.interpolation}")

    def forward(self, inputs, bound=1):
        prefix_shape = list(inputs.shape[:-1])
        inputs = inputs.view(-1, self.input_dim)
# ... 29 lines not shown
```

### laenerf_amd/optim.py

```python
import ctypes
import os

import torch

from . import _lib
from .ffmlp import FFMLP
from .gridencoder import GridEncoder


_direct_grad = {"depth": 0}


class FusedAdam(torch.optim.Optimizer):
    def __init__(self, model, lr=1e-2, betas=(0.9, 0.99), eps=1e-15, weight_decay=0.0, param_groups=None,
                 grad_scaler=True, init_scale=2.0 ** 16, growth_factor=2.0, backoff_factor=0.5, growth_interval=2000, device_lr=False):
        groups = param_groups if param_groups is not None else [{"params": [p for p in model.parameters() if p.requires_grad], "lr": lr}]
        groups = [{**g, "params": [p for p in g["params"] if p.requires_grad]} for g in groups]
        super().__init__(groups, dict(lr=lr, betas=tuple(betas), eps=eps, weight_decay=weight_decay))
        self.betas, self.eps, self.weight_decay = betas, eps, weight_decay
        self.use_scaler = bool(grad_scaler)
        self.growth_factor, self.backoff_factor, self.growth_interval = growth_factor, backoff_factor, growth_interval
        tables = {id(m.embeddings): m for m in model.modules() if isinstance(m, GridEncoder) and m.level_dim % 2 == 0}
        tables.update({id(m.weights): m for m in model.modules() if isinstance(m, FFMLP)})
        self.items = []
        dev = None
        for gi, g in enumerate(self.param_groups):
            for p in g["params"]:
                if not p.is_cuda or p.dtype != torch.float32 or not p.is_contiguous():
                    raise RuntimeError("FusedAdam: parameters must be contiguous fp32 tensors on the GPU (no CPU fallback)")
                dev = p.device
                shadow = None
                owner = tables.get(id(p))
                if owner is not None:
                    shadow = owner.attach_shadow()
                else:
                    p.grad = torch.zeros_like(p)
                    p._lae_persistent_grad = True
                m, v = torch.zeros_like(p), torch.zeros_like(p)
                self.state[p] = {"step": torch.tensor(0.0), "exp_avg": m, "exp_avg_sq": v}
                self.items.append((p, m, v, shadow, gi))
        if dev is None:
            raise ValueError("FusedAdam: no parameter to optimise")
        self.dev_state = torch.zeros(16, dtype=torch.int32, device=dev)
        if self.use_scaler:
            for p, _, _, shadow, _ in self.items:
                owner = tables.get(id(p))
                if shadow is not None and isinstance(owner, GridEncoder) and owner.input_dim == 3 and owner.level_dim == 2 \
                        and owner.num_levels <= 32 and int((owner.offsets_host[1:] - owner.offsets_host[:-1]).max()) <= (1 << 21):
                    shadow.nonfinite_flag = self.dev_state.data_ptr() + 8
                    if weight_decay == 0 and not os.environ.get("LAE_ADAM_NO_TOUCHED_LINES"):
                        n_words = int(_lib.load().lae_grid_touched_lines_words(p.shape[0]))
                        shadow.touched_lines = torch.zeros(n_words, dtype=torch.int32, device=p.device)
                elif shadow is not None and isinstance(owner, FFMLP):
                    shadow.nonfinite_flag = self.dev_state.data_ptr() + 8
        self._scale_view = self.dev_state.view(torch.float32)
        self._scale_view[0] = init_scale if self.use_scaler else 1.0
        self.device_lr = bool(device_lr)
        self._lr_host = [float(g["lr"]) for g in self.param_groups]
        self.lrs = torch.tensor(self._lr_host, dtype=torch.float32, device=dev)
        if len(self.items) > 8:
            raise RuntimeError("FusedAdam: at most 8 parameter tensors (one multi-tensor launch)")
        self._args = None

    def scale(self, loss):
        return loss * self._scale_view[0] if self.use_scaler else loss

    def backward(self, loss):
        key = (tuple(loss.shape), loss.dtype, str(loss.device))
        cache = self.__dict__.setdefault("_root_grads", {})
        one = cache.get(key)
        if one is None:
            one = cache[key] = torch.ones(loss.shape, dtype=loss.dtype, device=loss.device)
            from .raymarching.raymarching import register_unit_root_grad
            register_unit_root_grad(one)
        _direct_grad["depth"] += 1
        try:
            loss.backward(gradient=one)
        finally:
            _direct_grad["depth"] -= 1
        self.finish_loss()

    @staticmethod
    def finish_loss():
        from .backend import flush_pending_loss
        flush_pending_loss()

    def get_scale(self):
        return float(self._scale_view[0].item())

    @property
    def steps_taken(self):
        return int(self.dev_state[4].item())

    @property
    def steps_skipped(self):
        return int(self.dev_state[8].item())

    def set_lr(self, lr, group=None):
        for gi, g in enumerate(self.param_groups):
            if group is None or gi == group:
                g["lr"] = float(lr)
        self.sync_lr()

    def sync_lr(self):
        if self.device_lr:
            return
        cur = [float(g["lr"]) for g in self.param_groups]
        if cur != self._lr_host:
            if torch.cuda.is_current_stream_capturing():
                raise RuntimeError("FusedAdam: a learning rate changed inside a stream capture; call sync_lr() outside the capture")
            st = self.__dict__.setdefault("_lr_stage", {"bufs": [torch.empty(len(cur), dtype=torch.float32).pin_memory() for _ in range(2)],
                                                        "evs": [None, None], "k": 0})
            k = st["k"]
            if st["evs"][k] is not None:
                st["evs"][k].synchronize()
            st["bufs"][k].copy_(torch.tensor(cur, dtype=torch.float32))
            self.lrs.copy_(st["bufs"][k], non_blocking=True)
            ev = st["evs"][k] or torch.cuda.Event()
            ev.record()
            st["evs"][k] = ev
            st["k"] = 1 - k
            self._lr_host = cur

    def sync_shadows(self):
        for p, _, _, shadow, _ in self.items:
            if shadow is not None:
                shadow.half.copy_(p.detach())
                shadow.version = p._version

    def zero_grad(self, set_to_none=False):
        self.dev_state[2:3].zero_()
        for p, _, _, shadow, _ in self.items:
            if shadow is not None:
                shadow.grad_half.zero_()
                p.grad = None
            elif p.grad is not None:
                p.grad.zero_()

    def _grad(self, p, shadow):
        if shadow is not None:
            if p.grad is not None:
                shadow.grad_half.add_(p.grad.to(torch.half))
                p.grad = None
                if hasattr(shadow, "unreported"):
                    shadow.unreported = True
                    shadow.mark_all_touched()
            return shadow.grad_half, 1
        if p.grad is None:
            p.grad = torch.zeros_like(p)
        if p.grad.dtype != torch.float32 or not p.grad.is_contiguous():
            raise RuntimeError("FusedAdam: fp32 contiguous .grad expected")
        return p.grad, 0

    def _tables(self):
        grads = [self._grad(p, sh) for p, _, _, sh, _ in self.items]
        key = tuple(g.data_ptr() for g, _ in grads)
        if self._args is None or self._args["key"] != key:
            n = len(self.items)
            arr = lambda vals: (ctypes.c_void_p * n)(*vals)
            self._args = {
                "key": key, "n": n,
                "grads": arr(key), "is_half": (ctypes.c_int * n)(*[h for _, h in grads]),
                "sizes": (ctypes.c_uint64 * n)(*[p.numel() for p, *_ in self.items]),
                "params": arr([p.data_ptr() for p, *_ in self.items]),
                "m": arr([m.data_ptr() for _, m, *_ in self.items]), "v": arr([v.data_ptr() for _, _, v, *_ in self.items]),
                "shadows": arr([None if sh is None else sh.half.data_ptr() for _, _, _, sh, _ in self.items]),
                "lrs": arr([self.lrs.data_ptr() + 4 * gi for *_, gi in self.items]),
                "touched": arr([None if sh is None or getattr(sh, "touched_lines", None) is None else sh.touched_lines.data_ptr()
                                for _, _, _, sh, _ in self.items]),
            }
        return self._args

    @torch.no_grad()
    def step(self, closure=None):
        if closure is not None:
            raise RuntimeError("FusedAdam.step: closures are not supported")
        self.sync_lr()
        self.finish_loss()
        lib, st, s = _lib.load(), self.dev_state.data_ptr(), _lib.stream()
        a = self._tables()
        for *_, shadow, _ in self.items:
            if shadow is not None and getattr(shadow, "unreported", False) and hasattr(shadow, "mark_all_touched"):
                shadow.mark_all_touched()
        if self.use_scaler:
            c = self._check_tables(a)
            if c["n"]:
                _lib.check(lib.lae_adam_check_multi(c["n"], c["grads"], c["is_half"], c["sizes"], st, s), "adam_check")
        _lib.check(lib.lae_adam_begin(st, self.betas[0], self.betas[1], self.growth_interval, self.growth_factor,
                                      self.backoff_factor, int(self.use_scaler), s), "adam_begin")
        _lib.check(lib.lae_adam_apply_multi(a["n"], a["params"], a["m"], a["v"], a["grads"], a["is_half"], a["shadows"],
                                            a["sizes"], a["lrs"], a["touched"], st, self.betas[0], self.betas[1], self.eps,
                                            self.weight_decay, s), "adam_apply")
        for *_, shadow, _ in self.items:
            if shadow is not None and hasattr(shadow, "unreported"):
                shadow.unreported = False

    def _check_tables(self, a):
        keep = tuple(not (sh is not None and getattr(sh, "nonfinite_flag", None) is not None and not sh.unreported)
                     for _, _, _, sh, _ in self.items)
        cached = a.get("check")
        if cached is None or cached["keep"] != keep:
            idx = [i for i, k in enumerate(keep) if k]
            n = len(idx)
            arr = (ctypes.c_void_p * max(n, 1))
            cached = a["check"] = {"keep": keep, "n": n, "grads": arr(*[a["grads"][i] for i in idx]),
                                   "is_half": (ctypes.c_int * max(n, 1))(*[a["is_half"][i] for i in idx]),
                                   "sizes": (ctypes.c_uint64 * max(n, 1))(*[a["sizes"][i] for i in idx])}
        return cached

    def state_dict(self):
        step = float(self.steps_taken)
        for p, *_ in self.items:
            self.state[p]["step"] = torch.tensor(step)
        sd = super().state_dict()
        sd["scaler"] = {"scale": self.get_scale(), "growth_tracker": int(self.dev_state[1].item())}
        return sd

    def load_state_dict(self, sd):
        sd = dict(sd)
        scaler = sd.pop("scaler", None)
        keep = {id(p): (m, v) for p, m, v, _, _ in self.items}
        super().load_state_dict(sd)
        step = 0
        for p, m, v, _, _ in self.items:
            e = self.state[p]
            step = int(float(e["step"]))
            m.copy_(e["exp_avg"].to(m.device)); v.copy_(e["exp_avg_sq"].to(v.device))
            e["exp_avg"], e["exp_avg_sq"] = keep[id(p)]
        self.dev_state[4] = step
        for *_, shadow, _ in self.items:
            if shadow is not None and hasattr(shadow, "mark_all_touched"):
                shadow.mark_all_touched()
        self._lr_host = None
        self.sync_lr()
        if scaler is not None:
            self._scale_view[0] = scaler["scale"]
            self.dev_state[1] = scaler["growth_tracker"]


class EMA:

    def __init__(self, parameters, decay=0.95, use_num_updates=True):
        if not 0.0 <= decay <= 1.0:
            raise ValueError("decay must be between 0 and 1")
        self.params = [p for p in parameters if p.requires_grad]
        for p in self.params:
            if not p.is_cuda or p.dtype != torch.float32 or not p.is_contiguous():
                raise RuntimeError("EMA: parameters must be contiguous fp32 tensors on the GPU (no CPU fallback)")
        if len(self.params) > 8:
            raise RuntimeError("EMA: at most 8 parameter tensors (one multi-tensor launch)")
        self.decay = decay
        self.num_updates = 0 if use_num_updates else None
        self.shadow_params = [p.detach().clone() for p in self.params]
        self.collected_params = None
        n = len(self.params)
        self._n = n
        self._shadows = (ctypes.c_void_p * n)(*[t.data_ptr() for t in self.shadow_params])
        self._params = (ctypes.c_void_p * n)(*[p.data_ptr() for p in self.params])
        self._sizes = (ctypes.c_uint64 * n)(*[p.numel() for p in self.params])

    @torch.no_grad()
    def update(self):
        decay = self.decay
        if self.num_updates is not None:
            self.num_updates += 1
            decay = min(decay, (1 + self.num_updates) / (10 + self.num_updates))
        if [p.data_ptr() for p in self.params] != list(self._params):
            self._params = (ctypes.c_void_p * self._n)(*[p.data_ptr() for p in self.params])
        _lib.check(_lib.load().lae_ema_update_multi(self._n, self._shadows, self._params, self._sizes, float(1.0 - decay), _lib.stream()),
                   "ema_update")

    @torch.no_grad()
    def store(self):
        self.collected_params = [p.detach().clone() for p in self.params]

    @torch.no_grad()
    def copy_to(self):
        for s_, p in zip(self.shadow_params, self.params):
# ... 21 lines not shown
```

Baseline: 11.22.

## Skip reading zeroed fp16 grad table and fuse Adam begin/apply into one launch

Adds a device-side grad_zero flag, set when the half-precision gradient shadow has just been zeroed. The binned backward accumulator then writes fresh values without reading the old gradient, and the last exiting block clears the flag. Separately, the Adam begin and apply kernels are merged into a single step launch that uses an arrival counter. The aim is to cut memory reads of the large hash-table gradient and one kernel launch per step, at the cost of version-tracking bookkeeping that could produce stale gradients if the flag gets out of sync.

```diff
diff --git a/include/laenerf.h b/include/laenerf.h
--- a/include/laenerf.h
+++ b/include/laenerf.h
@@ -34,7 +34,7 @@
 #define LAE_ACT_SOFTPLUS 5
 #define LAE_ACT_NONE 6
 
-#define LAE_ABI_TAG "abi10"
+#define LAE_ABI_TAG "abi11"
 LAE_API const char* lae_version(void);
 LAE_API const char* lae_last_error(void);
 
@@ -195,7 +195,8 @@
                                 void* grad_embeddings, uint32_t B, uint32_t D, uint32_t C, uint32_t L, float S,
                                 uint32_t H, const void* dy_dx, void* grad_inputs, uint32_t gridtype,
                                 int align_corners, uint32_t interp, int dtype, int blc, float in_shift, float in_scale,
-                                const int32_t* offsets_host, int32_t* nonfinite_flag, uint32_t* touched_lines, void* stream);
+                                const int32_t* offsets_host, int32_t* nonfinite_flag, uint32_t* touched_lines, int32_t* grad_zero_flag,
+                                void* stream);
 
 LAE_API uint64_t lae_grid_backward_plan_bytes(uint32_t B, uint32_t L);
 LAE_API uint64_t lae_grid_touched_lines_words(uint64_t n_entries);
@@ -206,7 +207,8 @@
 LAE_API int lae_grid_encode_backward_planned(const void* grad, const float* inputs, const int32_t* offsets, void* grad_embeddings,
                                      uint32_t B, uint32_t D, uint32_t C, uint32_t L, float S, uint32_t H, uint32_t gridtype,
                                      int align_corners, uint32_t interp, int dtype, float in_shift, float in_scale,
-                                     const int32_t* offsets_host, const void* plan, int32_t* nonfinite_flag, void* stream);
+                                     const int32_t* offsets_host, const void* plan, int32_t* nonfinite_flag, int32_t* grad_zero_flag,
+                                     void* stream);
 
 LAE_API uint64_t lae_grid_backward_workspace_bytes(uint32_t B, uint32_t L, int dtype);
 
@@ -353,7 +355,12 @@
                          void* stream);
 LAE_API int lae_adam_apply_multi(uint32_t n_tensors, float* const* params, float* const* exp_avgs, float* const* exp_avg_sqs, void* const* grads,
                          const int* grad_is_half, void* const* shadows_half, const uint64_t* sizes, const float* const* lrs, const void* const* touched_lines,
-                         const void* state, float beta1, float beta2, float eps, float weight_decay, void* stream);
+                         void* const* grad_zero_flags, const void* state, float beta1, float beta2, float eps, float weight_decay, void* stream);
+#define LAE_ADAM_STEP_ARRIVAL_BYTES 4096
+LAE_API int lae_adam_step_multi(uint32_t n_tensors, float* const* params, float* const* exp_avgs, float* const* exp_avg_sqs, void* const* grads,
+                        const int* grad_is_half, void* const* shadows_half, const uint64_t* sizes, const float* const* lrs, const void* const* touched_lines,
+                        void* const* grad_zero_flags, void* state, float beta1, float beta2, float eps, float weight_decay, int growth_interval,
+                        float growth_factor, float backoff_factor, int use_scaler, void* stream);
 
 LAE_API int lae_ema_update_multi(uint32_t n_tensors, float* const* shadows, const float* const* params, const uint64_t* sizes,
                          float one_minus_decay, void* stream);
diff --git a/laenerf_amd/_lib.py b/laenerf_amd/_lib.py
--- a/laenerf_amd/_lib.py
+++ b/laenerf_amd/_lib.py
@@ -46,12 +46,12 @@
     "lae_grid_encode_forward": [vp, vp, vp, vp, u32, u32, u32, u32, f32, u32, vp, u32, i32, u32, i32, vp],
     "lae_grid_encode_backward": [vp, vp, vp, vp, vp, u32, u32, u32, u32, f32, u32, vp, vp, u32, i32, u32, i32, vp],
     "lae_grid_encode_forward_ex": [vp, vp, vp, vp, u32, u32, u32, u32, f32, u32, vp, u32, i32, u32, i32, i32, f32, f32, vp, vp],
-    "lae_grid_encode_backward_ex": [vp, vp, vp, vp, vp, u32, u32, u32, u32, f32, u32, vp, vp, u32, i32, u32, i32, i32, f32, f32, vp, vp, vp, vp],
+    "lae_grid_encode_backward_ex": [vp, vp, vp, vp, vp, u32, u32, u32, u32, f32, u32, vp, vp, u32, i32, u32, i32, i32, f32, f32, vp, vp, vp, vp, vp],
     "lae_grid_backward_workspace_bytes": [u32, u32, i32],
     "lae_grid_backward_plan_bytes": [u32, u32],
     "lae_grid_touched_lines_words": [u64],
     "lae_grid_encode_backward_plan": [vp, vp, u32, u32, u32, u32, f32, u32, u32, i32, u32, i32, f32, f32, vp, vp, vp, vp],
-    "lae_grid_encode_backward_planned": [vp, vp, vp, vp, u32, u32, u32, u32, f32, u32, u32, i32, u32, i32, f32, f32, vp, vp, vp, vp],
+    "lae_grid_encode_backward_planned": [vp, vp, vp, vp, u32, u32, u32, u32, f32, u32, u32, i32, u32, i32, f32, f32, vp, vp, vp, vp, vp],
     "lae_grid_set_backward_mode": [i32],
     "lae_grid_set_forward_mode": [i32],
     "lae_grid_forward_schedule": [vp, u32, f32, u32, u32, vp, vp],
@@ -91,7 +91,8 @@
     "lae_mse_loss_forward": [vp, vp, u32, vp, vp, vp, vp],
     "lae_adam_check": [vp, i32, u64, vp, vp],
     "lae_adam_check_multi": [u32, vp, vp, vp, vp, vp],
-    "lae_adam_apply_multi": [u32, vp, vp, vp, vp, vp, vp, vp, vp, vp, vp, f32, f32, f32, f32, vp],
+    "lae_adam_apply_multi": [u32, vp, vp, vp, vp, vp, vp, vp, vp, vp, vp, vp, f32, f32, f32, f32, vp],
+    "lae_adam_step_multi": [u32, vp, vp, vp, vp, vp, vp, vp, vp, vp, vp, vp, f32, f32, f32, f32, i32, f32, f32, i32, vp],
     "lae_adam_begin": [vp, f32, f32, i32, f32, f32, i32, vp],
     "lae_ema_update_multi": [u32, vp, vp, vp, f32, vp],
     "lae_adam_apply": [vp, vp, vp, vp, i32, vp, u64, vp, vp, f32, f32, f32, f32, vp],
@@ -120,7 +121,7 @@
 }
 
 _lib = None
-ABI_TAG = b"abi10"
+ABI_TAG = b"abi11"
 
 
 def _abi_of(path):
diff --git a/laenerf_amd/backend.py b/laenerf_amd/backend.py
--- a/laenerf_amd/backend.py
+++ b/laenerf_amd/backend.py
@@ -397,7 +397,7 @@
     @staticmethod
     def grid_encode_backward(grad, inputs, embeddings, offsets, grad_embeddings, B, D, C, L, S, H, dy_dx, grad_inputs,
                              gridtype, align_corners, interp, blc=False, in_map=(0.0, 1.0), offsets_host=None, plan=None,
-                             nonfinite_flag=None, touched_lines=None):
+                             nonfinite_flag=None, touched_lines=None, grad_zero_flag=None):
         ts = (grad, inputs, embeddings, offsets, grad_embeddings, dy_dx, grad_inputs, plan)
         need_cuda(*ts); need_contig(*ts)
         if grad.dtype != grad_embeddings.dtype:
@@ -410,14 +410,16 @@
                 raise RuntimeError("grid_encode_backward: the plan was made without the touched-lines bitmap (pass it to grid_backward_plan)")
             check(lib.lae_grid_encode_backward_planned(ptr(grad), ptr(inputs), ptr(offsets), ptr(grad_embeddings), B, D, C, L, float(S), H,
                                                        gridtype, int(bool(align_corners)), interp, _dtype_code(grad), float(in_map[0]),
-                                                       float(in_map[1]), _host_i32(offsets_host, L + 1), ptr(plan), nonfinite_flag, stream()),
+                                                       float(in_map[1]), _host_i32(offsets_host, L + 1), ptr(plan), nonfinite_flag, grad_zero_flag,
+                                                       stream()),
                   "grid_encode_backward")
             return
         args = (ptr(grad), ptr(inputs), ptr(embeddings), ptr(offsets), ptr(grad_embeddings), B, D, C, L, float(S), H,
                 ptr(dy_dx), ptr(grad_inputs), gridtype, int(bool(align_corners)), interp, _dtype_code(grad))
-        if blc or tuple(in_map) != (0.0, 1.0) or offsets_host is not None or nonfinite_flag is not None or touched_lines is not None:
+        if blc or tuple(in_map) != (0.0, 1.0) or offsets_host is not None or nonfinite_flag is not None or touched_lines is not None \
+                or grad_zero_flag is not None:
             check(lib.lae_grid_encode_backward_ex(*args, int(bool(blc)), float(in_map[0]), float(in_map[1]), _host_i32(offsets_host, L + 1),
-                                                  nonfinite_flag, touched_lines, stream()), "grid_encode_backward")
+                                                  nonfinite_flag, touched_lines, grad_zero_flag, stream()), "grid_encode_backward")
         else:
             check(lib.lae_grid_encode_backward(*args, stream()), "grid_encode_backward")
 
diff --git a/laenerf_amd/csrc/gridencoder.hip b/laenerf_amd/csrc/gridencoder.hip
--- a/laenerf_amd/csrc/gridencoder.hip
+++ b/laenerf_amd/csrc/gridencoder.hip
@@ -398,6 +398,7 @@
 constexpr uint32_t COARSE_RES = 64;
 constexpr bool WIDE_COARSE_UNITS = false;
 constexpr uint32_t SUB_RECS = 64;
+constexpr uint32_t TICKET_EXITS = 1;
 constexpr uint32_t TICKET_ARRIVALS = 2;
 constexpr uint32_t TICKET_WORDS = TICKET_ARRIVALS + MAX_LEVELS * SUB_RECS;
 template <typename T> constexpr uint32_t sub_rec_words() { return (sizeof(T) == 2 ? 2 * PART : PART) + PART / 64; }
@@ -810,15 +811,16 @@
 __global__ __launch_bounds__(ACC_THREADS, 8) void k_bwd_acc(
     const int32_t* __restrict__ offsets, T* __restrict__ grad_grid, uint32_t L, LevelScales sc, uint32_t gridtype,
     bool align_corners, BwdPlan plan, const typename BVal<T>::type* __restrict__ qvals, const uint16_t* __restrict__ qkeys,
-    unsigned long long* __restrict__ partials, int32_t* __restrict__ nf_flag, uint32_t bk_target) {
+    unsigned long long* __restrict__ partials, int32_t* __restrict__ nf_flag, uint32_t bk_target, int32_t* __restrict__ zero_flag) {
     using V = typename BVal<T>::type;
     constexpr bool HALF = sizeof(T) == 2;
     constexpr uint32_t ACCW = HALF ? 2 * PART : PART;
     __shared__ unsigned long long acc64[ACCW];
     __shared__ uint32_t poison[PART / 32];
     __shared__ uint32_t s_cnt[MAX_LEVELS], s_sub[MAX_LEVELS], s_first[MAX_LEVELS];
-    __shared__ uint32_t s_ticket, s_arr;
+    __shared__ uint32_t s_ticket, s_arr, s_zero;
     const uint32_t tid = threadIdx.x;
+    if (tid == 0) s_zero = zero_flag ? (uint32_t)*zero_flag : 0u;
     if (tid < L) {
         const LevelBins lb = level_bins_of((uint32_t)(offsets[tid + 1] - offsets[tid]), bk_target);
         s_cnt[tid] = lb.P <= BK_MAX ? lb.P * lb.SUB : 0u;
@@ -828,6 +830,7 @@
     if (tid == 0) { uint32_t run = 0; for (uint32_t l = 0; l < L; l++) { s_first[l] = run; run += s_cnt[l]; } s_arr = run; }
     __syncthreads();
     const uint32_t total_buckets = s_arr;
+    const bool grad_zero = HALF && __builtin_amdgcn_readfirstlane(s_zero) != 0u;
     __syncthreads();
 
     auto apply = [&](uint32_t key, const V& v) {
@@ -875,7 +878,10 @@
         __syncthreads();
         const uint32_t t = __builtin_amdgcn_readfirstlane(s_ticket);
         GRID_STAMP(4096 + blockIdx.x, 1 + stamp_task * 6);
-        if (t >= total_buckets) break;
+        if (t >= total_buckets) {
+            if (zero_flag && tid == 0 && atomicAdd(&plan.tickets[TICKET_EXITS], 1u) == gridDim.x - 1) *zero_flag = 0;
+            break;
+        }
         GRID_NOTE(4096 + blockIdx.x, 2 + stamp_task * 6, t);
         const uint32_t item = t;
         uint32_t level = 0;
@@ -893,7 +899,7 @@
         uint32_t oldv[HALF ? PART / ACC_THREADS : 1];
         if constexpr (HALF) {
 #pragma unroll
-            for (int it = 0; it < (int)(PART / ACC_THREADS); it++) { const uint32_t e = tid + it * ACC_THREADS; oldv[it] = e < n_ent ? reinterpret_cast<const uint32_t*>(dst)[e] : 0u; }
+            for (int it = 0; it < (int)(PART / ACC_THREADS); it++) { const uint32_t e = tid + it * ACC_THREADS; oldv[it] = e < n_ent && !grad_zero ? reinterpret_cast<const uint32_t*>(dst)[e] : 0u; }
         }
         for (uint32_t i = tid; i < ACCW; i += ACC_THREADS) acc64[i] = 0ull;
         if (tid < PART / 32) poison[tid] = 0u;
@@ -1019,6 +1025,7 @@
                 const uint32_t o = oldv[it];
                 uint32_t r0, r1;
                 if (bad) { r0 = 0x7e00u; r1 = 0x7e00u; }
+                else if (grad_zero) { r0 = fix24_to_half(i0); r1 = fix24_to_half(i1); }
                 else {
                     r0 = half_nonfinite(o) ? (o & 0xffffu) : fix24_to_half(i0 + half_to_fix24(o & 0xffffu));
                     r1 = half_nonfinite(o >> 16) ? (o >> 16) : fix24_to_half(i1 + half_to_fix24(o >> 16));
@@ -1313,6 +1320,7 @@
     uint32_t gridtype; bool align; uint32_t interp; uint64_t gs_b, gs_l; hipStream_t stream;
     const int32_t* offsets_host = nullptr;
     int32_t* nf_flag = nullptr;
+    int32_t* zero_flag = nullptr;
     uint32_t* touched = nullptr;
     uint32_t* touched_full = nullptr;
 };
@@ -1494,7 +1502,8 @@
     static const uint32_t bk_env = [] { const char* e = getenv("LAE_GRID_BWD_BK_TARGET"); return e ? (uint32_t)std::min(std::max(atoi(e), 1), (int)SUB_RECS) : 0u; }();
     static_assert(BK_TARGET <= SUB_RECS && 64u <= SUB_RECS, "bk_target choices must fit the merge records");
     const uint32_t bk_target = std::min(bk_env ? bk_env : (B >= 400000u ? 64u : BK_TARGET), SUB_RECS);
-    k_bwd_acc<T><<<(uint32_t)lae::num_cus() * 2, ACC_THREADS, 0, a.stream>>>(offsets, ge, L, a.sc, a.gridtype, a.align, plan, qvals, qkeys, partials, a.nf_flag, bk_target);
+    k_bwd_acc<T><<<(uint32_t)lae::num_cus() * 2, ACC_THREADS, 0, a.stream>>>(offsets, ge, L, a.sc, a.gridtype, a.align, plan, qvals, qkeys, partials, a.nf_flag, bk_target,
+                                                                             a.zero_flag);
     bool need_generic = true;
     if (a.offsets_host) {
         need_generic = false;
@@ -1518,14 +1527,14 @@
                          const void* dy_dx, void* grad_inputs, uint32_t gridtype, int align_corners, uint32_t interp,
                          int dtype, bool blc, void* stream, float in_shift = 0.0f, float in_scale = 1.0f,
                          const int32_t* offsets_host = nullptr, const void* plan = nullptr, int32_t* nf_flag = nullptr,
-                         uint32_t* touched = nullptr) {
+                         uint32_t* touched = nullptr, int32_t* zero_flag = nullptr) {
     (void)embeddings;
     if (B == 0) return LAE_OK;
     if (!grad || !inputs || !offsets || !grad_embeddings) return LAE_ENULL;
     if (plan && !(D == 3 && C == 2 && L <= 32 && B <= BWD_MAX_SAMPLES && !blc && !g_force_atomic_bwd)) return LAE_EINVAL;
     if (gridtype > 1 || interp > 1) return LAE_EINVAL;
     if (touched && dtype != LAE_F16) return LAE_EINVAL;
-    if (nf_flag || touched) {
+    if (nf_flag || touched || zero_flag) {
         if (!(D == 3 && C == 2 && L <= 32 && B <= BWD_MAX_SAMPLES && !g_force_atomic_bwd) || !offsets_host) return LAE_EINVAL;
         for (uint32_t l = 0; l < L; l++)
             if (!level_is_binned((uint32_t)(offsets_host[l + 1] - offsets_host[l]))) return LAE_EINVAL;
@@ -1533,6 +1542,7 @@
     BwdArgs a;
     a.offsets_host = offsets_host;
     a.nf_flag = nf_flag;
+    a.zero_flag = zero_flag;
     a.touched = touched;
     if (touched) a.touched_full = touched + touched_words(offsets_host, L);
     a.grad = grad; a.inputs = inputs; a.offsets = offsets; a.gemb = grad_embeddings; a.B = B; a.L = L;
@@ -1634,10 +1644,11 @@
                                 void* grad_embeddings, uint32_t B, uint32_t D, uint32_t C, uint32_t L, float S,
                                 uint32_t H, const void* dy_dx, void* grad_inputs, uint32_t gridtype,
                                 int align_corners, uint32_t interp, int dtype, int blc, float in_shift, float in_scale,
-                                const int32_t* offsets_host, int32_t* nonfinite_flag, uint32_t* touched_lines, void* stream) {
+                                const int32_t* offsets_host, int32_t* nonfinite_flag, uint32_t* touched_lines, int32_t* grad_zero_flag,
+                                void* stream) {
     return grid_backward(grad, inputs, embeddings, offsets, grad_embeddings, B, D, C, L, S, H, dy_dx, grad_inputs,
                          gridtype, align_corners, interp, dtype, blc != 0, stream, in_shift, in_scale, offsets_host, nullptr,
-                         nonfinite_flag, touched_lines);
+                         nonfinite_flag, touched_lines, grad_zero_flag);
 }
 
 uint64_t lae_grid_backward_workspace_bytes(uint32_t B, uint32_t L, int dtype) {
@@ -1678,10 +1689,10 @@
 int lae_grid_encode_backward_planned(const void* grad, const float* inputs, const int32_t* offsets, void* grad_embeddings, uint32_t B,
                                      uint32_t D, uint32_t C, uint32_t L, float S, uint32_t H, uint32_t gridtype, int align_corners,
                                      uint32_t interp, int dtype, float in_shift, float in_scale, const int32_t* offsets_host,
-                                     const void* plan, int32_t* nonfinite_flag, void* stream) {
+                                     const void* plan, int32_t* nonfinite_flag, int32_t* grad_zero_flag, void* stream) {
     if (!plan) return LAE_ENULL;
     return grid_backward(grad, inputs, nullptr, offsets, grad_embeddings, B, D, C, L, S, H, nullptr, nullptr, gridtype, align_corners,
-                         interp, dtype, false, stream, in_shift, in_scale, offsets_host, plan, nonfinite_flag, nullptr);
+                         interp, dtype, false, stream, in_shift, in_scale, offsets_host, plan, nonfinite_flag, nullptr, grad_zero_flag);
 }
 
 int lae_grid_forward_schedule(const int32_t* offsets_host, uint32_t L, float S, uint32_t H, uint32_t n_chunks, uint32_t* nseg_out,
diff --git a/laenerf_amd/csrc/optimizer.hip b/laenerf_amd/csrc/optimizer.hip
--- a/laenerf_amd/csrc/optimizer.hip
+++ b/laenerf_amd/csrc/optimizer.hip
@@ -22,15 +22,16 @@
     int32_t next_for;
     float next_beta1;
     float next_beta2;
-    int32_t pad[2];
+    uint32_t arrivals;
+    int32_t pad;
 };
 
 __device__ __forceinline__ void bias_corrections(float beta1, float beta2, int step, float& inv_bc1, float& bc2_sqrt) {
     inv_bc1 = (float)(1.0 / (1.0 - pow((double)beta1, (double)step)));
     bc2_sqrt = (float)sqrt(1.0 - pow((double)beta2, (double)step));
 }
-__device__ __forceinline__ void prepare_next_step(OptState* st, float beta1, float beta2) {
-    const int nxt = st->step + 1;
+__device__ __forceinline__ void prepare_next_step(OptState* st, int step, float beta1, float beta2) {
+    const int nxt = step + 1;
     float a, b;
     bias_corrections(beta1, beta2, nxt, a, b);
     st->next_inv_bc1 = a; st->next_bc2_sqrt = b; st->next_beta1 = beta1; st->next_beta2 = beta2;
@@ -62,31 +63,43 @@
     if (__any(bad) && (threadIdx.x & 63) == 0) atomicOr(&st->found_inf, 1);
 }
 
-__global__ void k_begin(OptState* __restrict__ st, float beta1, float beta2, int growth_interval, float growth, float backoff,
-                        int use_scaler) {
-    if (threadIdx.x != 0 || blockIdx.x != 0) return;
-    const bool bad = use_scaler && st->found_inf != 0;
-    st->found_inf = 0;
-    st->skip = bad;
-    st->inv_scale = use_scaler ? (float)(1.0 / (double)st->scale) : 1.0f;
+struct ScalerHyper { int growth_interval; float growth, backoff; int use_scaler; };
+
+__device__ __forceinline__ void begin_step(OptState& s, float beta1, float beta2, const ScalerHyper& sh) {
+    const bool bad = sh.use_scaler && s.found_inf != 0;
+    s.found_inf = 0;
+    s.skip = bad;
+    s.inv_scale = sh.use_scaler ? (float)(1.0 / (double)s.scale) : 1.0f;
     if (bad) {
-        st->scale = st->scale * backoff;
-        st->growth_tracker = 0;
-        st->skipped_total += 1;
+        s.scale = s.scale * sh.backoff;
+        s.growth_tracker = 0;
+        s.skipped_total += 1;
         return;
     }
-    st->step += 1;
-    if (st->next_for == st->step && st->next_beta1 == beta1 && st->next_beta2 == beta2) {
-        st->inv_bc1 = st->next_inv_bc1; st->bc2_sqrt = st->next_bc2_sqrt;
+    s.step += 1;
+    if (s.next_for == s.step && s.next_beta1 == beta1 && s.next_beta2 == beta2) {
+        s.inv_bc1 = s.next_inv_bc1; s.bc2_sqrt = s.next_bc2_sqrt;
     } else {
         float a, b;
-        bias_corrections(beta1, beta2, st->step, a, b);
-        st->inv_bc1 = a; st->bc2_sqrt = b;
-    }
-    if (use_scaler) {
-        st->growth_tracker += 1;
-        if (st->growth_tracker == growth_interval) { st->scale = st->scale * growth; st->growth_tracker = 0; }
-    }
+        bias_corrections(beta1, beta2, s.step, a, b);
+        s.inv_bc1 = a; s.bc2_sqrt = b;
+    }
+    if (sh.use_scaler) {
+        s.growth_tracker += 1;
+        if (s.growth_tracker == sh.growth_interval) { s.scale = s.scale * sh.growth; s.growth_tracker = 0; }
+    }
+}
+
+__device__ __forceinline__ void store_begun(OptState* st, const OptState& s) {
+    st->scale = s.scale; st->growth_tracker = s.growth_tracker; st->found_inf = s.found_inf; st->skip = s.skip; st->step = s.step;
+    st->inv_bc1 = s.inv_bc1; st->bc2_sqrt = s.bc2_sqrt; st->inv_scale = s.inv_scale; st->skipped_total = s.skipped_total;
+}
+
+__global__ void k_begin(OptState* __restrict__ st, float beta1, float beta2, ScalerHyper sh) {
+    if (threadIdx.x != 0 || blockIdx.x != 0) return;
+    OptState s = *st;
+    begin_step(s, beta1, beta2, sh);
+    store_begun(st, s);
 }
 
 struct AdamHyper { float beta1, beta2, eps, weight_decay; };
@@ -106,7 +119,7 @@
     const bool skip = st->skip != 0;
     const float inv_scale = st->inv_scale, bc2_sqrt = st->bc2_sqrt;
     const float lr_over_bc1 = (float)((double)lr_ptr[0] * (double)st->inv_bc1);
-    if (blockIdx.x == 0 && threadIdx.x == 0) prepare_next_step(st, h.beta1, h.beta2);
+    if (blockIdx.x == 0 && threadIdx.x == 0) prepare_next_step(st, st->step, h.beta1, h.beta2);
     const size_t stride = (size_t)gridDim.x * blockDim.x * 4;
     for (size_t i = ((size_t)blockIdx.x * blockDim.x + threadIdx.x) * 4; i < n; i += stride) {
         if (i + 4 <= n) {
@@ -156,6 +169,7 @@
     float* p[MAX_SEGS]; float* m[MAX_SEGS]; float* v[MAX_SEGS]; void* grad[MAX_SEGS]; half_t* shadow[MAX_SEGS];
     const float* lr[MAX_SEGS]; size_t n[MAX_SEGS]; int is_half[MAX_SEGS]; int count;
     const uint32_t* touched[MAX_SEGS];
+    int32_t* zero_flag[MAX_SEGS];
 };
 
 template <typename G>
@@ -239,14 +253,45 @@
     }
 }
 
-__global__ __launch_bounds__(256) void k_apply_multi(ApplySegs sg, OptState* __restrict__ st, AdamHyper h) {
-    const bool skip = st->skip != 0;
-    const float inv_scale = st->inv_scale, bc2_sqrt = st->bc2_sqrt;
-    if (blockIdx.x == gridDim.x - 1 && threadIdx.x == 0) prepare_next_step(st, h.beta1, h.beta2);
-    for (int s = 0; s < sg.count; s++) {
-        const float lr_over_bc1 = (float)((double)sg.lr[s][0] * (double)st->inv_bc1);
-        if (sg.is_half[s]) seg_apply(sg.p[s], sg.m[s], sg.v[s], (half_t*)sg.grad[s], sg.shadow[s], sg.n[s], skip, inv_scale, bc2_sqrt, lr_over_bc1, h, sg.touched[s]);
-        else seg_apply(sg.p[s], sg.m[s], sg.v[s], (float*)sg.grad[s], sg.shadow[s], sg.n[s], skip, inv_scale, bc2_sqrt, lr_over_bc1, h, sg.touched[s]);
+constexpr uint32_t ARRIVAL_GROUPS = 64, ARRIVAL_STRIDE = 16;
+static_assert(ARRIVAL_GROUPS * ARRIVAL_STRIDE * 4 <= LAE_ADAM_STEP_ARRIVAL_BYTES, "arrival counters exceed the documented area");
+
+__device__ __forceinline__ float uniform(float x) { return __builtin_bit_cast(float, __builtin_amdgcn_readfirstlane(__builtin_bit_cast(int, x))); }
+
+template <bool ONE_LAUNCH>
+__global__ __launch_bounds__(256) void k_apply_multi(ApplySegs sg, OptState* __restrict__ st, AdamHyper h, ScalerHyper sh) {
+    float inv_scale, bc2_sqrt, inv_bc1;
+    bool skip;
+    {
+        OptState s = *st;
+        if constexpr (ONE_LAUNCH) begin_step(s, h.beta1, h.beta2, sh);
+        else if (blockIdx.x == gridDim.x - 1 && threadIdx.x == 0) prepare_next_step(st, s.step, h.beta1, h.beta2);
+        skip = __builtin_amdgcn_readfirstlane(s.skip) != 0;
+        inv_scale = uniform(s.inv_scale); bc2_sqrt = uniform(s.bc2_sqrt); inv_bc1 = uniform(s.inv_bc1);
+    }
+    if (blockIdx.x == 0 && threadIdx.x == 0)
+        for (int k = 0; k < sg.count; k++) if (sg.zero_flag[k]) *sg.zero_flag[k] = 1;
+    for (int k = 0; k < sg.count; k++) {
+        const float lr_over_bc1 = (float)((double)sg.lr[k][0] * (double)inv_bc1);
+        if (sg.is_half[k]) seg_apply(sg.p[k], sg.m[k], sg.v[k], (half_t*)sg.grad[k], sg.shadow[k], sg.n[k], skip, inv_scale, bc2_sqrt, lr_over_bc1, h, sg.touched[k]);
+        else seg_apply(sg.p[k], sg.m[k], sg.v[k], (float*)sg.grad[k], sg.shadow[k], sg.n[k], skip, inv_scale, bc2_sqrt, lr_over_bc1, h, sg.touched[k]);
+    }
+    if constexpr (ONE_LAUNCH) {
+        __syncthreads();
+        if (threadIdx.x == 0) {
+            const uint32_t groups = min(gridDim.x, ARRIVAL_GROUPS), g = blockIdx.x % groups;
+            uint32_t* cnt = reinterpret_cast<uint32_t*>(st + 1) + g * ARRIVAL_STRIDE;
+            if (atomicAdd(cnt, 1u) == (gridDim.x - 1 - g) / groups) {
+                atomicExch(cnt, 0u);
+                if (atomicAdd(&st->arrivals, 1u) == groups - 1) {
+                    OptState s = *st;
+                    begin_step(s, h.beta1, h.beta2, sh);
+                    store_begun(st, s);
+                    prepare_next_step(st, s.step, h.beta1, h.beta2);
+                    atomicExch(&st->arrivals, 0u);
+                }
+            }
+        }
     }
 }
 
@@ -323,10 +368,12 @@
     return lae::check_launch("ema_update_multi");
 }
 
-int lae_adam_apply_multi(uint32_t n_tensors, float* const* params, float* const* exp_avgs, float* const* exp_avg_sqs, void* const* grads,
-                         const int* grad_is_half, void* const* shadows_half, const uint64_t* sizes, const float* const* lrs,
-                         const void* const* touched_lines, const void* state, float beta1, float beta2, float eps, float weight_decay,
-                         void* stream) {
+}
+
+static int adam_apply_multi(bool one_launch, uint32_t n_tensors, float* const* params, float* const* exp_avgs, float* const* exp_avg_sqs,
+                            void* const* grads, const int* grad_is_half, void* const* shadows_half, const uint64_t* sizes,
+                            const float* const* lrs, const void* const* touched_lines, void* const* grad_zero_flags, void* state,
+                            float beta1, float beta2, float eps, float weight_decay, ScalerHyper sh, void* stream) {
     if (n_tensors == 0) return LAE_OK;
     if (!params || !exp_avgs || !exp_avg_sqs || !grads || !grad_is_half || !shadows_half || !sizes || !lrs || !state) return LAE_ENULL;
     if (n_tensors > (uint32_t)MAX_SEGS) return LAE_EINVAL;
@@ -341,19 +388,42 @@
         sg.p[i] = params[i]; sg.m[i] = exp_avgs[i]; sg.v[i] = exp_avg_sqs[i]; sg.grad[i] = grads[i];
         sg.shadow[i] = (half_t*)shadows_half[i]; sg.lr[i] = lrs[i]; sg.n[i] = sizes[i]; sg.is_half[i] = grad_is_half[i];
         sg.touched[i] = (touched_lines && weight_decay == 0.0f) ? (const uint32_t*)touched_lines[i] : nullptr;
+        sg.zero_flag[i] = grad_zero_flags ? (int32_t*)grad_zero_flags[i] : nullptr;
         biggest = std::max(biggest, (size_t)sizes[i]);
     }
     sg.count = (int)n_tensors;
-    k_apply_multi<<<stream_blocks(biggest, 4), 256, 0, STREAM(stream)>>>(sg, reinterpret_cast<OptState*>(const_cast<void*>(state)),
-                                                                        AdamHyper{beta1, beta2, eps, weight_decay});
-    return lae::check_launch("adam_apply_multi");
+    OptState* st = reinterpret_cast<OptState*>(state);
+    const AdamHyper h{beta1, beta2, eps, weight_decay};
+    if (one_launch) k_apply_multi<true><<<stream_blocks(biggest, 4), 256, 0, STREAM(stream)>>>(sg, st, h, sh);
+    else k_apply_multi<false><<<stream_blocks(biggest, 4), 256, 0, STREAM(stream)>>>(sg, st, h, sh);
+    return lae::check_launch(one_launch ? "adam_step_multi" : "adam_apply_multi");
+}
+
+extern "C" {
+
+int lae_adam_apply_multi(uint32_t n_tensors, float* const* params, float* const* exp_avgs, float* const* exp_avg_sqs, void* const* grads,
+                         const int* grad_is_half, void* const* shadows_half, const uint64_t* sizes, const float* const* lrs,
+                         const void* const* touched_lines, void* const* grad_zero_flags, const void* state, float beta1, float beta2,
+                         float eps, float weight_decay, void* stream) {
+    return adam_apply_multi(false, n_tensors, params, exp_avgs, exp_avg_sqs, grads, grad_is_half, shadows_half, sizes, lrs, touched_lines,
+                            grad_zero_flags, const_cast<void*>(state), beta1, beta2, eps, weight_decay, ScalerHyper{}, stream);
+}
+
+int lae_adam_step_multi(uint32_t n_tensors, float* const* params, float* const* exp_avgs, float* const* exp_avg_sqs, void* const* grads,
+                        const int* grad_is_half, void* const* shadows_half, const uint64_t* sizes, const float* const* lrs,
+                        const void* const* touched_lines, void* const* grad_zero_flags, void* state, float beta1, float beta2, float eps,
+                        float weight_decay, int growth_interval, float growth_factor, float backoff_factor, int use_scaler, void* stream) {
+    if (!state) return LAE_ENULL;
+    return adam_apply_multi(true, n_tensors, params, exp_avgs, exp_avg_sqs, grads, grad_is_half, shadows_half, sizes, lrs, touched_lines,
+                            grad_zero_flags, state, beta1, beta2, eps, weight_decay,
+                            ScalerHyper{growth_interval, growth_factor, backoff_factor, use_scaler}, stream);
 }
 
 int lae_adam_begin(void* state, float beta1, float beta2, int growth_interval, float growth_factor, float backoff_factor,
                    int use_scaler, void* stream) {
     if (!state) return LAE_ENULL;
-    k_begin<<<1, 64, 0, STREAM(stream)>>>(reinterpret_cast<OptState*>(state), beta1, beta2, growth_interval, growth_factor,
-                                          backoff_factor, use_scaler);
+    k_begin<<<1, 64, 0, STREAM(stream)>>>(reinterpret_cast<OptState*>(state), beta1, beta2,
+                                          ScalerHyper{growth_interval, growth_factor, backoff_factor, use_scaler});
     return lae::check_launch("adam_begin");
 }
 
diff --git a/laenerf_amd/dist.py b/laenerf_amd/dist.py
--- a/laenerf_amd/dist.py
+++ b/laenerf_amd/dist.py
@@ -213,6 +213,8 @@
     grads = []
     for p, _, _, shadow, _ in optimizer.items:
         if shadow is not None:
+            if hasattr(shadow, "drop_zero_flag"):
+                shadow.drop_zero_flag()
             if p.grad is not None:
                 shadow.grad_half.add_(p.grad.to(torch.half)); p.grad = None
             if hasattr(shadow, "unreported"):
diff --git a/laenerf_amd/editing/style_encoder.py b/laenerf_amd/editing/style_encoder.py
--- a/laenerf_amd/editing/style_encoder.py
+++ b/laenerf_amd/editing/style_encoder.py
@@ -137,9 +137,10 @@
         if enc.shadow is not None and touched is None:
             enc.shadow.unreported = enc.shadow.unreported or flag is None
             enc.shadow.mark_all_touched()
+        zero = enc.shadow.zero_flag_for_backward(flag is not None) if enc.shadow is not None else None
         _grid.grid_encode_backward(grad_feats, x, table, enc.offsets, grad_table, M, 3, 2, L, S, H, None, None, enc.gridtype_id,
                                    enc.align_corners, enc.interp_id, blc=False, in_map=ctx.in_map, offsets_host=enc.offsets_host,
-                                   plan=ctx.plan, nonfinite_flag=flag, touched_lines=touched)
+                                   plan=ctx.plan, nonfinite_flag=flag, touched_lines=touched, grad_zero_flag=zero)
         return None, None, (None if enc.shadow is not None else grad_table), None, None, None, None, None
 
 
diff --git a/laenerf_amd/field.py b/laenerf_amd/field.py
--- a/laenerf_amd/field.py
+++ b/laenerf_amd/field.py
@@ -66,9 +66,10 @@
             touched = None
         if enc.shadow is not None and touched is None:
             enc.shadow.mark_all_touched()
+        zero = enc.shadow.zero_flag_for_backward(flag is not None) if enc.shadow is not None else None
         _grid.grid_encode_backward(grad_feats, x, table, enc.offsets, grad_table, M, 3, 2, L, S, H, None, None, enc.gridtype_id,
                                    enc.align_corners, enc.interp_id, blc=False, in_map=ctx.in_map, offsets_host=enc.offsets_host, plan=ctx.plan,
-                                   nonfinite_flag=flag, touched_lines=touched)
+                                   nonfinite_flag=flag, touched_lines=touched, grad_zero_flag=zero)
         return (None, None, None if enc.shadow is not None else grad_table,
                 None if ctx.shadows is not None else gws.to(ctx.wdtypes[0]),
                 None if ctx.shadows is not None else gwc.to(ctx.wdtypes[1]), None, None, None, None, None, None)
diff --git a/laenerf_amd/gridencoder/grid.py b/laenerf_amd/gridencoder/grid.py
--- a/laenerf_amd/gridencoder/grid.py
+++ b/laenerf_amd/gridencoder/grid.py
@@ -55,9 +55,10 @@
         if ctx.shadow is not None and (flag is None or touched is None):
             ctx.shadow.unreported = ctx.shadow.unreported or flag is None
             ctx.shadow.mark_all_touched()
+        zero = ctx.shadow.zero_flag_for_backward(flag is not None) if ctx.shadow is not None else None
         _backend.grid_encode_backward(grad, inputs, embeddings, offsets, grad_embeddings, B, D, C, L, S, H, dy_dx,
                                       grad_inputs, gridtype, ctx.align_corners, interpolation, blc=True, in_map=ctx.in_map,
-                                      offsets_host=ctx.offsets_host, nonfinite_flag=flag, touched_lines=touched)
+                                      offsets_host=ctx.offsets_host, nonfinite_flag=flag, touched_lines=touched, grad_zero_flag=zero)
         if dy_dx is not None:
             grad_inputs = grad_inputs.to(inputs.dtype)
             if ctx.in_map[1] != 1.0:
@@ -77,6 +78,21 @@
         self.nonfinite_flag = None
         self.unreported = False
         self.touched_lines = None
+        self.zero_flag = None
+        self.zero_version = None
+
+    def zero_flag_for_backward(self, binned=True):
+        if self.zero_flag is None:
+            return None
+        if binned and self.zero_version == self.grad_half._version:
+            return self.zero_flag.data_ptr()
+        self.drop_zero_flag()
+        return None
+
+    def drop_zero_flag(self):
+        if self.zero_flag is not None and self.zero_version is not None:
+            self.zero_flag.zero_()
+        self.zero_version = None
 
     def mark_all_touched(self):
         if self.touched_lines is not None:
diff --git a/laenerf_amd/optim.py b/laenerf_amd/optim.py
--- a/laenerf_amd/optim.py
+++ b/laenerf_amd/optim.py
@@ -41,13 +41,15 @@
                 self.items.append((p, m, v, shadow, gi))
         if dev is None:
             raise ValueError("FusedAdam: no parameter to optimise")
-        self.dev_state = torch.zeros(16, dtype=torch.int32, device=dev)
+        self.dev_state = torch.zeros(16 + 1024, dtype=torch.int32, device=dev)
         if self.use_scaler:
             for p, _, _, shadow, _ in self.items:
                 owner = tables.get(id(p))
                 if shadow is not None and isinstance(owner, GridEncoder) and owner.input_dim == 3 and owner.level_dim == 2 \
                         and owner.num_levels <= 32 and int((owner.offsets_host[1:] - owner.offsets_host[:-1]).max()) <= (1 << 21):
                     shadow.nonfinite_flag = self.dev_state.data_ptr() + 8
+                    if not os.environ.get("LAE_ADAM_NO_ZERO_FLAG"):
+                        shadow.zero_flag = torch.zeros(1, dtype=torch.int32, device=p.device)
                     if weight_decay == 0 and not os.environ.get("LAE_ADAM_NO_TOUCHED_LINES"):
                         n_words = int(_lib.load().lae_grid_touched_lines_words(p.shape[0]))
                         shadow.touched_lines = torch.zeros(n_words, dtype=torch.int32, device=p.device)
@@ -61,6 +63,7 @@
         if len(self.items) > 8:
             raise RuntimeError("FusedAdam: at most 8 parameter tensors (one multi-tensor launch)")
         self._args = None
+        self._one_launch = not os.environ.get("LAE_ADAM_TWO_LAUNCH")
 
     def scale(self, loss):
         return loss * self._scale_view[0] if self.use_scaler else loss
@@ -133,6 +136,9 @@
         for p, _, _, shadow, _ in self.items:
             if shadow is not None:
                 shadow.grad_half.zero_()
+                if getattr(shadow, "zero_flag", None) is not None:
+                    shadow.zero_flag.fill_(1)
+                    shadow.zero_version = shadow.grad_half._version
                 p.grad = None
             elif p.grad is not None:
                 p.grad.zero_()
@@ -140,6 +146,8 @@
     def _grad(self, p, shadow):
         if shadow is not None:
             if p.grad is not None:
+                if hasattr(shadow, "drop_zero_flag"):
+                    shadow.drop_zero_flag()
                 shadow.grad_half.add_(p.grad.to(torch.half))
                 p.grad = None
                 if hasattr(shadow, "unreported"):
@@ -168,6 +176,8 @@
                 "lrs": arr([self.lrs.data_ptr() + 4 * gi for *_, gi in self.items]),
                 "touched": arr([None if sh is None or getattr(sh, "touched_lines", None) is None else sh.touched_lines.data_ptr()
                                 for _, _, _, sh, _ in self.items]),
+                "zero": arr([None if sh is None or getattr(sh, "zero_flag", None) is None else sh.zero_flag.data_ptr()
+                             for _, _, _, sh, _ in self.items]),
             }
         return self._args
 
@@ -186,14 +196,23 @@
             c = self._check_tables(a)
             if c["n"]:
                 _lib.check(lib.lae_adam_check_multi(c["n"], c["grads"], c["is_half"], c["sizes"], st, s), "adam_check")
-        _lib.check(lib.lae_adam_begin(st, self.betas[0], self.betas[1], self.growth_interval, self.growth_factor,
-                                      self.backoff_factor, int(self.use_scaler), s), "adam_begin")
-        _lib.check(lib.lae_adam_apply_multi(a["n"], a["params"], a["m"], a["v"], a["grads"], a["is_half"], a["shadows"],
-                                            a["sizes"], a["lrs"], a["touched"], st, self.betas[0], self.betas[1], self.eps,
-                                            self.weight_decay, s), "adam_apply")
+        b1, b2 = self.betas
+        if self._one_launch:
+            _lib.check(lib.lae_adam_step_multi(a["n"], a["params"], a["m"], a["v"], a["grads"], a["is_half"], a["shadows"],
+                                               a["sizes"], a["lrs"], a["touched"], a["zero"], st, b1, b2, self.eps, self.weight_decay,
+                                               self.growth_interval, self.growth_factor, self.backoff_factor, int(self.use_scaler),
+                                               s), "adam_step")
+        else:
+            _lib.check(lib.lae_adam_begin(st, b1, b2, self.growth_interval, self.growth_factor, self.backoff_factor,
+                                          int(self.use_scaler), s), "adam_begin")
+            _lib.check(lib.lae_adam_apply_multi(a["n"], a["params"], a["m"], a["v"], a["grads"], a["is_half"], a["shadows"],
+                                                a["sizes"], a["lrs"], a["touched"], a["zero"], st, b1, b2, self.eps,
+                                                self.weight_decay, s), "adam_apply")
         for *_, shadow, _ in self.items:
             if shadow is not None and hasattr(shadow, "unreported"):
                 shadow.unreported = False
+            if shadow is not None and getattr(shadow, "zero_flag", None) is not None:
+                shadow.zero_version = shadow.grad_half._version
 
     def _check_tables(self, a):
         keep = tuple(not (sh is not None and getattr(sh, "nonfinite_flag", None) is not None and not sh.unreported)
```

After: 11.28 (median of 6 runs). No clear change (+0.5%).
